# kaleo996/F5E-TTS

Measured on AMD Instinct MI355X. Metric: mel_frames_per_sec, higher is better.
Workload: dtype bf16; 1 GPU; C2: F5TTS_v1_Base random-init, batch 1 per GPU, N_ref=188 N=469 frames, euler NFE=32, CFG=2.0 (cond+uncond batched), sway=-1.0, hipGraph ODE loop, HIP log-mel front-end + Vocos decode on GPU; parallelism=replica x1 (utterance sharding, no collective on the data path)

## Files before the change

### f5e-tts_amd/_C.py

```python
from __future__ import annotations

import ctypes as C
import os

_HERE = os.path.dirname(os.path.abspath(__file__))
LIB_PATH = os.environ.get("F5E_HIP_LIB") or os.path.join(_HERE, "libf5e_hip.so")

ABI_VERSION = 2

ACT_NONE, ACT_SILU, ACT_GELU_ERF, ACT_GELU_TANH, ACT_RELU, ACT_MISH = range(6)

_P, _I, _F, _LL = C.c_void_p, C.c_int, C.c_float, C.c_longlong

SIGNATURES = {
    "f5e_abi_version": [],
    "f5e_last_error": [],
    "f5e_check_device": [],
    "f5e_gemm_bf16_bias": [_P, _P, _I, _P, _I, _P, _P, _I, _I, _I, _I, _I, _I, _I],
    "f5e_gemm_bf16_gate_residual": [_P, _P, _I, _P, _I, _P, _P, _I, _P, _I, _I, _P, _I, _I, _P, _I, _I, _I, _I],
    "f5e_gemm_bf16_qkv_rope": [_P, _P, _I, _P, _I, _P, _P, _P, _P, _I, _I, _I, _P, _P, _P, _I, _I, _I, _I],
    "f5e_gemm_bf16_bias_ln": [_P, _P, _I, _P, _I, _P, _P, _I, _I, _I, _I, _I, _I, _I, _P],
    "f5e_gemm_bf16_gate_residual_ln": [_P, _P, _I, _P, _I, _P, _P, _I, _P, _I, _I, _P, _I, _I, _P, _I, _I, _I, _I, _P],
    "f5e_gemm_bf16_qkv_rope_ln": [_P, _P, _I, _P, _I, _P, _P, _P, _P, _I, _I, _I, _P, _P, _P, _I, _I, _I, _I, _P],
    "f5e_adaln_pre": [_P, _P, _I, _P, _I, _P, _I, _I, _I, _P, _I, _P, _I, _P, _I, _I],
    "f5e_flash_attn": [_P, _P, _P, _P, _P, _I, _P, _I, _I, _I, _I, _I],
    "f5e_joint_attn": [_P, _P, _P, _P, _P, _P, _P, _P, _I, _P, _I, _P, _I, _I, _I, _I, _I, _I, _I],
    "f5e_layernorm": [_P, _P, _I, _P, _I, _I, _P, _P, _P, _P, _I, _I, _I, _P, _I, _I, _I, _F],
    "f5e_grn": [_P, _P, _P, _P, _P, _P, _I, _I, _I],
    "f5e_l2norm": [_P, _P, _I, _P, _I, _I, _P, _I, _I],
    "f5e_gemm_f32": [_P, _P, _I, _I, _I, _P, _I, _P, _I, _P, _P, _I, _I, _P, _P, _I, _P, _I, _I, _I, _I],
    "f5e_convpos": [_P, _P, _I, _P, _P, _I, _P, _I, _P, _I, _P, _I, _I, _I, _I, _I],
    "f5e_dwconv7": [_P, _P, _P, _P, _P, _I, _I, _I],
    "f5e_im2col": [_P, _P, _P, _I, _I, _I, _I, _I],
    "f5e_sinus_embed": [_P, _P, _P, _P, _I, _I, _F],
    "f5e_rope_table": [_P, _P, _P, _I, _I],
    "f5e_text_gather": [_P, _P, _P, _P, _P, _P, _I, _I, _I, _I, _I],
    "f5e_ode_update": [_P, _P, _LL, _I, _F, _F, _P, _P, _P, _P, _P, _P, _LL],
    "f5e_ode_update_traj": [_P, _P, _LL, _I, _F, _F, _P, _P, _P, _LL, _I, _P, _P, _P, _LL],
    "f5e_advance_eval": [_P, _P],
    "f5e_stitch": [_P, _P, _P, _P, _P, _LL, _I],
    "f5e_cast_bf16": [_P, _P, _P, _LL],
    "f5e_cast_f32": [_P, _P, _P, _LL],
    "f5e_axpby": [_P, _P, _P, _P, _F, _F, _F, _LL],
    "f5e_vq_eval": [_P, _P, _I, _P, _I, _P, _P, _P, _I, _I, _I, _I],
    "f5e_mas_workspace_bytes": [_I, _I, _I, C.POINTER(C.c_ulonglong)],
    "f5e_mas_path": [_P, _P, _LL, _I, _P, _P, _P, _P, _P, C.c_ulonglong, _I, _I, _I],
    "f5e_stft_logmel": [_P, _P, _I, _I, _P, _P, _P, _P, _I, _I, _I, _I],
    "f5e_stft_logmel_banded": [_P, _P, _I, _I, _P, _P, _P, _P, _I, _P, _I, _I, _I, _I],
    "f5e_stft_logmel_banded_ex": [_P, _P, _I, _I, _P, _P, _P, _P, _I, _P, _I, _I, _I, _I, _I, _I, _F],
    "f5e_bigvgan_act": [_P, _P, _P, _I, _P, _P, _P, _P, _I, _I, _I],
    "f5e_bigvgan_conv": [_P, _P, _P, _P, _P, _P, _P, _F, _I, _I, _I, _I, _I, _I, _I, _I, _I],
    "f5e_bigvgan_post": [_P, _P, _P, _P, _P, _I, _I, _I, _I, _I],
    "f5e_istft_head": [_P, _P, _I, _P, _P, _P, _P, _I, _I, _I, _I],
    "f5e_kaldi_fbank": [_P, _P, _I, _I, _P, _P, _P, _P, _I, _I, _I, _I, _F, _F, _F],
    "f5e_glu": [_P, _P, _I, _P, _I, _LL, _I],
    "f5e_dwconv": [_P, _P, _P, _P, _P, _P, _I, _I, _I, _I],
    "f5e_softmax_rows": [_P, _P, _I, _P, _I, _P, _LL, _I, _I, _F],
    "f5e_dwconv_stream": [_P, _P, _P, _P, _P, _P, _I, _I, _I, _I, _I, _I],
    "f5e_relpos_attn": [_P, _P, _I, _P, _I, _P, _I, _P, _I, _P, _I, _P, _I, _I, _I, _I, _I, _I, _I, _F],
    "f5e_dit_forward": [_P, _P],
    "f5e_sample_loop": [_P, _P],
    "f5e_workspace_bytes": [_P, _P],
    "f5e_timer_create": [_I, C.POINTER(C.c_void_p)],
    "f5e_timer_destroy": [_P],
    "f5e_timer_reset": [_P],
    "f5e_timer_read": [_P, C.POINTER(C.c_float), _I, C.POINTER(C.c_int)],
    "f5e_timer_read_ops": [_P, C.POINTER(C.c_int), _I, C.POINTER(C.c_int)],
    "f5e_graph_begin": [_P],
    "f5e_graph_end": [_P, C.POINTER(C.c_void_p)],
    "f5e_graph_launch": [_P, _P],
    "f5e_graph_destroy": [_P],
}
_RESTYPE = {"f5e_last_error": C.c_char_p}


class BlockWeights(C.Structure):
    _fields_ = [(n, _P) for n in ("w_qkv", "b_qkv", "w_out", "b_out", "w_ff1", "b_ff1", "w_ff2", "b_ff2",
                                  "q_norm_w", "k_norm_w")]


class LnFuse(C.Structure):
    _fields_ = [("stats", _P), ("parts", _I), ("c", _P), ("d", _P), ("cd_stride", _I), ("cd_rows", _I),
                ("cd_eval_stride", _I), ("eval_ptr", _P), ("rows_per_seq", _I), ("eps", _F),
                ("xs_out", _P), ("ld_xs", _I), ("next_scale", _P), ("stats_out", _P), ("row_mean", _P)]


class DitPlan(C.Structure):
    _fields_ = (
        [(n, _I) for n in ("S", "B", "N", "n_pad", "D", "H", "rope_heads", "FF", "L", "mel", "mod_rows")]
        + [("y", _P), ("w_x", _P), ("ldw_x", _I), ("in_const", _P)]
        + [(n, _P) for n in ("convpos_w1", "convpos_b1", "convpos_w2", "convpos_b2")] + [("convpos_groups", _I)]
        + [(n, _P) for n in ("rope_cs", "seq_len", "mod", "eval_ptr")]
        + [("blocks", C.POINTER(BlockWeights)), ("w_proj", _P), ("b_proj", _P)]
        + [("w_skip", _P), ("skip_res", _P), ("skip_tmp", _P)]
        + [(n, _P) for n in ("h0", "h0_bf16", "c1", "x", "hn", "q", "k", "vt", "ao", "ff", "pred")]
        + [("timer", _P), ("timer_op", _I)]
        + [("fuse_ln", _I), ("ln_stats", _P), ("ln_rowmean", _P), ("cd", _P), ("cd_stride", _I)]
        + [("mall_prefetch", _I)]
    )

class LoopPlan(C.Structure):
    _fields_ = [("eval_a", C.POINTER(DitPlan)), ("eval_b", C.POINTER(DitPlan)), ("steps", _I), ("mode", _I), ("w0", _F),
                ("w1", _F), ("n", _LL), ("y", _P), ("y_mid", _P), ("pred", _P), ("coef", _P), ("eval_ptr", _P),
                ("done_ctr", _P), ("traj", _P)]


WS_NAMES = ("h0", "h0_bf16", "c1", "x", "hn", "q", "k", "vt", "ao", "ff", "pred", "ln_stats", "skip_res", "skip_tmp",
            "ln_rowmean")


class DitWorkspace(C.Structure):
    _fields_ = [("n_pad", _I), ("bytes", C.c_ulonglong * len(WS_NAMES)), ("offset", C.c_ulonglong * len(WS_NAMES)),
                ("total", C.c_ulonglong)]


OP_NONE, OP_INPROJ, OP_CONVPOS, OP_LN, OP_QKV, OP_ATTN, OP_OUT, OP_FF1, OP_FF2, OP_FINAL = range(10)


_lib = None


def lib() -> C.CDLL:
    global _lib
    if _lib is None:
        if not os.path.exists(LIB_PATH):
            raise RuntimeError(
                f"{LIB_PATH} is missing: the HIP extension is required (no CPU/PyTorch fallback exists). "
                "Build it with `make -C f5e-tts_amd/csrc` or `__graft_entry__.build()`."
            )
        handle = C.CDLL(LIB_PATH)
        for name, argtypes in SIGNATURES.items():
            fn = getattr(handle, name)
            fn.argtypes = argtypes
            fn.restype = _RESTYPE.get(name, C.c_int)
        if handle.f5e_abi_version() != ABI_VERSION:
            raise RuntimeError(f"libf5e_hip ABI version {handle.f5e_abi_version()} != {ABI_VERSION}")
        _lib = handle
    return _lib


class F5EError(RuntimeError):
    pass


def check(rc: int, name: str) -> None:
    if rc != 0:
        msg = lib().f5e_last_error()
        raise F5EError(f"{name} failed ({rc}): {msg.decode() if msg else '?'}")
```

### f5e-tts_amd/csrc/conv.hip

```cpp
#include <cstdlib>
#include "f5e_common.h"

namespace {

struct ConvPosArgs {
  const bf16* x; int ldx;
  const bf16* w;
  const float* bias;
  bf16* out_bf16; int ldo;
  float* out_f32; int ldo32;
  const float* resid; int ldr;
  int S, N, D, mode, tiles_t, cpg;
  unsigned long long* trace;
};

__device__ __forceinline__ void glds16c(const void* g, void* lds) {
  __builtin_amdgcn_global_load_lds((const __attribute__((address_space(1))) void*)g,
                                   (__attribute__((address_space(3))) void*)lds, 16, 0, 0);
}

__device__ const uint4 conv_zero16 = {0u, 0u, 0u, 0u};

__device__ __forceinline__ void wait_vm_lgkm0(int n) {
  switch (n) {
// ... 152 lines not shown
}

template <bool TRC = false>
__global__ __launch_bounds__(256) void convpos_split_kernel(ConvPosArgs a) {
  unsigned long long ts[8] = {0, 0, 0, 0, 0, 0, 0, 0};
  if constexpr (TRC) { ts[0] = __builtin_amdgcn_s_memrealtime(); ts[1] = __builtin_amdgcn_s_memtime(); }
  constexpr int BT = 64, HALO = 15, XR = BT + 2 * HALO;
  constexpr int X_BYTES = 96 * 128, W_BYTES = 8192, NST = 4;
  constexpr int TAPS = 31, RS = 68;
  extern __shared__ __attribute__((aligned(16))) char smem[];
  char* Xs = smem;
  char* ring_base = smem + X_BYTES;
  float* Red = (float*)ring_base;

  const int tid = threadIdx.x, lane = tid & 63;
  const int wave = __builtin_amdgcn_readfirstlane(tid >> 6);
  const int g = blockIdx.x, tt = blockIdx.y, seq = blockIdx.z;
  const int c0 = g * a.cpg;
  const int t0 = tt * BT;
  const int fr = lane & 15, fq = lane >> 4;

  const int oc = (lane & 15) * 4;
  const int n = c0 + (oc < a.cpg ? oc : 0);
  f32x4 rv[4];
  if (a.mode == 1) {
#pragma unroll
    for (int p = 0; p < 4; ++p) {
      const int t = t0 + wave * 16 + p * 4 + (lane >> 4);
      rv[p] = *(const f32x4*)(a.resid + ((size_t)seq * a.N + (t < a.N ? t : a.N - 1)) * a.ldr + n);
    }
  }
  const f32x4 bias = *(const f32x4*)(a.bias + n);
  asm volatile("" ::: "memory");
  __builtin_amdgcn_sched_barrier(0);
#pragma unroll
  for (int r = 0; r < 3; ++r) {
    const int i = tid + 256 * r;
    const int row = i >> 3, c = (i & 7) ^ ((row >> 1) & 7);
    const int t = t0 - HALO + row;
    const void* src = &conv_zero16;
    if (row < XR && t >= 0 && t < a.N && c0 + c * 8 < a.D) src = a.x + ((size_t)seq * a.N + t) * a.ldx + c0 + c * 8;
    glds16c(src, Xs + (wave * 64 + 256 * r) * 16);
  }
  asm volatile("" ::: "memory");
  __builtin_amdgcn_sched_barrier(0);

  char* ring = ring_base + wave * (NST * W_BYTES);
  const bf16* wg = a.w + (size_t)g * TAPS * 4096;
  const bf16* w_src[8];
#pragma unroll
  for (int j = 0; j < 8; ++j) {
    const int i = lane + 64 * j;
    const int row = i >> 3, c = (i & 7) ^ ((row >> 1) & 7);
    w_src[j] = wg + row * 64 + c * 8;
  }
  auto stage_w = [&](int slot, int u) {
    int tap = wave + 4 * u;
    tap = tap < TAPS ? tap : TAPS - 1;
#pragma unroll
    for (int j = 0; j < 8; ++j) glds16c(w_src[j] + (size_t)tap * 4096, ring + slot * W_BYTES + j * 1024);
  };
#pragma unroll
  for (int u = 0; u < NST - 1; ++u) stage_w(u, u);

  f32x4 acc[4][4];
#pragma unroll
  for (int i = 0; i < 4; ++i)
#pragma unroll
    for (int j = 0; j < 4; ++j) acc[i][j] = f32x4{0.f, 0.f, 0.f, 0.f};

#pragma unroll
  for (int u = 0; u < 8; ++u) {
    const int issued = u + NST - 1 < 8 ? u + NST - 1 : 8;
    const int pend = 8 * (issued - u - 1);
    if (pend == 16) asm volatile("s_waitcnt vmcnt(16) lgkmcnt(0)" ::: "memory");
    else if (pend == 8) asm volatile("s_waitcnt vmcnt(8) lgkmcnt(0)" ::: "memory");
    else asm volatile("s_waitcnt vmcnt(0) lgkmcnt(0)" ::: "memory");
    if (u == 0) {
      __builtin_amdgcn_s_barrier();
      if constexpr (TRC) ts[2] = __builtin_amdgcn_s_memtime();
    }
    if constexpr (TRC) { if (u == 1) ts[3] = __builtin_amdgcn_s_memtime(); if (u == 4) ts[4] = __builtin_amdgcn_s_memtime(); }
    const int tap = wave + 4 * u;
    const bool live = !(u == 7 && tap >= TAPS);
    const char* Ws = ring + (u % NST) * W_BYTES;
    bf16x8 xf[4], wf[4];
    auto reads = [&](int kk) {
      const int c = kk * 4 + fq;
#pragma unroll
      for (int j = 0; j < 4; ++j) {
        const int row = j * 16 + fr + tap;
        xf[j] = *(const bf16x8*)(Xs + row * 128 + ((c ^ ((row >> 1) & 7)) << 4));
      }
#pragma unroll
      for (int i = 0; i < 4; ++i) {
        const int row = i * 16 + fr;
        wf[i] = *(const bf16x8*)(Ws + row * 128 + ((c ^ ((row >> 1) & 7)) << 4));
      }
    };
    auto mfmas = [&]() {
#pragma unroll
      for (int i = 0; i < 4; ++i)
#pragma unroll
        for (int j = 0; j < 4; ++j)
          acc[i][j] = __builtin_amdgcn_mfma_f32_16x16x32_bf16(wf[i], xf[j], acc[i][j], 0, 0, 0);
    };
    if (live) reads(0);
    if (u + NST - 1 < 8) stage_w((u + NST - 1) % NST, u + NST - 1);
    if (!live) break;
    mfmas();
    reads(1);
    mfmas();
  }

  if constexpr (TRC) ts[5] = __builtin_amdgcn_s_memtime();
  asm volatile("s_waitcnt vmcnt(0) lgkmcnt(0)" ::: "memory");
  __builtin_amdgcn_s_barrier();
  float* mine = Red + wave * (64 * RS);
#pragma unroll
  for (int i = 0; i < 4; ++i)
#pragma unroll
    for (int j = 0; j < 4; ++j) *(f32x4*)(mine + (j * 16 + fr) * RS + i * 16 + fq * 4) = acc[i][j];
  asm volatile("s_waitcnt lgkmcnt(0)" ::: "memory");
  __builtin_amdgcn_s_barrier();
#pragma unroll
  for (int p = 0; p < 4; ++p) asm volatile("" : "+v"(rv[p]));

  if (oc < a.cpg) {
#pragma unroll
    for (int p = 0; p < 4; ++p) {
      const int row = wave * 16 + p * 4 + (lane >> 4);
      const int t = t0 + row;
      const size_t m = (size_t)seq * a.N + t;
      const float* rp = Red + row * RS + oc;
      f32x4 v = (*(const f32x4*)rp + *(const f32x4*)(rp + 64 * RS)) + (*(const f32x4*)(rp + 2 * 64 * RS) + *(const f32x4*)(rp + 3 * 64 * RS));
      v += bias;
      v[0] = mish_f(v[0]); v[1] = mish_f(v[1]); v[2] = mish_f(v[2]); v[3] = mish_f(v[3]);
      if (t >= a.N) continue;
      if (a.mode == 0) {
        *(bf16x4*)(a.out_bf16 + m * a.ldo + n) = f2bf4(v[0], v[1], v[2], v[3]);
      } else {
        v += rv[p];
        *(f32x4*)(a.out_f32 + m * a.ldo32 + n) = v;
      }
    }
  }
  if constexpr (TRC) {
    asm volatile("s_waitcnt vmcnt(0)" ::: "memory");
    ts[6] = __builtin_amdgcn_s_memtime(); ts[7] = __builtin_amdgcn_s_memrealtime();
    if (tid == 0 && a.trace) {
      unsigned long long* o = a.trace + ((size_t)(blockIdx.z * gridDim.y + blockIdx.y) * gridDim.x + blockIdx.x) * 8;
#pragma unroll
      for (int i = 0; i < 8; ++i) o[i] = ts[i];
    }
  }
}

__global__ __launch_bounds__(256) void dwconv7_kernel(const float* x, const float* wT, const float* bias, float* y,
                                                       int B, int T, int C) {
  const int c4n = C / 4;
  const size_t total = (size_t)B * T * c4n;
  for (size_t i = (size_t)blockIdx.x * 256 + threadIdx.x; i < total; i += (size_t)gridDim.x * 256) {
    const int c = (int)(i % c4n) * 4;
    const size_t bt = i / c4n;
    const int t = (int)(bt % T);
    const size_t b = bt / T;
    f32x4 acc = *(const f32x4*)(bias + c);
#pragma unroll
    for (int j = 0; j < 7; ++j) {
      const int tj = t + j - 3;
      if (tj >= 0 && tj < T)
        acc += *(const f32x4*)(wT + (size_t)j * C + c) * *(const f32x4*)(x + (b * T + tj) * C + c);
    }
    *(f32x4*)(y + (b * T + t) * C + c) = acc;
  }
}

__global__ __launch_bounds__(256) void im2col_kernel(const float* x, float* col, int B, int T, int Cin, int ksize,
                                                      int pad) {
  const size_t total = (size_t)B * T * ksize * Cin;
  for (size_t i = (size_t)blockIdx.x * 256 + threadIdx.x; i < total; i += (size_t)gridDim.x * 256) {
    const int ic = (int)(i % Cin);
    size_t r = i / Cin;
    const int j = (int)(r % ksize);
    r /= ksize;
    const int t = (int)(r % T);
    const size_t b = r / T;
    const int tj = t + j - pad;
    col[i] = (tj >= 0 && tj < T) ? x[(b * T + tj) * Cin + ic] : 0.f;
  }
}

inline int grid_for(size_t total) {
  size_t g = (total + 255) / 256;
  return (int)(g < 4096 ? (g ? g : 1) : 4096);
}

}

#ifdef F5E_TOOLS
static unsigned long long* g_convpos_trace = nullptr;
#define F5E_CONVPOS_TRACE g_convpos_trace
#else
#define F5E_CONVPOS_TRACE ((unsigned long long*)nullptr)
#endif

extern "C" {

#ifdef F5E_TOOLS
void f5e_debug_convpos_trace(void* buf) { g_convpos_trace = (unsigned long long*)buf; }
#endif

static int convpos_launch(hipStream_t st, const void* x, int ldx, const void* w_packed, const float* bias, int mode,
                          void* out_bf16, int ldo, float* out_f32, int ldo32, const float* resid, int ldr, int S, int N,
                          int D, int groups) {
  F5E_REQUIRE(x && w_packed && bias, "convpos: null operand");
  F5E_REQUIRE(S > 0 && N > 0 && D > 0 && groups > 0 && D % groups == 0, "convpos: bad D=%d / groups=%d", D, groups);
  const int cpg = D / groups;
  F5E_REQUIRE(cpg % 16 == 0 && cpg <= 64, "convpos: channels per group = %d must be 16, 32, 48 or 64", cpg);
  F5E_REQUIRE(ldx % 8 == 0, "convpos: ldx must be a multiple of 8");
  if (mode == 0) F5E_REQUIRE(out_bf16 && ldo % 4 == 0, "convpos: mode 0 needs a bf16 output");
  else {
    F5E_REQUIRE(mode == 1, "convpos: mode must be 0 or 1");
    F5E_REQUIRE(out_f32 && resid && ldo32 % 4 == 0 && ldr % 4 == 0, "convpos: mode 1 needs f32 output + residual");
  }
  ConvPosArgs a{};
  a.x = (const bf16*)x; a.ldx = ldx; a.w = (const bf16*)w_packed; a.bias = bias;
  a.out_bf16 = (bf16*)out_bf16; a.ldo = ldo; a.out_f32 = out_f32; a.ldo32 = ldo32; a.resid = resid; a.ldr = ldr;
  a.S = S; a.N = N; a.D = D; a.mode = mode; a.cpg = cpg;
  a.tiles_t = (N + 63) / 64;
  F5E_REQUIRE(a.tiles_t <= 65535 && S <= 65535, "convpos: grid too large");
  const dim3 grid(groups, a.tiles_t, S);
  const int xs = 96 * 128;
#ifdef F5E_TOOLS
  static const int forced = getenv("F5E_CONVPOS") ? atoi(getenv("F5E_CONVPOS")) : 0;
#else
  constexpr int forced = 0;
#endif
  const int n_cu = f5e_cu_count();
  const bool split = forced ? forced == 1 : (size_t)groups * a.tiles_t * S <= (size_t)n_cu;
  const int lds_split = xs + 4 * 4 * 8192, lds_ring = xs + 4 * 8192;
  a.trace = F5E_CONVPOS_TRACE;
  static F5eDeviceOnce once_split;
  if (split) F5E_OPT_IN_LDS(once_split, convpos_split_kernel<false>, lds_split);
#ifdef F5E_TOOLS
  static F5eDeviceOnce once_split_trace;
  if (split && a.trace) {
    F5E_OPT_IN_LDS(once_split_trace, convpos_split_kernel<true>, lds_split);
    hipLaunchKernelGGL(convpos_split_kernel<true>, grid, dim3(256), lds_split, st, a);
  } else if (a.trace) {
    hipLaunchKernelGGL((convpos_kernel<4, true>), grid, dim3(256), lds_ring, st, a);
  } else
#endif
  if (split) {
    hipLaunchKernelGGL(convpos_split_kernel<false>, grid, dim3(256), lds_split, st, a);
  } else {
    hipLaunchKernelGGL((convpos_kernel<4, false>), grid, dim3(256), lds_ring, st, a);
  }
  F5E_LAUNCH_CHECK("convpos");
  return F5E_OK;
}

int f5e_convpos(hipStream_t st, const void* x, int ldx, const void* w_packed, const float* bias, int mode,
                void* out_bf16, int ldo, float* out_f32, int ldo32, const float* resid, int ldr, int S, int N, int D,
                int groups) {
  return convpos_launch(st, x, ldx, w_packed, bias, mode, out_bf16, ldo, out_f32, ldo32, resid, ldr, S, N, D, groups);
}

int f5e_dwconv7(hipStream_t st, const float* x, const float* w_t, const float* bias, float* y, int B, int T, int C) {
  F5E_REQUIRE(x && w_t && bias && y, "dwconv7: null operand");
  F5E_REQUIRE(B > 0 && T > 0 && C > 0 && C % 4 == 0, "dwconv7: C=%d must be a positive multiple of 4", C);
  hipLaunchKernelGGL(dwconv7_kernel, dim3(grid_for((size_t)B * T * C / 4)), dim3(256), 0, st, x, w_t, bias, y, B, T, C);
  F5E_LAUNCH_CHECK("dwconv7");
  return F5E_OK;
}

int f5e_im2col(hipStream_t st, const float* x, float* col, int B, int T, int Cin, int ksize, int pad) {
  F5E_REQUIRE(x && col && B > 0 && T > 0 && Cin > 0 && ksize > 0 && pad >= 0, "im2col: bad arguments");
  hipLaunchKernelGGL(im2col_kernel, dim3(grid_for((size_t)B * T * Cin * ksize)), dim3(256), 0, st, x, col, B, T, Cin,
                     ksize, pad);
  F5E_LAUNCH_CHECK("im2col");
  return F5E_OK;
}

}
```

### f5e-tts_amd/csrc/elementwise.hip

```cpp
#include "f5e_common.h"

namespace {

inline int grid_for(size_t total) {
  size_t g = (total + 255) / 256;
  return (int)(g < 2048 ? (g ? g : 1) : 2048);
}

__global__ void sinus_embed_kernel(const float* t, const float* freqs, float* out, int E, int dim, float scale) {
  const int half = dim / 2;
  const int i = blockIdx.x * blockDim.x + threadIdx.x;
  if (i >= E * half) return;
  const int e = i / half, k = i - e * half;
  const float arg = (scale * t[e]) * freqs[k];
  float s, c;
  sincosf(arg, &s, &c);
  out[(size_t)e * dim + k] = s;
  out[(size_t)e * dim + half + k] = c;
}

__global__ void rope_table_kernel(const float* inv_freq, float* out, int N, int half) {
  const int i = blockIdx.x * blockDim.x + threadIdx.x;
  if (i >= N * half) return;
  const int n = i / half, k = i - n * half;
  const float ang = (float)n * inv_freq[k];
  float s, c;
  sincosf(ang, &s, &c);
  out[(size_t)i * 2] = c;
  out[(size_t)i * 2 + 1] = s;
}

__global__ void text_gather_kernel(const int* ids, const float* table, const float* pos, const float* keep, float* out,
                                   int B, int N, int TD, int max_pos, int table_rows) {
  const int td4 = TD / 4;
  const size_t total = (size_t)B * N * td4;
  for (size_t i = (size_t)blockIdx.x * 256 + threadIdx.x; i < total; i += (size_t)gridDim.x * 256) {
    const int c = (int)(i % td4) * 4;
    const size_t bn = i / td4;
    const int n = (int)(bn % N);
    const int id = min(max(ids[bn], 0), table_rows - 1);
    f32x4 v = *(const f32x4*)(table + (size_t)id * TD + c);
    if (pos) v += *(const f32x4*)(pos + (size_t)min(n, max_pos - 1) * TD + c);
    if (keep) v *= keep[bn];
    *(f32x4*)(out + bn * TD + c) = v;
  }
}

__global__ void ode_update_kernel(const float* pred, size_t branch_stride, int mode, float w0, float w1,
                                  const float* base, float* dst, float* traj, size_t traj_stride, int traj_div,
                                  const float* coef, int* eval_ptr, unsigned* done_ctr, size_t n) {
  const int e = eval_ptr ? load_uniform_i32(eval_ptr) : 0;
  const float h = __builtin_bit_cast(float, load_uniform_i32((const int*)(coef + e)));
  if (traj && traj_stride) traj += (size_t)((e + 1) / traj_div) * traj_stride;
  for (size_t i = (size_t)blockIdx.x * 256 + threadIdx.x; i < n; i += (size_t)gridDim.x * 256) {
    const float p0 = pred[i];
    float v = p0;
    if (mode == 1) {
      v = p0 + (p0 - pred[i + branch_stride]) * w0;
    } else if (mode == 2) {
      const float p1 = pred[i + branch_stride], p2 = pred[i + 2 * branch_stride];
      v = w0 * (p2 - p1) + w1 * (p1 - p0) + p0;
    }
    const float y = base[i] + h * v;
    dst[i] = y;
    if (traj) traj[i] = y;
  }
  if (done_ctr) {
    __syncthreads();
    if (threadIdx.x == 0) {
      const unsigned t = atomicAdd(done_ctr, 1u);
      if (t == gridDim.x - 1) {
        *eval_ptr = e + 1;
        *done_ctr = 0u;
      }
    }
  }
}

__global__ void advance_eval_kernel(int* eval_ptr) { *eval_ptr += 1; }

__global__ void stitch_kernel(const float* cond, const float* y, const unsigned char* mask, float* out, size_t rows,
                              int C) {
  const size_t total = rows * C;
  for (size_t i = (size_t)blockIdx.x * 256 + threadIdx.x; i < total; i += (size_t)gridDim.x * 256)
    out[i] = mask[i / C] ? cond[i] : y[i];
}

__global__ void cast_bf16_kernel(const float* x, bf16* y, size_t n) {
  for (size_t i = (size_t)blockIdx.x * 256 + threadIdx.x; i < n; i += (size_t)gridDim.x * 256) y[i] = (bf16)x[i];
}

__global__ void cast_f32_kernel(const bf16* x, float* y, size_t n) {
  for (size_t i = (size_t)blockIdx.x * 256 + threadIdx.x; i < n; i += (size_t)gridDim.x * 256) y[i] = (float)x[i];
}

__global__ void axpby_kernel(const float* x, const float* y, float* out, float a, float b, float c, size_t n) {
  for (size_t i = (size_t)blockIdx.x * 256 + threadIdx.x; i < n; i += (size_t)gridDim.x * 256)
    out[i] = a * x[i] + (y ? b * y[i] : 0.0f) + c;
}

__global__ __launch_bounds__(256) void vq_lookup_kernel(const float* logits, int ld, const float* vars, int combine,
                                                         float* out, int* targets, int rows, int G, int V, int vd) {
  const int lane = threadIdx.x & 63;
  const long long item = (long long)blockIdx.x * 4 + (threadIdx.x >> 6);
  if (item >= (long long)rows * G) return;
  const int r = (int)(item / G), g = (int)(item % G);
  const float* lp = logits + (size_t)r * ld + (size_t)g * V;
  float best = -INFINITY;
  int bi = 0x7fffffff;
  for (int v = lane; v < V; v += 64) {
    const float x = lp[v];
    if (x > best) { best = x; bi = v; }
  }
#pragma unroll
  for (int o = 32; o > 0; o >>= 1) {
    const float ob = __shfl_xor(best, o, 64);
    const int oi = __shfl_xor(bi, o, 64);
    if (ob > best || (ob == best && oi < bi)) { best = ob; bi = oi; }
  }
  if (lane == 0 && targets) targets[(size_t)r * G + g] = bi;
  const float* src = vars + ((size_t)(combine ? 0 : g) * V + bi) * vd;
  for (int d = lane; d < vd; d += 64) out[(size_t)r * G * vd + (size_t)g * vd + d] = src[d];
}

__global__ __launch_bounds__(256) void vq_stats_kernel(const float* logits, int ld, const int* targets, float* stats,
                                                        int rows, int G, int V) {
  extern __shared__ float sm[];
  float* accw = sm;
  float* cnt = sm + 4 * V;
  __shared__ float red[2];
  const int tid = threadIdx.x, lane = tid & 63, wave = tid >> 6;
  float code_ppl = 0.f, prob_ppl = 0.f;
  for (int g = 0; g < G; ++g) {
    for (int i = tid; i < 5 * V; i += 256) sm[i] = 0.f;
    __syncthreads();
    for (int r = wave; r < rows; r += 4) {
      const float* lp = logits + (size_t)r * ld + (size_t)g * V;
      float mx = -INFINITY;
      for (int v = lane; v < V; v += 64) mx = fmaxf(mx, lp[v]);
      mx = wave_max(mx);
      float s = 0.f;
      for (int v = lane; v < V; v += 64) s += expf(lp[v] - mx);
      s = wave_sum(s);
      const float inv = 1.0f / s;
      for (int v = lane; v < V; v += 64) accw[wave * V + v] += expf(lp[v] - mx) * inv;
    }
    __syncthreads();
    if (tid == 0)
      for (int r = 0; r < rows; ++r) cnt[targets[(size_t)r * G + g]] += 1.0f;
    __syncthreads();
    float hc = 0.f, hp = 0.f;
    for (int v = tid; v < V; v += 256) {
      const float p_hard = cnt[v] / (float)rows;
      const float p_avg = ((accw[v] + accw[V + v]) + (accw[2 * V + v] + accw[3 * V + v])) / (float)rows;
      hc += p_hard * logf(p_hard + 1e-7f);
      hp += p_avg * logf(p_avg + 1e-7f);
    }
    hc = wave_sum(hc);
    hp = wave_sum(hp);
    if (tid == 0) { red[0] = 0.f; red[1] = 0.f; }
    __syncthreads();
    if (lane == 0) { atomicAdd(&red[0], hc); atomicAdd(&red[1], hp); }
    __syncthreads();
    code_ppl += expf(-red[0]);
    prob_ppl += expf(-red[1]);
    __syncthreads();
  }
  if (tid == 0) { stats[0] = code_ppl; stats[1] = prob_ppl; }
}

}

extern "C" {

int f5e_sinus_embed(hipStream_t st, const float* t, const float* freqs, float* out, int E, int dim, float scale) {
  F5E_REQUIRE(t && freqs && out && E > 0 && dim >= 4 && dim % 2 == 0, "sinus_embed: bad arguments");
  const int total = E * dim / 2;
  hipLaunchKernelGGL(sinus_embed_kernel, dim3((total + 255) / 256), dim3(256), 0, st, t, freqs, out, E, dim, scale);
  F5E_LAUNCH_CHECK("sinus_embed");
  return F5E_OK;
}

int f5e_rope_table(hipStream_t st, const float* inv_freq, float* out, int N, int half) {
  F5E_REQUIRE(inv_freq && out && N > 0 && half > 0, "rope_table: bad arguments");
  const int total = N * half;
  hipLaunchKernelGGL(rope_table_kernel, dim3((total + 255) / 256), dim3(256), 0, st, inv_freq, out, N, half);
  F5E_LAUNCH_CHECK("rope_table");
  return F5E_OK;
}

int f5e_text_gather(hipStream_t st, const int* ids, const float* table, const float* pos, const float* keep,
                    float* out, int B, int N, int TD, int max_pos, int table_rows) {
  F5E_REQUIRE(ids && table && out && B > 0 && N > 0 && TD > 0 && TD % 4 == 0 && table_rows > 0, "text_gather: bad arguments");
  hipLaunchKernelGGL(text_gather_kernel, dim3(grid_for((size_t)B * N * TD / 4)), dim3(256), 0, st, ids, table, pos,
                     keep, out, B, N, TD, max_pos, table_rows);
  F5E_LAUNCH_CHECK("text_gather");
  return F5E_OK;
}

int f5e_ode_update(hipStream_t st, const float* pred, long long branch_stride, int mode, float w0, float w1,
                   const float* base, float* dst, float* traj, const float* coef, int* eval_ptr, unsigned* done_ctr,
                   long long n) {
  return f5e_ode_update_traj(st, pred, branch_stride, mode, w0, w1, base, dst, traj, 0, 1, coef, eval_ptr, done_ctr, n);
}

int f5e_ode_update_traj(hipStream_t st, const float* pred, long long branch_stride, int mode, float w0, float w1,
                        const float* base, float* dst, float* traj, long long traj_stride, int traj_div,
                        const float* coef, int* eval_ptr, unsigned* done_ctr, long long n) {
  F5E_REQUIRE(pred && base && dst && coef && n > 0, "ode_update: bad arguments");
  F5E_REQUIRE(mode >= 0 && mode <= 2, "ode_update: mode must be 0 (plain), 1 (cfg) or 2 (three-branch)");
  F5E_REQUIRE(!done_ctr || eval_ptr, "ode_update: done_ctr (auto-advance) needs eval_ptr");
  F5E_REQUIRE(traj_stride >= 0 && traj_div >= 1 && (traj_stride == 0 || eval_ptr), "ode_update: bad trajectory indexing");
  hipLaunchKernelGGL(ode_update_kernel, dim3(grid_for((size_t)n)), dim3(256), 0, st, pred, (size_t)branch_stride, mode,
                     w0, w1, base, dst, traj, (size_t)traj_stride, traj_div, coef, eval_ptr, done_ctr, (size_t)n);
  F5E_LAUNCH_CHECK("ode_update");
  return F5E_OK;
// ... 58 lines not shown
```

### f5e-tts_amd/csrc/f5e_common.h

```cpp
#pragma once
#include <hip/hip_runtime.h>
#include <stdint.h>
#define F5E_STREAM_T hipStream_t
#include "../../include/f5e_abi.h"

typedef __bf16 bf16;
typedef __attribute__((ext_vector_type(2))) __bf16 bf16x2;
typedef __attribute__((ext_vector_type(4))) __bf16 bf16x4;
typedef __attribute__((ext_vector_type(8))) __bf16 bf16x8;
typedef __attribute__((ext_vector_type(2))) float f32x2;
typedef __attribute__((ext_vector_type(4))) float f32x4;
typedef __attribute__((ext_vector_type(16))) float f32x16;

#define F5E_WAVE 64

void f5e_set_error(const char* fmt, ...);

#define F5E_REQUIRE(cond, ...)                         \
  do {                                                 \
    if (!(cond)) {                                     \
      f5e_set_error(__VA_ARGS__);                      \
      return F5E_ERR_BAD_SHAPE;                        \
    }                                                  \
  } while (0)

#include <atomic>
inline int f5e_device_index() {
  int dev = 0;
  (void)hipGetDevice(&dev);
  return dev < 0 ? 0 : (dev > 63 ? 63 : dev);
}
struct F5eDeviceOnce {
  std::atomic<unsigned long long> done{0};
};
inline hipError_t f5e_opt_in_lds(F5eDeviceOnce& once, const void* kernel, int lds_bytes) {
  const unsigned long long bit = 1ull << f5e_device_index();
  if (once.done.load(std::memory_order_acquire) & bit) return hipSuccess;
  hipError_t e = hipFuncSetAttribute(kernel, hipFuncAttributeMaxDynamicSharedMemorySize, lds_bytes);
  if (e == hipSuccess) once.done.fetch_or(bit, std::memory_order_release);
  return e;
}
#define F5E_OPT_IN_LDS(once, kernel, lds)                                                    \
  do {                                                                                       \
    hipError_t e_ = f5e_opt_in_lds(once, (const void*)(kernel), lds);                        \
    if (e_ != hipSuccess) {                                                                  \
      f5e_set_error("hipFuncSetAttribute(%d B of LDS): %s", (int)(lds), hipGetErrorString(e_)); \
      return F5E_ERR_HIP;                                                                    \
    }                                                                                        \
  } while (0)
inline int f5e_cu_count() {
  static std::atomic<int> cache[64];
  const int dev = f5e_device_index();
  int n = cache[dev].load(std::memory_order_relaxed);
  if (n == 0) {
    int v = 0;
    if (hipDeviceGetAttribute(&v, hipDeviceAttributeMultiprocessorCount, dev) != hipSuccess || v <= 0) v = 256;
    cache[dev].store(v, std::memory_order_relaxed);
    n = v;
  }
  return n;
}

struct F5ePrefetch {
  const void* ptr[2];
  unsigned bytes[2];
};
constexpr int F5E_PF_BYTES_PER_WG = 32 * 1024;
inline int f5e_prefetch_wgs(const F5ePrefetch* pf) {
  if (!pf) return 0;
  unsigned long long b = (pf->ptr[0] ? pf->bytes[0] : 0) + (unsigned long long)(pf->ptr[1] ? pf->bytes[1] : 0);
  return (int)((b + F5E_PF_BYTES_PER_WG - 1) / F5E_PF_BYTES_PER_WG);
}
template <int NT = 256>
__device__ __forceinline__ void f5e_prefetch_run(const F5ePrefetch& pf, int wg, int tid, void* lds) {
  unsigned long long off = (unsigned long long)wg * F5E_PF_BYTES_PER_WG + (unsigned)tid * 16u;
  const unsigned long long b0 = pf.ptr[0] ? pf.bytes[0] : 0, b1 = pf.ptr[1] ? pf.bytes[1] : 0;
  char* dst = (char*)lds + (tid >> 6) * 1024;
#pragma unroll
  for (int i = 0; i < F5E_PF_BYTES_PER_WG / (NT * 16); ++i, off += NT * 16) {
    const char* p = nullptr;
    if (off + 16 <= b0) p = (const char*)pf.ptr[0] + off;
    else if (off >= b0 && off - b0 + 16 <= b1) p = (const char*)pf.ptr[1] + (off - b0);
    if (p)
      __builtin_amdgcn_global_load_lds((const __attribute__((address_space(1))) void*)p,
                                       (__attribute__((address_space(3))) void*)dst, 16, 0, 0);
  }
}

__device__ __forceinline__ void f5e_prefetch_run_packed(const F5ePrefetch& pf, int wg, int tid, int nt, unsigned per_wg,
                                                        void* lds) {
  unsigned long long off = (unsigned long long)wg * per_wg + (unsigned)tid * 16u;
  const unsigned long long end = (unsigned long long)(wg + 1) * per_wg;
  const unsigned long long b0 = pf.ptr[0] ? pf.bytes[0] : 0, b1 = pf.ptr[1] ? pf.bytes[1] : 0;
  char* dst = (char*)lds + (tid >> 6) * 1024;
  for (; off < end; off += (unsigned)nt * 16u) {
    const char* p = nullptr;
    if (off + 16 <= b0) p = (const char*)pf.ptr[0] + off;
    else if (off >= b0 && off - b0 + 16 <= b1) p = (const char*)pf.ptr[1] + (off - b0);
    if (p)
      __builtin_amdgcn_global_load_lds((const __attribute__((address_space(1))) void*)p,
                                       (__attribute__((address_space(3))) void*)dst, 16, 0, 0);
  }
}

int f5e_gemm_bf16_bias_pf(hipStream_t st, const void* A, int lda, const void* W, int ldw, const float* bias, void* out,
                          int ldo, int M, int N, int K, int act, int out_f32, int tile_hint, const f5e_ln_fuse* ln,
                          const F5ePrefetch* pf);
int f5e_gemm_bf16_gate_residual_pf(hipStream_t st, const void* A, int lda, const void* W, int ldw, const float* bias,
                                   float* resid, int ldr, const float* gate, int gate_stride, int gate_rows,
                                   const int* eval_ptr, int eval_stride, int rows_per_seq, const int* seq_len, int M,
                                   int N, int K, int tile_hint, const f5e_ln_fuse* ln, const F5ePrefetch* pf);
int f5e_gemm_bf16_qkv_rope_pf(hipStream_t st, const void* A, int lda, const void* W, int ldw, const float* bias, void* q,
                              void* k, void* vt, int n_pad, int heads, int rope_heads, const float* cos_sin,
                              const float* q_norm_w, const float* k_norm_w, int rows_per_seq, int M, int K, int tile_hint,
                              const f5e_ln_fuse* ln, const F5ePrefetch* pf);
int f5e_flash_attn_pf(hipStream_t st, const void* q, const void* k, const void* v, void* o, int ldo, const int* kv_len,
                      int S, int H, int rows_per_seq, int n_pad, int splits, const F5ePrefetch* pf);

#define F5E_LAUNCH_CHECK(name)                                                   \
  do {                                                                           \
    hipError_t e_ = hipGetLastError();                                           \
    if (e_ != hipSuccess) {                                                      \
      f5e_set_error("%s: launch failed: %s", name, hipGetErrorString(e_));       \
      return F5E_ERR_HIP;                                                        \
    }                                                                            \
  } while (0)

__device__ __forceinline__ int load_uniform_i32(const int* p) {
  return *(const __attribute__((address_space(4))) int*)(uintptr_t)p;
}

__device__ __forceinline__ bf16x4 f2bf4(float a, float b, float c, float d) {
  f32x4 v = {a, b, c, d};
  return __builtin_convertvector(v, bf16x4);
}
__device__ __forceinline__ bf16x2 f2bf2(float a, float b) {
  f32x2 v = {a, b};
  return __builtin_convertvector(v, bf16x2);
}
template <int CTRL>
__device__ __forceinline__ float dpp_f32(float v) {
  return __builtin_bit_cast(float, __builtin_amdgcn_update_dpp(0, __builtin_bit_cast(int, v), CTRL, 0xF, 0xF, false));
}
__device__ __forceinline__ float add_xor1(float v) { return v + dpp_f32<0xB1>(v); }
__device__ __forceinline__ float add_xor2(float v) { return v + dpp_f32<0x4E>(v); }
__device__ __forceinline__ void swap16(float& a, float& b) {
  asm volatile("s_nop 1\n\tv_permlane16_swap_b32 %0, %1" : "+v"(a), "+v"(b));
}
__device__ __forceinline__ void swap32(float& a, float& b) {
  asm volatile("s_nop 1\n\tv_permlane32_swap_b32 %0, %1" : "+v"(a), "+v"(b));
}
__device__ __forceinline__ float add_xor16(float v) {
  float a = v, b = v;
  swap16(a, b);
  return a + b;
}
__device__ __forceinline__ float add_xor32(float v) {
  float a = v, b = v;
  swap32(a, b);
  return a + b;
}
__device__ __forceinline__ float max_xor32(float v) {
  float a = v, b = v;
  swap32(a, b);
  return fmaxf(a, b);
}
__device__ __forceinline__ float wave_sum(float v) {
  v = add_xor1(v);
  v = add_xor2(v);
  v += dpp_f32<0x124>(v);
  v += dpp_f32<0x128>(v);
  v = add_xor16(v);
  return add_xor32(v);
}
__device__ __forceinline__ float wave_max(float v) {
#pragma unroll
  for (int o = 32; o > 0; o >>= 1) v = fmaxf(v, __shfl_xor(v, o, 64));
  return v;
}
__device__ __forceinline__ float gelu_tanh_f(float x) {
  const float t = x * x;
  const float p = __builtin_fmaf(t, -2.0f * 0.7978845608028654f * 1.4426950408889634f * 0.044715f,
                                 -2.0f * 0.7978845608028654f * 1.4426950408889634f);
  const float e = __builtin_amdgcn_exp2f(x * p);
  return x * __builtin_amdgcn_rcpf(1.0f + e);
}
__device__ __forceinline__ float gelu_erf_f(float x) { return 0.5f * x * (1.0f + erff(x * 0.7071067811865476f)); }
__device__ __forceinline__ float silu_f(float x) { return x / (1.0f + __expf(-x)); }
__device__ __forceinline__ float mish_f(float x) {
  const float e = __builtin_amdgcn_exp2f(fminf(x, 20.0f) * 1.4426950408889634f);
  const float n = e * (e + 2.0f);
  const float r = x * (n * __builtin_amdgcn_rcpf(n + 2.0f));
  return x > 20.0f ? x : r;
}
__device__ __forceinline__ float apply_act(float x, int act) {
  switch (act) {
    case F5E_ACT_SILU: return silu_f(x);
    case F5E_ACT_GELU_ERF: return gelu_erf_f(x);
    case F5E_ACT_GELU_TANH: return gelu_tanh_f(x);
    case F5E_ACT_RELU: return fmaxf(x, 0.0f);
    case F5E_ACT_MISH: return mish_f(x);
    default: return x;
  }
}
```

### f5e-tts_amd/csrc/gemm_bf16.hip

```cpp
#include <cstdlib>
#include <type_traits>

#include "f5e_common.h"
#include "gemm_bf16_args.h"

namespace {

using namespace f5e_gemm;

template <int N>
__device__ __forceinline__ void wait_vm_lgkm0() {
  asm volatile("s_waitcnt vmcnt(%0) lgkmcnt(0)" ::"n"(N) : "memory");
}

template <int LPT, int EXTRA>
__device__ __forceinline__ void wait_stages(int nst) {
  constexpr auto C = [](int v) constexpr { return v > 63 ? 63 : v; };
  switch (nst) {
    case 0: wait_vm_lgkm0<C(EXTRA)>(); break;
    case 1: wait_vm_lgkm0<C(LPT + EXTRA)>(); break;
    case 2: wait_vm_lgkm0<C(2 * LPT + EXTRA)>(); break;
    case 3: wait_vm_lgkm0<C(3 * LPT + EXTRA)>(); break;
    case 4: wait_vm_lgkm0<C(4 * LPT + EXTRA)>(); break;
    case 5: wait_vm_lgkm0<C(5 * LPT + EXTRA)>(); break;
    default: wait_vm_lgkm0<C(6 * LPT + EXTRA)>(); break;
  }
}

template <int BM, int BN, int EPI, int NSTAGE, int DBG = 0, int WGM = 2, int WGN = 2, int FUSE = 0, int NLOAD = 0, int DSTEP = 1, int DBUF = 1>
__global__ __launch_bounds__(64 * (WGM * WGN + NLOAD)) void gemm_bf16_kernel(GemmArgs a) {
  constexpr int BK = 64;
  constexpr int CPR = BK / 8;
  constexpr int ROWB = BK * 2;
  auto swz = [](int row) { return (row >> 1) & 7; };
  constexpr int NCW = WGM * WGN;
  constexpr int NC = 64 * NCW;
  constexpr int NT = NLOAD ? 64 * NLOAD : NC;
  constexpr int A_BYTES = BM * BK * 2;
  constexpr int W_BYTES = BN * BK * 2;
  constexpr int STAGE = A_BYTES + W_BYTES;
  constexpr int WM = BM / WGM, WN = BN / WGN;
  constexpr int TM = WM / 16, TN = WN / 16;
  extern __shared__ __attribute__((aligned(16))) char smem[];

  const int lane = threadIdx.x & 63;
  const int wave = __builtin_amdgcn_readfirstlane(threadIdx.x >> 6);
  const int tid = (int)threadIdx.x;
  const bool is_loader = NLOAD > 0 && wave >= NCW;
  const int stid = NLOAD ? tid - NC : tid;
  const int swave = NLOAD ? wave - NCW : wave;
  unsigned long long* trc = nullptr;
  if constexpr (DBG >= 3) {
    trc = a.trace + (size_t)blockIdx.x * 48;
    if (tid == 0) { trc[0] = __builtin_amdgcn_s_memrealtime(); trc[1] = __builtin_amdgcn_s_memtime(); }
  }

  if (FUSE == 1)
    asm volatile("" ::"s"(a.ln_stats), "s"(a.ln_c), "s"(a.ln_d), "s"(a.ln_parts), "s"(a.cd_stride), "s"(a.cd_rows),
                 "s"(a.cd_eval_stride), "s"(a.eval_ptr));
  if (EPI == EPI_GATE_RES)
    asm volatile("" ::"s"(a.resid), "s"(a.gate), "s"(a.seq_len), "s"(a.eval_ptr), "s"(a.ldr), "s"(a.gate_stride),
                 "s"(a.gate_rows), "s"(a.eval_stride), "s"(a.bias));
  if (FUSE == 2) asm volatile("" ::"s"(a.next_scale), "s"(a.xs_out), "s"(a.stats_out), "s"(a.ld_xs), "s"(a.row_mean));
  if (EPI == EPI_QKV_ROPE) asm volatile("" ::"s"(a.q), "s"(a.k), "s"(a.vt), "s"(a.cos_sin), "s"(a.n_pad), "s"(a.heads), "s"(a.rope_heads));

  if ((int)blockIdx.x >= a.n_main) {
    if (NLOAD > 0 && a.pf_per_wg) f5e_prefetch_run_packed(a.pf, (int)blockIdx.x - a.n_main, tid, 64 * (NCW + NLOAD), a.pf_per_wg, smem);
    else if (tid < 256) f5e_prefetch_run(a.pf, (int)blockIdx.x - a.n_main, tid, smem);
    return;
  }
  int bid = blockIdx.x;
  {
    const int nblk = a.n_main;
    const int q8 = nblk >> 3, r8 = nblk & 7;
    const int xcd = bid & 7, idx = bid >> 3;
    bid = (xcd < r8 ? xcd * (q8 + 1) : r8 * (q8 + 1) + (xcd - r8) * q8) + idx;
  }
  int tile_m, tile_n;
  if (a.m_major > 0) {
    tile_m = div_magic(bid, a.tiles_n, a.tile_magic);
    tile_n = bid - tile_m * a.tiles_n;
  } else {
    const int sh = -a.m_major, per = a.tiles_m << sh;
    const int g = div_magic(bid, per, a.tile_magic);
    const int r = bid - g * per;
    tile_m = r >> sh;
    tile_n = (g << sh) + (r & ((1 << sh) - 1));
  }
  const int m0 = tile_m * BM, n0 = tile_n * BN;

  constexpr int A_IT = BM * CPR / NT;
  constexpr int W_IT = BN * CPR / NT;
  static_assert(A_IT >= 1 && W_IT >= 1 && A_IT * NT == BM * CPR && W_IT * NT == BN * CPR, "tile / thread-count mismatch");
  unsigned a_off[A_IT], w_off[W_IT];
#pragma unroll
  for (int j = 0; j < A_IT; ++j) {
    const int i = (stid & (NT - 1)) + NT * j;
    const int row = i / CPR, c = (i % CPR) ^ swz(row);
    a_off[j] = (unsigned)(min(m0 + row, a.M - 1) - m0) * (unsigned)(a.lda * 2) + (unsigned)c * 16u;
  }
#pragma unroll
  for (int j = 0; j < W_IT; ++j) {
    const int i = (stid & (NT - 1)) + NT * j;
    const int row = i / CPR, c = (i % CPR) ^ swz(row);
    w_off[j] = (unsigned)(min(n0 + row, a.N - 1) - n0) * (unsigned)(a.ldw * 2) + (unsigned)c * 16u;
  }
  const char* const a_base = (const char*)(a.A + (size_t)m0 * a.lda);
  const char* const w_base = (const char*)(a.W + (size_t)n0 * a.ldw);
  const int KT = a.K / BK;
  char* const ring = smem;
  auto stage = [&](int buf, int kt) {
    char* base = ring + buf * STAGE;
    const char* ak = a_base + (size_t)kt * (BK * 2);
    const char* wk = w_base + (size_t)kt * (BK * 2);
#pragma unroll
    for (int j = 0; j < A_IT; ++j) glds16_s(ak, a_off[j], base + (swave * 64 + NT * j) * 16);
#pragma unroll
    for (int j = 0; j < W_IT; ++j) glds16_s(wk, w_off[j], base + A_BYTES + (swave * 64 + NT * j) * 16);
  };

  const int wm0 = (wave / WGN) * WM, wn0 = (wave % WGN) * WN;
  const int fr = lane & 15, fq = lane >> 4;

  f32x4 acc[TN][TM];
#pragma unroll
  for (int i = 0; i < TN; ++i)
#pragma unroll
    for (int j = 0; j < TM; ++j) acc[i][j] = f32x4{0.f, 0.f, 0.f, 0.f};

  constexpr int LPT = A_IT + W_IT;
  static_assert(NSTAGE >= 2 && NSTAGE <= 8 && (DSTEP > 1 || (NSTAGE - 2) * LPT <= 63), "vmcnt is a 6-bit counter");
  static_assert((NT & (NT - 1)) == 0, "staging thread count must be a power of two");
  static_assert(DSTEP == 1 || (NLOAD > 0 && DSTEP == 2 && NSTAGE >= 3 * DSTEP), "DSTEP: role split, ring of >= 3 steps");
  constexpr int NPRO = NSTAGE - DSTEP;
  static_assert((NSTAGE - 2 * DSTEP) * LPT <= 63, "vmcnt is a 6-bit counter");
  if (NLOAD == 0 || is_loader) {
#pragma unroll
    for (int s = 0; s < NPRO; ++s)
      if (s < KT) stage(s, s);
  }
  if constexpr (NLOAD > 0) {
    if (is_loader) {
      int nbuf_l = NPRO % NSTAGE;
      if constexpr (DBG >= 3) { if (stid == 0) trc[47] = __builtin_amdgcn_s_memtime(); }
      for (int kt = 0; kt < KT; kt += DSTEP) {
        const int rem = KT - DSTEP - kt;
        wait_stages<LPT, 0>(rem < NSTAGE - 2 * DSTEP ? (rem < 0 ? 0 : rem) : NSTAGE - 2 * DSTEP);
        __builtin_amdgcn_s_barrier();
#pragma unroll
        for (int d = 0; d < DSTEP; ++d) {
          if (kt + NPRO + d < KT) stage(nbuf_l, kt + NPRO + d);
          nbuf_l = (nbuf_l + 1 == NSTAGE) ? 0 : nbuf_l + 1;
        }
      }
      if (FUSE == 1) __syncthreads();
      if (FUSE == 2) __builtin_amdgcn_s_barrier();
      return;
    }
  }
  asm volatile("" ::: "memory");
  if constexpr (DBG >= 3) { if (tid == 0) trc[46] = __builtin_amdgcn_s_memtime(); }
  constexpr bool PREF = (TM * TN <= 4);
  static_assert(FUSE != 2 || (PREF && WM == 32 && WN == 32 && BN == 64 && (BM == 64 || (BM == 128 && NLOAD > 0))),
                "fused AdaLN producer: 64 (or, role split, 128) x 64 tiles of 32 x 32 wave sub-tiles");
  static_assert(FUSE != 1 || (WN == 32 && (BN == 64 || NLOAD > 0) && ((BM == 64 && WM == 32) || (BM == 128 && WM == 64 && NLOAD > 0))),
                "fused AdaLN consumer: 64-row tiles of 32 x 32 wave sub-tiles, or (role split) 128-row tiles of 64 x 32 ones");
  static_assert(DBUF == 1 || (NLOAD > 0 && DSTEP == 1), "single fragment set: role split, one tile per hand-over");
  constexpr int NSTATT = BM * 4;
  static_assert(FUSE != 1 || NSTATT <= NC, "fused consumer: 4 statistics threads per row");
  static_assert(FUSE != 2 || EPI == EPI_GATE_RES, "the AdaLN producer is the gate+residual epilogue");
  constexpr int NPC = NLOAD ? 0 : (FUSE == 1 ? 2 * TN + 4 : (FUSE == 2 ? 3 * TM * TN : ((PREF && EPI == EPI_GATE_RES) ? 2 * TM * TN : 0)));
  static_assert((NSTAGE - 2) * LPT + NPC <= 63, "vmcnt is a 6-bit counter");
  constexpr bool COLG = NLOAD > 0;
  f32x4 pf_bias[PREF ? TN : 1], pf_gate[PREF ? TN : 1][PREF ? (COLG ? 1 : TM) : 1], pf_x[PREF ? TN : 1][PREF ? TM : 1];
  f32x4 pf_c[FUSE == 1 ? TN : 1], pf_d[FUSE == 1 ? TN : 1];
  f32x4 pf_ns[FUSE == 2 ? TN : 1][FUSE == 2 ? (COLG ? 1 : TM) : 1];
  f32x2 pf_st[FUSE == 1 ? 4 : 1];
  bool pf_live[PREF ? TM : 1];
  int pf_len[PREF ? TM : 1];
  float pf_rm[FUSE == 2 ? TM : 1];
  auto ldv4 = [](const float* ptr) -> f32x4 { return *(const f32x4*)ptr; };
  auto fetch_epilogue_operands = [&]() {
    if (PREF) {
      if (EPI == EPI_GATE_RES) {
        const size_t eoff = a.eval_ptr ? (size_t)load_uniform_i32(a.eval_ptr) * a.eval_stride : 0;
#pragma unroll
        for (int j = 0; j < TM; ++j) {
          const int m = m0 + wm0 + j * 16 + fr, mc = min(m, a.M - 1);
          const int seq = div_magic(mc, a.rows_per_seq, a.rps_magic);
#pragma unroll
          for (int i = 0; i < TN; ++i) {
            const int nc = min(n0 + wn0 + i * 16 + fq * 4, a.N - 4);
            const size_t goff = eoff + ((COLG || a.gate_rows == 1) ? 0 : (size_t)(seq % a.gate_rows) * a.gate_stride) + nc;
            if (!COLG || j == 0) pf_gate[i][COLG ? 0 : j] = ldv4(a.gate + goff);
            pf_x[i][j] = ldv4(a.resid + (size_t)mc * a.ldr + nc);
            if (FUSE == 2 && (!COLG || j == 0)) pf_ns[i][COLG ? 0 : j] = ldv4(a.next_scale + goff);
          }
        }
      }
    }
    if (FUSE == 1) {
      const size_t eoff = a.eval_ptr ? (size_t)load_uniform_i32(a.eval_ptr) * a.cd_eval_stride : 0;
      const float* cbase = a.ln_c + eoff;
      const float* dbase = a.ln_d + eoff;
#pragma unroll
      for (int i = 0; i < TN; ++i) {
        const unsigned nc = (unsigned)min(n0 + wn0 + i * 16 + fq * 4, a.N - 4);
        pf_c[i] = ldv4(cbase + nc);
        pf_d[i] = ldv4(dbase + nc);
      }
      const int pp = a.ln_parts >> 2;
      const float* sbase = a.ln_stats + (size_t)m0 * a.ln_parts * 2;
      const unsigned rel_max = (unsigned)((a.M - m0) * a.ln_parts - 1);
#pragma unroll
      for (int u = 0; u < 4; ++u) {
        const unsigned rel = min((unsigned)((tid & (NSTATT - 1)) * pp + min(u, pp - 1)), rel_max);
        if (NC == NSTATT || tid < NSTATT) pf_st[u] = *(const f32x2*)(sbase + rel * 2u);
      }
    }
    if (PREF) {
#pragma unroll
      for (int i = 0; i < TN; ++i) {
        const int n = n0 + wn0 + i * 16 + fq * 4;
        pf_bias[i] = (a.bias && n < a.N) ? *(const f32x4*)(a.bias + n) : f32x4{0.f, 0.f, 0.f, 0.f};
      }
      if (EPI == EPI_GATE_RES) {
#pragma unroll
        for (int j = 0; j < TM; ++j) {
          const int mc = min(m0 + wm0 + j * 16 + fr, a.M - 1);
          pf_len[j] = a.seq_len ? a.seq_len[div_magic(mc, a.rows_per_seq, a.rps_magic)] : a.rows_per_seq;
          if (FUSE == 2) pf_rm[j] = a.row_mean[mc];
        }
      }
    }
  };
  if (NLOAD == 0) fetch_epilogue_operands();

  int buf = 0, nbuf = NSTAGE - 1;
  if constexpr (DBG >= 3) { if (tid == 0) trc[2] = __builtin_amdgcn_s_memtime(); }
  if constexpr (NLOAD > 0) {
    bf16x8 xs2[DBUF + 1][BK / 32][TM], ws2[DBUF + 1][BK / 32][TN];
    auto reads = [&](auto pc, int b) {
      constexpr int P = decltype(pc)::value;
      const char* As = ring + b * STAGE;
      const char* Ws = As + A_BYTES;
#pragma unroll
      for (int kk = 0; kk < BK / 32; ++kk) {
        const int c = kk * 4 + fq;
#pragma unroll
        for (int j = 0; j < TM; ++j) {
          const int row = wm0 + j * 16 + fr;
          xs2[P][kk][j] = *(const bf16x8*)(As + row * ROWB + ((c ^ swz(row)) << 4));
        }
#pragma unroll
        for (int i = 0; i < TN; ++i) {
          const int row = wn0 + i * 16 + fr;
          ws2[P][kk][i] = *(const bf16x8*)(Ws + row * ROWB + ((c ^ swz(row)) << 4));
        }
      }
    };
    auto mfmas = [&](auto pc) {
      constexpr int P = decltype(pc)::value;
#pragma unroll
      for (int kk = 0; kk < BK / 32; ++kk)
#pragma unroll
        for (int i = 0; i < TN; ++i)
#pragma unroll
          for (int j = 0; j < TM; ++j)
            acc[i][j] = __builtin_amdgcn_mfma_f32_16x16x32_bf16(ws2[P][kk][i], xs2[P][kk][j], acc[i][j], 0, 0, 0);
    };
    auto body = [&](auto pc, int kt) {
      constexpr int P = decltype(pc)::value;
      if (DSTEP == 1 || P == 0) __builtin_amdgcn_s_barrier();
      if constexpr (DBG >= 3) { if (tid == 0 && kt < 36) trc[4 + kt] = __builtin_amdgcn_s_memtime(); }
      reads(pc, buf);
      if (kt > 0) mfmas(std::integral_constant<int, 1 - P>{});
      if (DSTEP == 1 || P == 1) asm volatile("s_waitcnt lgkmcnt(0)" ::: "memory");
      buf = (buf + 1 == NSTAGE) ? 0 : buf + 1;
    };
    if constexpr (DBUF == 0) {
      auto reads_half = [&](int kk, int b) {
        if constexpr (DBG == 5) return;
        const char* As = ring + b * STAGE;
        const char* Ws = As + A_BYTES;
        const int c = kk * 4 + fq;
#pragma unroll
        for (int j = 0; j < TM; ++j) {
          const int row = wm0 + j * 16 + fr;
          xs2[0][kk][j] = *(const bf16x8*)(As + row * ROWB + ((c ^ swz(row)) << 4));
        }
#pragma unroll
        for (int i = 0; i < TN; ++i) {
          const int row = wn0 + i * 16 + fr;
          ws2[0][kk][i] = *(const bf16x8*)(Ws + row * ROWB + ((c ^ swz(row)) << 4));
        }
      };
      auto mfmas_half = [&](int kk) {
        if constexpr (DBG == 4 || DBG == 5) return;
#pragma unroll
        for (int i = 0; i < TN; ++i)
#pragma unroll
          for (int j = 0; j < TM; ++j)
            acc[i][j] = __builtin_amdgcn_mfma_f32_16x16x32_bf16(ws2[0][kk][i], xs2[0][kk][j], acc[i][j], 0, 0, 0);
      };
      static_assert(BK == 64, "half-tile pipelining: two 32-k halves per K-tile");
      for (int kt = 0; kt < KT; ++kt) {
        __builtin_amdgcn_s_barrier();
        if constexpr (DBG >= 3) { if (tid == 0 && kt < 36) trc[4 + kt] = __builtin_amdgcn_s_memtime(); }
        reads_half(0, buf);
        if (kt > 0) mfmas_half(1);
        if (kt == 0) fetch_epilogue_operands();
        asm volatile("s_waitcnt lgkmcnt(0)" ::: "memory");
        reads_half(1, buf);
        mfmas_half(0);
        asm volatile("s_waitcnt lgkmcnt(0)" ::: "memory");
        buf = (buf + 1 == NSTAGE) ? 0 : buf + 1;
      }
      mfmas_half(1);
    } else {
      for (int kt = 0; kt < KT; kt += 2) {
        body(std::integral_constant<int, 0>{}, kt);
        if (kt == 0) fetch_epilogue_operands();
        if (kt + 1 < KT) body(std::integral_constant<int, 1>{}, kt + 1);
      }
      if ((KT - 1) & 1) mfmas(std::integral_constant<int, 1>{});
      else mfmas(std::integral_constant<int, 0>{});
    }
  } else
  for (int kt = 0; kt < KT; ++kt) {
    const int rem = KT - 1 - kt;
    const int nst = rem < NSTAGE - 2 ? rem : NSTAGE - 2;
    if (NPC > 0 && kt <= NSTAGE - 2) wait_stages<LPT, NPC>(nst);
    else wait_stages<LPT, 0>(nst);
    __builtin_amdgcn_s_barrier();
    if constexpr (DBG >= 3) { if (tid == 0 && kt < 36) trc[4 + kt] = __builtin_amdgcn_s_memtime(); }
    const bool more = kt + NSTAGE - 1 < KT;
    const char* As = ring + buf * STAGE;
    const char* Ws = As + A_BYTES;
    bf16x8 xf[BK / 32][TM], wf[BK / 32][TN];
#pragma unroll
    for (int kk = 0; kk < BK / 32; ++kk) {
      const int c = kk * 4 + fq;
#pragma unroll
      for (int j = 0; j < TM; ++j) {
        const int row = wm0 + j * 16 + fr;
        xf[kk][j] = *(const bf16x8*)(As + row * ROWB + ((c ^ swz(row)) << 4));
      }
#pragma unroll
      for (int i = 0; i < TN; ++i) {
        const int row = wn0 + i * 16 + fr;
        wf[kk][i] = *(const bf16x8*)(Ws + row * ROWB + ((c ^ swz(row)) << 4));
      }
    }
    if (more) stage(nbuf, kt + NSTAGE - 1);
#pragma unroll
    for (int kk = 0; kk < BK / 32; ++kk)
#pragma unroll
      for (int i = 0; i < TN; ++i)
#pragma unroll
        for (int j = 0; j < TM; ++j)
          acc[i][j] = __builtin_amdgcn_mfma_f32_16x16x32_bf16(wf[kk][i], xf[kk][j], acc[i][j], 0, 0, 0);
    buf = (buf + 1 == NSTAGE) ? 0 : buf + 1;
    nbuf = (nbuf + 1 == NSTAGE) ? 0 : nbuf + 1;
  }

  if constexpr (DBG >= 3) { if (tid == 0) trc[3] = __builtin_amdgcn_s_memtime(); }
  float* fuse_lds = (float*)(smem + NSTAGE * STAGE);
  if (FUSE == 1) {
    const int sq = tid & 3, pp = a.ln_parts >> 2;
    float sm = 0.f;
#pragma unroll
    for (int u = 0; u < 4; ++u)
      if (u < pp) sm += pf_st[u][0];
    sm = add_xor2(add_xor1(sm));
    const float mean = sm / (float)a.ln_parts;
    const float cols = (float)(a.K / a.ln_parts);
    float m2 = 0.f;
#pragma unroll
    for (int u = 0; u < 4; ++u)
      if (u < pp) {
        const float dm = pf_st[u][0] - mean;
        m2 += pf_st[u][1] + cols * dm * dm;
      }
    m2 = add_xor2(add_xor1(m2));
    if (sq == 0 && (NC == NSTATT || tid < NSTATT)) {
      fuse_lds[(tid >> 2) * 2] = mean;
      fuse_lds[(tid >> 2) * 2 + 1] = rsqrtf(m2 / (float)a.K + a.ln_eps);
      if (tile_n == 0 && m0 + (tid >> 2) < a.M) a.row_mean[m0 + (tid >> 2)] += mean;
    }
    __syncthreads();
    if constexpr (DBG >= 3) { if (tid == 0) trc[42] = __builtin_amdgcn_s_memtime(); }
  }
  f32x4 xn[FUSE == 2 ? TN : 1][FUSE == 2 ? TM : 1];
  if (PREF && EPI == EPI_GATE_RES) {
#pragma unroll
    for (int j = 0; j < TM; ++j) {
      const int m = m0 + wm0 + j * 16 + fr;
      pf_live[j] = (m < a.M) && (m - div_magic(m, a.rows_per_seq, a.rps_magic) * a.rows_per_seq < pf_len[j]);
    }
  }

  int qkv_which = 0, qkv_head = 0, qkv_d0 = 0;
  bf16* qkv_base = nullptr;
  size_t qkv_seq_stride = 0;
  if (EPI == EPI_QKV_ROPE) {
    static_assert(EPI != EPI_QKV_ROPE || WN <= 64, "a wave's columns must stay inside one 64-wide head");
    const int inner = a.heads * 64, hb = n0 + wn0;
    qkv_which = hb / inner;
    qkv_head = (hb - qkv_which * inner) >> 6;
    qkv_d0 = hb & 63;
    qkv_seq_stride = (size_t)a.heads * a.n_pad * 64;
    qkv_base = (qkv_which == 0 ? a.q : (qkv_which == 1 ? a.k : a.vt)) + (size_t)qkv_head * a.n_pad * 64;
  }

#pragma unroll
  for (int j = 0; j < TM; ++j) {
    const int m = m0 + wm0 + j * 16 + fr;
    if (FUSE == 2) {
#pragma unroll
      for (int i = 0; i < TN; ++i) xn[i][j] = pf_x[i][j];
    }
    if (m >= a.M) continue;
    float ln_mean = 0.f, ln_rstd = 1.f;
    if (FUSE == 1) {
      ln_mean = fuse_lds[(wm0 + j * 16 + fr) * 2];
      ln_rstd = fuse_lds[(wm0 + j * 16 + fr) * 2 + 1];
    }
    int seq = 0, pos = m;
    if (EPI == EPI_GATE_RES || EPI == EPI_QKV_ROPE) {
      seq = div_magic(m, a.rows_per_seq, a.rps_magic);
      pos = m - seq * a.rows_per_seq;
    }
    float qk_rn = 1.0f;
    const float* qk_w = nullptr;
    if constexpr (EPI == EPI_QKV_ROPE && WN == 64) {
      const int which_w = (n0 + wn0) / (a.heads * 64);
      if (a.qn_w && which_w < 2) {
        float ss = 0.f;
#pragma unroll
        for (int i = 0; i < TN; ++i) {
          f32x4 t = acc[i][j];
          if (a.bias) t += *(const f32x4*)(a.bias + n0 + wn0 + i * 16 + fq * 4);
          ss += (t[0] * t[0] + t[1] * t[1]) + (t[2] * t[2] + t[3] * t[3]);
        }
        ss = add_xor32(add_xor16(ss));
        qk_rn = rsqrtf(ss * (1.0f / 64.0f) + a.qk_eps);
        qk_w = which_w == 0 ? a.qn_w : a.kn_w;
      }
    }
#pragma unroll
    for (int i = 0; i < TN; ++i) {
      const int n = n0 + wn0 + i * 16 + fq * 4;
      if (n >= a.N) continue;
      f32x4 v = acc[i][j];
      if (FUSE == 1) {
        v = ln_rstd * (v - ln_mean * pf_c[i]) + pf_d[i];
      } else if (PREF) {
        v += pf_bias[i];
      } else if (a.bias) {
        const f32x4 b = *(const f32x4*)(a.bias + n);
        v += b;
      }
      if (EPI == EPI_BF16) {
        *(bf16x4*)((bf16*)a.out + (size_t)m * a.ldo + n) = f2bf4(v[0], v[1], v[2], v[3]);
      } else if (EPI == EPI_BF16_GELU) {
        *(bf16x4*)((bf16*)a.out + (size_t)m * a.ldo + n) =
            f2bf4(gelu_tanh_f(v[0]), gelu_tanh_f(v[1]), gelu_tanh_f(v[2]), gelu_tanh_f(v[3]));
      } else if (EPI == EPI_F32) {
        *(f32x4*)((float*)a.out + (size_t)m * a.ldo + n) = v;
      } else if (EPI == EPI_GATE_RES && PREF) {
        if (pf_live[j]) {
          const f32x4 x_new = pf_x[i][j] + pf_gate[i][COLG ? 0 : j] * v;
          *(f32x4*)(a.resid + (size_t)m * a.ldr + n) = x_new;
          if (FUSE == 2) xn[i][j] = x_new;
        }
        if (FUSE == 2) {
          const f32x4 y = (xn[i][j] - pf_rm[j]) * (1.0f + pf_ns[i][COLG ? 0 : j]);
          *(bf16x4*)(a.xs_out + (size_t)m * a.ld_xs + n) = f2bf4(y[0], y[1], y[2], y[3]);
        }
      } else if (EPI == EPI_GATE_RES) {
        const bool live = (a.seq_len == nullptr) || (pos < a.seq_len[seq]);
        if (live) {
          const size_t eoff = a.eval_ptr ? (size_t)load_uniform_i32(a.eval_ptr) * a.eval_stride : 0;
          const f32x4 g = *(const f32x4*)(a.gate + eoff + (size_t)(seq % a.gate_rows) * a.gate_stride + n);
          float* xp = a.resid + (size_t)m * a.ldr + n;
          f32x4 x = *(const f32x4*)xp;
          x += g * v;
          *(f32x4*)xp = x;
        }
      } else if (EPI == EPI_QKV_ROPE) {
        const int d = qkv_d0 + i * 16 + fq * 4;
        if (qk_w) v = v * qk_rn * *(const f32x4*)(qk_w + d);
        if (qkv_which < 2) {
          if (qkv_head < a.rope_heads) {
            const f32x4 cs = *(const f32x4*)(a.cos_sin + (size_t)pos * 64 + d);
            const float x0 = v[0], x1 = v[1], x2 = v[2], x3 = v[3];
            v[0] = x0 * cs[0] - x1 * cs[1];
            v[1] = x1 * cs[0] + x0 * cs[1];
            v[2] = x2 * cs[2] - x3 * cs[3];
            v[3] = x3 * cs[2] + x2 * cs[3];
          }
          if (qkv_which == 0) v *= a.q_scale;
          const int off = (pos >> 5) * 2048 + (pos & 31) * 16 + (d >> 4) * 512 + ((d >> 3) & 1) * 8 + (d & 7);
          *(bf16x4*)(qkv_base + (size_t)seq * qkv_seq_stride + off) = f2bf4(v[0], v[1], v[2], v[3]);
        } else {
          const int k16 = pos & 15;
          const int off = (pos >> 4) * 1024 + (d >> 5) * 512 + (d & 31) * 16 + ((k16 >> 2) & 1) * 8 + (((k16 >> 3) << 2) | (k16 & 3));
          bf16* dst = qkv_base + (size_t)seq * qkv_seq_stride + off;
          dst[0] = (bf16)v[0];
          dst[16] = (bf16)v[1];
          dst[32] = (bf16)v[2];
          dst[48] = (bf16)v[3];
        }
      }
    }
  }
  if constexpr (DBG >= 3) { if (tid == 0) trc[43] = __builtin_amdgcn_s_memtime(); }
  if (FUSE == 2) {
#pragma unroll
    for (int j = 0; j < TM; ++j) {
      float sm = 0.f;
#pragma unroll
      for (int i = 0; i < TN; ++i) sm += (xn[i][j][0] + xn[i][j][1]) + (xn[i][j][2] + xn[i][j][3]);
      sm = add_xor32(add_xor16(sm));
      const float mw = sm * (1.0f / (float)WN);
      float q2 = 0.f;
#pragma unroll
      for (int i = 0; i < TN; ++i) {
        const f32x4 dv = xn[i][j] - mw;
        q2 += (dv[0] * dv[0] + dv[1] * dv[1]) + (dv[2] * dv[2] + dv[3] * dv[3]);
      }
      q2 = add_xor32(add_xor16(q2));
      if (fq == 0) {
        float* slot = fuse_lds + ((wm0 + j * 16 + fr) * WGN + (wave % WGN)) * 2;
        slot[0] = mw - pf_rm[j];
        slot[1] = q2;
      }
    }
    if constexpr (DBG >= 3) { if (tid == 0) trc[44] = __builtin_amdgcn_s_memtime(); }
    asm volatile("s_waitcnt lgkmcnt(0)" ::: "memory");
    __builtin_amdgcn_s_barrier();
    if constexpr (DBG >= 3) { if (tid == 0) trc[45] = __builtin_amdgcn_s_memtime(); }
    if (tid < BM && m0 + tid < a.M) {
      const float ma = fuse_lds[tid * 4], qa = fuse_lds[tid * 4 + 1], mb = fuse_lds[tid * 4 + 2], qb = fuse_lds[tid * 4 + 3];
      const float dm = ma - mb;
      float* dst = a.stats_out + ((size_t)(m0 + tid) * a.tiles_n + tile_n) * 2;
      dst[0] = 0.5f * (ma + mb);
      dst[1] = (qa + qb) + (0.25f * (float)BN) * dm * dm;
    }
  }
  if constexpr (DBG >= 3) {
    asm volatile("s_waitcnt vmcnt(0)" ::: "memory");
    if (tid == 0) { trc[40] = __builtin_amdgcn_s_memtime(); trc[41] = __builtin_amdgcn_s_memrealtime(); }
  }
}

inline int pick_group_shift(int tiles_m, int tiles_n, int bm, int bn) {
  struct Memo { int tm, tn, bm, bn, s; };
  static thread_local Memo memo[4] = {};
  static thread_local int next = 0;
  for (const Memo& e : memo)
    if (e.tm == tiles_m && e.tn == tiles_n && e.bm == bm && e.bn == bn) return e.s;
#ifdef F5E_TOOLS
  if (const char* f = getenv("F5E_GEMM_GROUP_SHIFT")) {
    const int s = atoi(f);
    if (s >= 0 && s <= 4 && tiles_n % (1 << s) == 0) return s;
  }
#endif
  const int n = tiles_m * tiles_n, q8 = n >> 3, r8 = n & 7;
  long best = -1;
  int best_s = 0;
  for (int s = 0; s <= 4 && (tiles_n % (1 << s)) == 0 && (1 << s) <= tiles_n; ++s) {
    long cost = 0;
    int id = 0;
    for (int x = 0; x < 8; ++x) {
      const int cnt = q8 + (x < r8 ? 1 : 0);
      unsigned long long seen_m[4] = {}, seen_n[4] = {};
      for (int i = 0; i < cnt; ++i, ++id) {
        const int per = tiles_m << s, g = id / per, r = id - g * per;
        const int tm = r >> s, tn = (g << s) + (r & ((1 << s) - 1));
        seen_m[(tm >> 6) & 3] |= 1ull << (tm & 63);
        seen_n[(tn >> 6) & 3] |= 1ull << (tn & 63);
      }
      for (int w = 0; w < 4; ++w) cost += (long)__builtin_popcountll(seen_m[w]) * bm + (long)__builtin_popcountll(seen_n[w]) * bn;
    }
    if (best < 0 || cost < best) { best = cost; best_s = s; }
  }
  memo[next] = Memo{tiles_m, tiles_n, bm, bn, best_s};
  next = (next + 1) & 3;
  return best_s;
}

inline bool pack_prefetch_on() {
#ifdef F5E_TOOLS
  if (const char* f = getenv("F5E_PF_PACK")) return atoi(f) != 0;
#endif
  return true;
}

template <int BM, int BN, int EPI, int NSTAGE, int WGM = 2, int WGN = 2, int DBG = 0, int FUSE = 0, int NLOAD = 0, int DSTEP = 1, int DBUF = 1>
int launch(GemmArgs& a, hipStream_t st) {
  constexpr int BK = 64;
  a.tiles_m = (a.M + BM - 1) / BM;
  a.tiles_n = (a.N + BN - 1) / BN;
  if (a.M > a.N) {
    a.m_major = 1;
    a.tile_magic = div_magic_of(a.tiles_n);
  } else {
    const int sh = (a.tiles_m <= 256 && a.tiles_n <= 256) ? pick_group_shift(a.tiles_m, a.tiles_n, BM, BN) : 0;
    a.m_major = -sh;
    a.tile_magic = div_magic_of(a.tiles_m << sh);
  }
  a.rps_magic = div_magic_of(a.rows_per_seq);
  a.n_main = a.tiles_m * a.tiles_n;
  int pf_wgs = ((WGM * WGN == 4 || NLOAD > 0) && a.n_main <= 3 * 256) ? f5e_prefetch_wgs(&a.pf) : 0;
  a.pf_per_wg = 0;
  constexpr int lds = NSTAGE * (BM + BN) * BK * 2 + (FUSE ? BM * 16 : 0);
  if (NLOAD > 0 && 2 * lds > 160 * 1024 && pf_wgs > 0 && pack_prefetch_on()) {
    const int idle = f5e_cu_count() - a.n_main;
    if (idle <= 0) {
      pf_wgs = 0;
    } else if (pf_wgs > idle) {
      constexpr unsigned gran = 64u * (WGM * WGN + NLOAD) * 16u;
      const unsigned long long total = (unsigned long long)pf_wgs * F5E_PF_BYTES_PER_WG;
      a.pf_per_wg = (unsigned)(((total + idle - 1) / idle + gran - 1) / gran * gran);
      pf_wgs = (int)((total + a.pf_per_wg - 1) / a.pf_per_wg);
    }
  }
  const int grid = a.n_main + pf_wgs;
  if (grid == a.n_main) a.pf = F5ePrefetch{};
  static_assert(lds <= 160 * 1024, "LDS budget");
  static F5eDeviceOnce lds_once;
  if (lds > 65536) F5E_OPT_IN_LDS(lds_once, (gemm_bf16_kernel<BM, BN, EPI, NSTAGE, DBG, WGM, WGN, FUSE, NLOAD, DSTEP, DBUF>), lds);
  hipLaunchKernelGGL((gemm_bf16_kernel<BM, BN, EPI, NSTAGE, DBG, WGM, WGN, FUSE, NLOAD, DSTEP, DBUF>), dim3(grid), dim3(64 * (WGM * WGN + NLOAD)), lds, st, a);
  F5E_LAUNCH_CHECK("gemm_bf16");
  return F5E_OK;
}

inline bool role_split_on() {
#ifdef F5E_TOOLS
  if (const char* f = getenv("F5E_GEMM_ROLE")) return atoi(f) != 0;
#endif
  return true;
}
inline int role_var() {
#ifdef F5E_TOOLS
  if (const char* f = getenv("F5E_GEMM_VAR")) return atoi(f);
#endif
  return -1;
}

inline bool big_tiles_on() {
#ifdef F5E_TOOLS
  if (const char* f = getenv("F5E_GEMM_BIG")) return atoi(f) != 0;
#endif
  return true;
}

template <int EPI>
int dispatch(GemmArgs& a, hipStream_t st, int tile_hint) {
  auto blocks = [&](int bm, int bn) { return ((a.M + bm - 1) / bm) * ((a.N + bn - 1) / bn); };
  int sel = tile_hint;
  F5E_REQUIRE(sel == 0 || sel == 1 || sel == 2 || sel == 3 || sel == 9, "gemm_bf16: unknown tile_hint %d (0, 1, 2, 3 or 9)", tile_hint);
  if (a.ln_stats || a.stats_out) {
    F5E_REQUIRE(!(a.ln_stats && a.stats_out), "gemm_bf16: a launch is an AdaLN consumer or a producer, not both");
    F5E_REQUIRE(!(EPI == EPI_QKV_ROPE && a.qn_w), "gemm_bf16: fused AdaLN and qk_norm need different tiles");
    if constexpr (EPI == EPI_GATE_RES) {
      F5E_REQUIRE(a.stats_out && !a.ln_stats, "gemm_bf16: the gate+residual epilogue is the AdaLN producer");
      if (role_split_on() && a.gate_rows == 1 && blocks(64, 64) <= 256) {
        if (a.K % 128 == 0 && role_var() != 0) return launch<64, 64, EPI, 6, 2, 2, 0, 2, 4, 2>(a, st);
        return launch<64, 64, EPI, 4, 2, 2, 0, 2, 4, 1>(a, st);
      }
      if (role_split_on() && a.gate_rows == 1 && big_tiles_on() && blocks(128, 64) <= 256) {
        if (a.K % 128 == 0) return launch<128, 64, EPI, 6, 4, 2, 0, 2, 4, 2>(a, st);
        return launch<128, 64, EPI, 4, 4, 2, 0, 2, 4, 1>(a, st);
      }
      if (a.K >= 2048 && blocks(64, 64) <= 256) return launch<64, 64, EPI, 4, 2, 2, 0, 2>(a, st);
      return launch<64, 64, EPI, 3, 2, 2, 0, 2>(a, st);
    } else {
      F5E_REQUIRE(a.ln_stats && !a.stats_out, "gemm_bf16: this epilogue can only consume AdaLN statistics");
      if (role_split_on()) {
        int wide = 3;
#ifdef F5E_TOOLS
        if (const char* f = getenv("F5E_GEMM_WIDE")) wide = atoi(f);
#endif
        if constexpr (EPI == EPI_QKV_ROPE) {
          if ((wide & 1) && a.N % 192 == 0 && blocks(64, 192) <= 256) {
            return launch<64, 192, EPI, 4, 2, 6, 0, 1, 4, 1>(a, st);
          }
          if (big_tiles_on() && a.N % 192 == 0 && blocks(128, 192) <= 256) return launch<128, 192, EPI, 3, 2, 6, 0, 1, 4, 1, 0>(a, st);
        } else {
          if ((wide & 2) && a.N % 128 == 0 && blocks(64, 128) <= 256) {
#ifdef F5E_TOOLS
            if (role_var() == 0) return launch<64, 128, EPI, 3, 2, 4, 0, 1, 4, 1>(a, st);
#endif
            if (a.K % 128 == 0) return launch<64, 128, EPI, 6, 2, 4, 0, 1, 4, 2>(a, st);
          }
          if (big_tiles_on() && a.N % 128 == 0 && blocks(128, 128) <= 256) return launch<128, 128, EPI, 4, 2, 4, 0, 1, 4, 1, 0>(a, st);
        }
      }
      return launch<64, 64, EPI, 3, 2, 2, 0, 1>(a, st);
    }
  }
  if (sel == 9 || (sel == 0 && uses_pp(a.M, a.K))) return launch_pp(EPI, a, st);
  if (EPI == EPI_QKV_ROPE && a.qn_w) sel = 1;
  if (sel == 0) {
    if (blocks(128, 128) >= 320) sel = 1;
    else if (blocks(128, 64) >= 512) sel = 2;
    else sel = 3;
  }
  if (sel == 1) return launch<128, 128, EPI, 2, 4, 2>(a, st);
  if (sel == 2) return launch<128, 64, EPI, 3>(a, st);
  if constexpr (EPI == EPI_GATE_RES) {
    if (role_split_on() && a.gate_rows == 1 && blocks(64, 64) <= 256) return launch<64, 64, EPI, 4, 2, 2, 0, 0, 4>(a, st);
  }
  if (a.K >= 2048 && blocks(64, 64) <= 256) return launch<64, 64, EPI, 4>(a, st);
  return launch<64, 64, EPI, 3>(a, st);
}

int check_common(const GemmArgs& a) {
  F5E_REQUIRE(a.M > 0 && a.N > 0 && a.K > 0, "gemm_bf16: empty problem M=%d N=%d K=%d", a.M, a.N, a.K);
  F5E_REQUIRE(a.K % 64 == 0, "gemm_bf16: K=%d must be a multiple of 64", a.K);
  F5E_REQUIRE(a.N % 4 == 0, "gemm_bf16: N=%d must be a multiple of 4", a.N);
  F5E_REQUIRE(a.lda % 8 == 0 && a.ldw % 8 == 0, "gemm_bf16: lda/ldw must be multiples of 8 elements");
  F5E_REQUIRE(a.A && a.W, "gemm_bf16: null operand");
  return F5E_OK;
}

int set_consumer(GemmArgs& a, const f5e_ln_fuse* ln, const float* bias) {
  if (!ln || !ln->stats) return F5E_OK;
  F5E_REQUIRE(bias == nullptr, "gemm_bf16: with fused AdaLN the bias is part of the d table");
  F5E_REQUIRE(ln->c && ln->d && ln->parts > 0 && ln->parts <= 16 && ln->parts % 4 == 0 && ln->cd_rows == 1 && a.K % ln->parts == 0 && ln->cd_rows > 0 &&
                  ln->cd_stride % 4 == 0 && ln->cd_eval_stride % 4 == 0 && ln->rows_per_seq > 0,
              "gemm_bf16: bad fused-AdaLN consumer arguments (parts=%d: a multiple of 4 up to 16; one table row per evaluation)",
              ln->parts);
  a.ln_stats = ln->stats; a.ln_parts = ln->parts; a.ln_c = ln->c; a.ln_d = ln->d; a.cd_stride = ln->cd_stride;
  a.cd_rows = ln->cd_rows; a.cd_eval_stride = ln->cd_eval_stride; a.ln_eps = ln->eps;
  a.eval_ptr = ln->eval_ptr;
  F5E_REQUIRE(ln->row_mean, "gemm_bf16: the fused-AdaLN consumer needs f5e_ln_fuse.row_mean (the rows' centring offsets)");
  a.row_mean = ln->row_mean;
  if (a.rows_per_seq <= 0) a.rows_per_seq = ln->rows_per_seq;
  return F5E_OK;
}

}

int f5e_gemm_bf16_bias_pf(hipStream_t st, const void* A, int lda, const void* W, int ldw, const float* bias, void* out,
                          int ldo, int M, int N, int K, int act, int out_f32, int tile_hint, const f5e_ln_fuse* ln,
                          const F5ePrefetch* pf) {
  GemmArgs a{};
  if (pf) a.pf = *pf;
  a.A = (const bf16*)A; a.lda = lda; a.W = (const bf16*)W; a.ldw = ldw; a.bias = bias;
  a.M = M; a.N = N; a.K = K; a.out = out; a.ldo = ldo;
  if (int e = check_common(a)) return e;
  if (int e = set_consumer(a, ln, bias)) return e;
  F5E_REQUIRE(out && ldo % 4 == 0, "gemm_bf16_bias: bad output");
  if (out_f32) {
    F5E_REQUIRE(act == F5E_ACT_NONE, "gemm_bf16_bias: f32 output supports no activation");
    return dispatch<EPI_F32>(a, st, tile_hint);
  }
  if (act == F5E_ACT_GELU_TANH) return dispatch<EPI_BF16_GELU>(a, st, tile_hint);
  F5E_REQUIRE(act == F5E_ACT_NONE, "gemm_bf16_bias: unsupported activation %d", act);
  return dispatch<EPI_BF16>(a, st, tile_hint);
}

int f5e_gemm_bf16_gate_residual_pf(hipStream_t st, const void* A, int lda, const void* W, int ldw, const float* bias,
                                   float* resid, int ldr, const float* gate, int gate_stride, int gate_rows,
                                   const int* eval_ptr, int eval_stride, int rows_per_seq, const int* seq_len, int M,
                                   int N, int K, int tile_hint, const f5e_ln_fuse* ln, const F5ePrefetch* pf) {
  GemmArgs a{};
  if (pf) a.pf = *pf;
  a.A = (const bf16*)A; a.lda = lda; a.W = (const bf16*)W; a.ldw = ldw; a.bias = bias;
  a.M = M; a.N = N; a.K = K;
  a.resid = resid; a.ldr = ldr; a.gate = gate; a.gate_stride = gate_stride; a.gate_rows = gate_rows;
  a.rows_per_seq = rows_per_seq; a.seq_len = seq_len; a.eval_ptr = eval_ptr; a.eval_stride = eval_stride;
  if (int e = check_common(a)) return e;
  F5E_REQUIRE(resid && gate && ldr % 4 == 0 && gate_stride % 4 == 0 && gate_rows > 0 && rows_per_seq > 0,
              "gemm_bf16_gate_residual: bad residual/gate arguments");
  if (ln && ln->stats_out) {
    F5E_REQUIRE(ln->xs_out && ln->next_scale && ln->row_mean && ln->ld_xs % 4 == 0 && N % 64 == 0,
                "gemm_bf16_gate_residual: AdaLN producer needs xs_out, next_scale, row_mean and N %% 64 == 0");
    a.xs_out = (bf16*)ln->xs_out; a.ld_xs = ln->ld_xs; a.next_scale = ln->next_scale; a.stats_out = ln->stats_out;
    a.row_mean = ln->row_mean;
  }
  return dispatch<EPI_GATE_RES>(a, st, tile_hint);
}

int f5e_gemm_bf16_qkv_rope_pf(hipStream_t st, const void* A, int lda, const void* W, int ldw, const float* bias, void* q,
                              void* k, void* vt, int n_pad, int heads, int rope_heads, const float* cos_sin,
                              const float* q_norm_w, const float* k_norm_w, int rows_per_seq, int M, int K, int tile_hint,
                              const f5e_ln_fuse* ln, const F5ePrefetch* pf) {
  GemmArgs a{};
  if (pf) a.pf = *pf;
  a.A = (const bf16*)A; a.lda = lda; a.W = (const bf16*)W; a.ldw = ldw; a.bias = bias;
  a.M = M; a.N = 3 * heads * 64; a.K = K;
  a.q = (bf16*)q; a.k = (bf16*)k; a.vt = (bf16*)vt; a.n_pad = n_pad; a.heads = heads; a.rope_heads = rope_heads;
  a.cos_sin = cos_sin; a.rows_per_seq = rows_per_seq;
  a.qn_w = q_norm_w; a.kn_w = k_norm_w; a.qk_eps = 1e-6f;
  a.q_scale = 0.125f * 1.4426950408889634f;
  F5E_REQUIRE((q_norm_w == nullptr) == (k_norm_w == nullptr), "gemm_bf16_qkv_rope: q and k norm weights go together");
  if (int e = check_common(a)) return e;
  F5E_REQUIRE(q && k && vt && cos_sin, "gemm_bf16_qkv_rope: null output/table");
  F5E_REQUIRE(heads > 0 && rope_heads >= 0 && rope_heads <= heads, "gemm_bf16_qkv_rope: bad head counts");
  F5E_REQUIRE(rows_per_seq > 0 && n_pad >= rows_per_seq && n_pad % 64 == 0,
              "gemm_bf16_qkv_rope: n_pad=%d must be a multiple of 64 and >= rows_per_seq=%d", n_pad, rows_per_seq);
  if (int e = set_consumer(a, ln, bias)) return e;
  return dispatch<EPI_QKV_ROPE>(a, st, tile_hint);
}

extern "C" {

int f5e_gemm_bf16_bias(hipStream_t st, const void* A, int lda, const void* W, int ldw, const float* bias, void* out,
                       int ldo, int M, int N, int K, int act, int out_f32, int tile_hint) {
  return f5e_gemm_bf16_bias_ln(st, A, lda, W, ldw, bias, out, ldo, M, N, K, act, out_f32, tile_hint, nullptr);
}

int f5e_gemm_bf16_bias_ln(hipStream_t st, const void* A, int lda, const void* W, int ldw, const float* bias, void* out,
                          int ldo, int M, int N, int K, int act, int out_f32, int tile_hint, const f5e_ln_fuse* ln) {
  return f5e_gemm_bf16_bias_pf(st, A, lda, W, ldw, bias, out, ldo, M, N, K, act, out_f32, tile_hint, ln, nullptr);
}

int f5e_gemm_bf16_gate_residual(hipStream_t st, const void* A, int lda, const void* W, int ldw, const float* bias,
                                float* resid, int ldr, const float* gate, int gate_stride, int gate_rows,
                                const int* eval_ptr, int eval_stride, int rows_per_seq, const int* seq_len, int M,
                                int N, int K, int tile_hint) {
  return f5e_gemm_bf16_gate_residual_ln(st, A, lda, W, ldw, bias, resid, ldr, gate, gate_stride, gate_rows, eval_ptr,
                                        eval_stride, rows_per_seq, seq_len, M, N, K, tile_hint, nullptr);
}

int f5e_gemm_bf16_gate_residual_ln(hipStream_t st, const void* A, int lda, const void* W, int ldw, const float* bias,
                                   float* resid, int ldr, const float* gate, int gate_stride, int gate_rows,
                                   const int* eval_ptr, int eval_stride, int rows_per_seq, const int* seq_len, int M,
                                   int N, int K, int tile_hint, const f5e_ln_fuse* ln) {
  return f5e_gemm_bf16_gate_residual_pf(st, A, lda, W, ldw, bias, resid, ldr, gate, gate_stride, gate_rows, eval_ptr,
                                        eval_stride, rows_per_seq, seq_len, M, N, K, tile_hint, ln, nullptr);
}

int f5e_gemm_bf16_qkv_rope(hipStream_t st, const void* A, int lda, const void* W, int ldw, const float* bias, void* q,
                           void* k, void* vt, int n_pad, int heads, int rope_heads, const float* cos_sin,
                           const float* q_norm_w, const float* k_norm_w, int rows_per_seq, int M, int K,
                           int tile_hint) {
  return f5e_gemm_bf16_qkv_rope_ln(st, A, lda, W, ldw, bias, q, k, vt, n_pad, heads, rope_heads, cos_sin, q_norm_w,
                                   k_norm_w, rows_per_seq, M, K, tile_hint, nullptr);
}

int f5e_gemm_bf16_qkv_rope_ln(hipStream_t st, const void* A, int lda, const void* W, int ldw, const float* bias,
                              void* q, void* k, void* vt, int n_pad, int heads, int rope_heads, const float* cos_sin,
                              const float* q_norm_w, const float* k_norm_w, int rows_per_seq, int M, int K,
                              int tile_hint, const f5e_ln_fuse* ln) {
  return f5e_gemm_bf16_qkv_rope_pf(st, A, lda, W, ldw, bias, q, k, vt, n_pad, heads, rope_heads, cos_sin, q_norm_w,
                                   k_norm_w, rows_per_seq, M, K, tile_hint, ln, nullptr);
}

}
```

### f5e-tts_amd/csrc/gemm_bf16_args.h

```cpp
#pragma once
#include <cstddef>

#include "f5e_common.h"

namespace f5e_gemm {

struct GemmArgs {
  const bf16* A; const bf16* W;
  int lda, ldw;
  int M, N, K;
  int tiles_m, tiles_n, m_major;
  unsigned tile_magic;
  int rows_per_seq;
  unsigned rps_magic;
  int n_main;
  const float* bias;
  void* out; int ldo;
  float* resid; int ldr;
  const float* gate; int gate_stride; int gate_rows;
  const int* eval_ptr; int eval_stride;
  const int* seq_len;
  bf16* q; bf16* k; bf16* vt;
  int n_pad; int heads; int rope_heads;
  const float* cos_sin;
  const float* qn_w; const float* kn_w; float qk_eps;
  float q_scale;
  unsigned long long* trace;
  const float* ln_stats; int ln_parts;
  const float* ln_c; const float* ln_d; int cd_stride, cd_rows, cd_eval_stride; float ln_eps;
  bf16* xs_out; int ld_xs; const float* next_scale; float* stats_out;
  float* row_mean;
  int pp_ngroup;
  F5ePrefetch pf;
  unsigned pf_per_wg;
};

static_assert(offsetof(GemmArgs, n_main) + sizeof(int) == 64, "hot kernarg fields must fill exactly the first 64-byte line");

__host__ __device__ inline unsigned div_magic_of(int d) {
  const unsigned long long m = 0x100000000ull / (unsigned long long)(d > 0 ? d : 1);
  return m > 0xFFFFFFFFull ? 0xFFFFFFFFu : (unsigned)m;
}
__device__ __forceinline__ int div_magic(int n, int d, unsigned magic) {
  unsigned q = __umulhi((unsigned)n, magic);
  if ((unsigned)n - q * (unsigned)d >= (unsigned)d) ++q;
  return (int)q;
}

enum { EPI_BF16 = 0, EPI_BF16_GELU = 1, EPI_GATE_RES = 2, EPI_QKV_ROPE = 3, EPI_F32 = 4 };

#pragma clang diagnostic push
#pragma clang diagnostic ignored "-Winline-asm"
__device__ __forceinline__ void glds16_s(const void* sbase, unsigned voff, void* lds) {
  const unsigned l = (unsigned)(unsigned long long)(__attribute__((address_space(3))) void*)lds;
  asm volatile("s_mov_b32 m0, %2\n\ts_nop 0\n\tglobal_load_lds_dwordx4 %0, %1" ::"v"(voff), "s"(sbase), "s"(l) : "memory", "m0");
}
#pragma clang diagnostic pop

__device__ __forceinline__ void glds16(const void* g, void* lds) {
  __builtin_amdgcn_global_load_lds((const __attribute__((address_space(1))) void*)g,
                                   (__attribute__((address_space(3))) void*)lds, 16, 0, 0);
}


int launch_pp(int epi, GemmArgs& a, hipStream_t st);
inline bool uses_pp(int M, int K) { return K >= 128 && (M + 255) / 256 >= 44; }

}
```

### f5e-tts_amd/csrc/runtime.hip

```cpp
#include <stdarg.h>
#include <stdio.h>
#include <string.h>
#include <cstdlib>

#include "f5e_common.h"
#include "gemm_bf16_args.h"

static thread_local char g_err[512] = "";

void f5e_set_error(const char* fmt, ...) {
  va_list ap;
  va_start(ap, fmt);
  vsnprintf(g_err, sizeof(g_err), fmt, ap);
  va_end(ap);
}

#define HIP_TRY(call, what)                                                        \
  do {                                                                             \
    hipError_t e_ = (call);                                                        \
    if (e_ != hipSuccess) {                                                        \
      f5e_set_error("%s: %s", what, hipGetErrorString(e_));                        \
      return F5E_ERR_HIP;                                                          \
    }                                                                              \
  } while (0)
// ... 2 lines not shown
  do {                       \
    int r_ = (call);         \
    if (r_ != F5E_OK) return r_; \
  } while (0)

extern "C" {

int f5e_abi_version(void) { return F5E_ABI_VERSION; }
const char* f5e_last_error(void) { return g_err; }

int f5e_check_device(void) {
  int dev = 0;
  HIP_TRY(hipGetDevice(&dev), "hipGetDevice");
  hipDeviceProp_t prop;
  HIP_TRY(hipGetDeviceProperties(&prop, dev), "hipGetDeviceProperties");
  if (strncmp(prop.gcnArchName, "gfx950", 6) != 0) {
    f5e_set_error("libf5e_hip is built for gfx950 only; device %d is %s", dev, prop.gcnArchName);
    return F5E_ERR_UNSUPPORTED;
  }
  return F5E_OK;
}

int f5e_graph_begin(hipStream_t st) {
  HIP_TRY(hipStreamBeginCapture(st, hipStreamCaptureModeRelaxed), "hipStreamBeginCapture");
  return F5E_OK;
}

int f5e_graph_end(hipStream_t st, void** graph_exec_out) {
  F5E_REQUIRE(graph_exec_out, "graph_end: null output");
  hipGraph_t g = nullptr;
  HIP_TRY(hipStreamEndCapture(st, &g), "hipStreamEndCapture");
  hipGraphExec_t ex = nullptr;
  hipError_t e = hipGraphInstantiate(&ex, g, nullptr, nullptr, 0);
  (void)hipGraphDestroy(g);
  if (e != hipSuccess) {
    f5e_set_error("hipGraphInstantiate: %s", hipGetErrorString(e));
    return F5E_ERR_HIP;
  }
  *graph_exec_out = (void*)ex;
  return F5E_OK;
}

int f5e_graph_launch(void* graph_exec, hipStream_t st) {
  F5E_REQUIRE(graph_exec, "graph_launch: null graph");
  HIP_TRY(hipGraphLaunch((hipGraphExec_t)graph_exec, st), "hipGraphLaunch");
  return F5E_OK;
}

int f5e_graph_destroy(void* graph_exec) {
  if (graph_exec) HIP_TRY(hipGraphExecDestroy((hipGraphExec_t)graph_exec), "hipGraphExecDestroy");
  return F5E_OK;
}

int f5e_workspace_bytes(const f5e_dit_plan* p, f5e_dit_workspace* out) {
  F5E_REQUIRE(p && out, "workspace_bytes: null argument");
  F5E_REQUIRE(p->S > 0 && p->N > 0 && p->D > 0 && p->H > 0 && p->FF > 0 && p->mel > 0, "workspace_bytes: bad shape");
  const unsigned long long M = (unsigned long long)p->S * p->N, D = p->D, inner = (unsigned long long)p->H * 64;
  const unsigned long long n_pad = ((unsigned long long)p->N + 63) / 64 * 64;
  const unsigned long long qk = (unsigned long long)p->S * p->H * n_pad * 64 * 2;
  memset(out, 0, sizeof(*out));
  out->n_pad = (int)n_pad;
  unsigned long long* b = out->bytes;
  b[F5E_WS_H0] = M * D * 4;       b[F5E_WS_H0_BF16] = M * D * 2;  b[F5E_WS_C1] = M * D * 2;
  b[F5E_WS_X] = M * D * 4;        b[F5E_WS_HN] = M * D * 2;
  b[F5E_WS_Q] = qk;               b[F5E_WS_K] = qk;               b[F5E_WS_VT] = qk;
  b[F5E_WS_AO] = M * inner * 2;   b[F5E_WS_FF] = M * (unsigned long long)p->FF * 2;
  b[F5E_WS_PRED] = M * (unsigned long long)p->mel * 4;
  b[F5E_WS_LN_STATS] = p->fuse_ln ? M * (D / 64) * 2 * 4 : 0;
  b[F5E_WS_LN_ROWMEAN] = p->fuse_ln ? M * 4 : 0;
  b[F5E_WS_SKIP_RES] = p->w_skip ? M * D * 4 : 0;
  b[F5E_WS_SKIP_TMP] = p->w_skip ? M * D * 4 : 0;
  unsigned long long off = 0;
  for (int i = 0; i < F5E_WS_COUNT; ++i) {
    out->offset[i] = off;
    off += (b[i] + 255) / 256 * 256;
  }
  out->total = off;
  return F5E_OK;
}

struct F5eTimer {
  int capacity, count;
  hipEvent_t* start;
  hipEvent_t* stop;
  int* op;
};

int f5e_timer_create(int capacity, void** timer_out) {
  F5E_REQUIRE(capacity > 0 && timer_out, "timer_create: bad arguments");
  F5eTimer* t = new F5eTimer{capacity, 0, new hipEvent_t[capacity], new hipEvent_t[capacity], new int[capacity]};
  for (int i = 0; i < capacity; ++i) {
    HIP_TRY(hipEventCreate(&t->start[i]), "hipEventCreate");
    HIP_TRY(hipEventCreate(&t->stop[i]), "hipEventCreate");
  }
  *timer_out = t;
  return F5E_OK;
}

int f5e_timer_destroy(void* timer) {
  if (!timer) return F5E_OK;
  F5eTimer* t = (F5eTimer*)timer;
  for (int i = 0; i < t->capacity; ++i) {
    (void)hipEventDestroy(t->start[i]);
    (void)hipEventDestroy(t->stop[i]);
  }
  delete[] t->start;
  delete[] t->stop;
  delete[] t->op;
  delete t;
  return F5E_OK;
}

int f5e_timer_reset(void* timer) {
  F5E_REQUIRE(timer, "timer_reset: null");
  ((F5eTimer*)timer)->count = 0;
  return F5E_OK;
}

int f5e_timer_read(void* timer, float* ms_out_host, int max_out, int* count_out_host) {
  F5E_REQUIRE(timer && ms_out_host && count_out_host, "timer_read: null");
  F5eTimer* t = (F5eTimer*)timer;
  const int n = t->count < max_out ? t->count : max_out;
  for (int i = 0; i < n; ++i) {
    HIP_TRY(hipEventSynchronize(t->stop[i]), "hipEventSynchronize");
    HIP_TRY(hipEventElapsedTime(&ms_out_host[i], t->start[i], t->stop[i]), "hipEventElapsedTime");
  }
  *count_out_host = n;
  return F5E_OK;
}

int f5e_timer_read_ops(void* timer, int* ops_out_host, int max_out, int* count_out_host) {
  F5E_REQUIRE(timer && ops_out_host && count_out_host, "timer_read_ops: null");
  F5eTimer* t = (F5eTimer*)timer;
  const int n = t->count < max_out ? t->count : max_out;
  for (int i = 0; i < n; ++i) ops_out_host[i] = t->op[i];
  *count_out_host = n;
  return F5E_OK;
}

#define F5E_TIMED(opclass, call)                                                  \
  do {                                                                            \
    const bool sel_ = p->timer_op >= 0 ? p->timer_op == (opclass) : (((-p->timer_op) >> (opclass)) & 1) != 0; \
    F5eTimer* tm_ = (p->timer && sel_) ? (F5eTimer*)p->timer : nullptr;          \
    const bool on_ = tm_ && tm_->count < tm_->capacity;                           \
    if (on_) HIP_TRY(hipEventRecord(tm_->start[tm_->count], st), "hipEventRecord"); \
    F5E_TRY(call);                                                                \
    if (on_) {                                                                    \
      HIP_TRY(hipEventRecord(tm_->stop[tm_->count], st), "hipEventRecord");       \
      tm_->op[tm_->count] = (opclass);                                            \
      tm_->count++;                                                               \
    }                                                                             \
  } while (0)

int f5e_dit_forward(hipStream_t st, const f5e_dit_plan* p) {
  F5E_REQUIRE(p, "dit_forward: null plan");
  F5E_REQUIRE(p->S > 0 && p->B > 0 && p->S % p->B == 0 && p->N > 0 && p->L > 0, "dit_forward: bad S/B/N/L");
  F5E_REQUIRE(p->D % 256 == 0 && p->H > 0 && p->FF % 64 == 0 && p->mel % 4 == 0, "dit_forward: unsupported dims");
  F5E_REQUIRE(p->y && p->w_x && p->in_const && p->rope_cs && p->mod && p->blocks && p->w_proj, "dit_forward: null input");
  F5E_REQUIRE(p->h0 && p->h0_bf16 && p->c1 && p->x && p->hn && p->q && p->k && p->vt && p->ao && p->ff && p->pred,
              "dit_forward: null workspace");
  const int M = p->S * p->N, D = p->D, inner = p->H * 64;
  const int row_stride = p->L * 6 * D + 2 * D;
  const int eval_stride = p->mod_rows * row_stride;

  F5E_TIMED(F5E_OP_INPROJ, f5e_gemm_f32(st, p->y, p->mel, p->B * p->N, F5E_ACT_NONE, p->w_x, p->ldw_x, nullptr, F5E_ACT_NONE, nullptr,
                       p->in_const, D, M, nullptr, p->h0, D, p->h0_bf16, D, M, D, p->mel));
  F5E_TIMED(F5E_OP_CONVPOS, f5e_convpos(st, p->h0_bf16, D, p->convpos_w1, p->convpos_b1, 0, p->c1, D, nullptr, 0, nullptr, 0, p->S, p->N, D, p->convpos_groups));
  F5E_TIMED(F5E_OP_CONVPOS, f5e_convpos(st, p->c1, D, p->convpos_w2, p->convpos_b2, 1, nullptr, 0, p->x, D, p->h0, D, p->S, p->N, D, p->convpos_groups));

  if (p->w_skip) {
    F5E_REQUIRE(p->skip_res && p->skip_tmp, "dit_forward: long skip needs skip_res / skip_tmp");
    HIP_TRY(hipMemcpyAsync(p->skip_res, p->x, (size_t)M * D * sizeof(float), hipMemcpyDeviceToDevice, st),
            "hipMemcpyAsync(skip_res)");
  }
  if (p->fuse_ln) {
    F5E_REQUIRE(!p->w_skip, "dit_forward: fused AdaLN does not cover the long skip connection");
    F5E_REQUIRE(p->ln_stats && p->ln_rowmean && p->cd && D % 256 == 0 && D <= 1024 && p->mod_rows == 1 && inner == D && p->cd_stride % 4 == 0,
                "dit_forward: fused AdaLN needs ln_stats, ln_rowmean, cd tables, D %% 256 == 0, D <= 1024, one modulation row and heads * 64 == D");
    const int parts = D / 64, ls = 6 * inner + 2 * p->FF, cd_eval_stride = p->mod_rows * p->cd_stride;
    F5E_REQUIRE(p->cd_stride >= p->L * ls + 2 * p->mel, "dit_forward: cd_stride too small");
    f5e_ln_fuse cons{}, prod{};
    cons.stats = p->ln_stats; cons.parts = parts; cons.cd_stride = p->cd_stride; cons.cd_rows = p->mod_rows;
    cons.cd_eval_stride = cd_eval_stride; cons.eval_ptr = p->eval_ptr; cons.rows_per_seq = p->N; cons.eps = 1e-6f;
    prod.xs_out = p->hn; prod.ld_xs = D; prod.stats_out = p->ln_stats;
    cons.row_mean = prod.row_mean = p->ln_rowmean;
    F5E_TIMED(F5E_OP_LN, f5e_adaln_pre(st, p->x, D, p->hn, D, p->mod + D, row_stride, p->mod_rows, p->N, p->eval_ptr, eval_stride,
                                       p->ln_stats, parts, p->ln_rowmean, M, D));
    const bool pfon = p->mall_prefetch != 0;
    const unsigned b_out = (unsigned)((size_t)D * inner * 2), b_ff = (unsigned)((size_t)p->FF * D * 2);
    const unsigned b_qkv = (unsigned)((size_t)3 * inner * D * 2);
    for (int l = 0; l < p->L; ++l) {
      const f5e_dit_block_weights& w = p->blocks[l];
      F5E_REQUIRE(!w.q_norm_w, "dit_forward: fused AdaLN and qk_norm are exclusive");
      const float* mb = p->mod + (size_t)l * 6 * D;
      const float* cdl = p->cd + (size_t)l * ls;
      const F5ePrefetch pf_next{{l + 1 < p->L ? p->blocks[l + 1].w_qkv : p->w_proj, nullptr},
                                {l + 1 < p->L ? b_qkv : (unsigned)((size_t)p->mel * D * 2), 0}};
      F5ePrefetch pf_qkv{{w.w_out, nullptr}, {b_out, 0}};
      F5ePrefetch pf_attn{{w.w_ff1, nullptr}, {b_ff, 0}};
      F5ePrefetch pf_out{{w.w_ff2, nullptr}, {b_ff, 0}};
      F5ePrefetch pf_nx = pf_next, pf_ff1{};
      {
        int scheme = 0;
#ifdef F5E_TOOLS
        static const int scheme_env = getenv("F5E_PF_SCHEME") ? atoi(getenv("F5E_PF_SCHEME")) : -1;
        if (scheme_env >= 0) scheme = scheme_env;
#endif
        const void* wout_next = l + 1 < p->L ? (const void*)p->blocks[l + 1].w_out : nullptr;
        if (scheme == 1 || scheme == 3) {
          pf_attn = F5ePrefetch{{w.w_ff1, w.w_ff2}, {b_ff, b_ff}};
          pf_out = F5ePrefetch{};
        }
        if (scheme == 2 || scheme == 3) {
          pf_nx = F5ePrefetch{{pf_next.ptr[0], wout_next}, {pf_next.bytes[0], wout_next ? b_out : 0}};
          if (l > 0) pf_qkv = F5ePrefetch{};
        }
#ifdef F5E_TOOLS
        if (scheme == 5 || scheme == 6) {
          pf_qkv = F5ePrefetch{{w.w_out, w.w_ff1}, {b_out, b_ff}};
          pf_attn = F5ePrefetch{};
          if (scheme == 6) { pf_out = F5ePrefetch{}; pf_ff1 = F5ePrefetch{{w.w_ff2, nullptr}, {b_ff, 0}}; }
        }
        if (scheme == 7) {
          pf_attn = F5ePrefetch{};
          pf_out = F5ePrefetch{{w.w_ff1, nullptr}, {b_ff, 0}};
          pf_ff1 = F5ePrefetch{{w.w_ff2, nullptr}, {b_ff, 0}};
        }
        if (scheme == 4) {
          pf_attn = F5ePrefetch{{w.w_ff1, pf_next.ptr[0]}, {b_ff, pf_next.bytes[0]}};
          pf_nx = F5ePrefetch{};
        }
#endif
      }
      cons.c = cdl; cons.d = cdl + 3 * inner;
      F5E_TIMED(F5E_OP_QKV, f5e_gemm_bf16_qkv_rope_pf(st, p->hn, D, w.w_qkv, D, nullptr, p->q, p->k, p->vt, p->n_pad, p->H,
                                        p->rope_heads, p->rope_cs, nullptr, nullptr, p->N, M, D, 0, &cons, pfon ? &pf_qkv : nullptr));
      F5E_TIMED(F5E_OP_ATTN, f5e_flash_attn_pf(st, p->q, p->k, p->vt, p->ao, inner, p->seq_len, p->S, p->H, p->N, p->n_pad, 0,
                                               pfon ? &pf_attn : nullptr));
      prod.next_scale = mb + 4 * D;
      F5E_TIMED(F5E_OP_OUT, f5e_gemm_bf16_gate_residual_pf(st, p->ao, inner, w.w_out, inner, w.b_out, p->x, D, mb + 2 * D,
                                          row_stride, p->mod_rows, p->eval_ptr, eval_stride, p->N, p->seq_len, M, D,
                                          inner, 0, &prod, pfon ? &pf_out : nullptr));
      cons.c = cdl + 6 * inner; cons.d = cdl + 6 * inner + p->FF;
      F5E_TIMED(F5E_OP_FF1, f5e_gemm_bf16_bias_pf(st, p->hn, D, w.w_ff1, D, nullptr, p->ff, p->FF, M, p->FF, D,
                                    F5E_ACT_GELU_TANH, 0, 0, &cons, pfon && pf_ff1.ptr[0] ? &pf_ff1 : nullptr));
      prod.next_scale = (l + 1 < p->L) ? mb + 6 * D + D : p->mod + (size_t)p->L * 6 * D;
      F5E_TIMED(F5E_OP_FF2, f5e_gemm_bf16_gate_residual_pf(st, p->ff, p->FF, w.w_ff2, p->FF, w.b_ff2, p->x, D, mb + 5 * D,
                                          row_stride, p->mod_rows, p->eval_ptr, eval_stride, p->N, nullptr, M, D, p->FF,
                                          0, &prod, pfon ? &pf_nx : nullptr));
    }
    cons.c = p->cd + (size_t)p->L * ls; cons.d = cons.c + p->mel;
    F5E_TIMED(F5E_OP_FINAL, f5e_gemm_bf16_bias_ln(st, p->hn, D, p->w_proj, D, nullptr, p->pred, p->mel, M, p->mel, D,
                                    F5E_ACT_NONE, 1, 0, &cons));
    return F5E_OK;
  }
  for (int l = 0; l < p->L; ++l) {
    const f5e_dit_block_weights& w = p->blocks[l];
    const float* mb = p->mod + (size_t)l * 6 * D;
    F5E_TIMED(F5E_OP_LN, f5e_layernorm(st, p->x, D, p->hn, D, 1, nullptr, nullptr, mb + D, mb, row_stride, p->mod_rows, p->N,
                          p->eval_ptr, eval_stride, M, D, 1e-6f));
    F5E_TIMED(F5E_OP_QKV, f5e_gemm_bf16_qkv_rope(st, p->hn, D, w.w_qkv, D, w.b_qkv, p->q, p->k, p->vt, p->n_pad, p->H, p->rope_heads,
                                   p->rope_cs, w.q_norm_w, w.k_norm_w, p->N, M, D, 0));
    F5E_TIMED(F5E_OP_ATTN, f5e_flash_attn(st, p->q, p->k, p->vt, p->ao, inner, p->seq_len, p->S, p->H, p->N, p->n_pad, 0));
    F5E_TIMED(F5E_OP_OUT, f5e_gemm_bf16_gate_residual(st, p->ao, inner, w.w_out, inner, w.b_out, p->x, D, mb + 2 * D, row_stride,
                                        p->mod_rows, p->eval_ptr, eval_stride, p->N, p->seq_len, M, D, inner, 0));
    F5E_TIMED(F5E_OP_LN, f5e_layernorm(st, p->x, D, p->hn, D, 1, nullptr, nullptr, mb + 4 * D, mb + 3 * D, row_stride, p->mod_rows,
                          p->N, p->eval_ptr, eval_stride, M, D, 1e-6f));
    F5E_TIMED(F5E_OP_FF1, f5e_gemm_bf16_bias(st, p->hn, D, w.w_ff1, D, w.b_ff1, p->ff, p->FF, M, p->FF, D, F5E_ACT_GELU_TANH, 0, 0));
    F5E_TIMED(F5E_OP_FF2, f5e_gemm_bf16_gate_residual(st, p->ff, p->FF, w.w_ff2, p->FF, w.b_ff2, p->x, D, mb + 5 * D, row_stride,
                                        p->mod_rows, p->eval_ptr, eval_stride, p->N, nullptr, M, D, p->FF, 0));
  }
  if (p->w_skip) {
    F5E_TRY(f5e_gemm_f32(st, p->x, D, M, F5E_ACT_NONE, p->w_skip, 2 * D, nullptr, F5E_ACT_NONE, nullptr, nullptr, 0, 0,
                         nullptr, p->skip_tmp, D, nullptr, 0, M, D, D));
    F5E_TRY(f5e_gemm_f32(st, p->skip_res, D, M, F5E_ACT_NONE, p->w_skip + D, 2 * D, nullptr, F5E_ACT_NONE, nullptr,
                         p->skip_tmp, D, M, nullptr, p->x, D, nullptr, 0, M, D, D));
  }
  const float* mf = p->mod + (size_t)p->L * 6 * D;
  F5E_TIMED(F5E_OP_LN, f5e_layernorm(st, p->x, D, p->hn, D, 1, nullptr, nullptr, mf, mf + D, row_stride, p->mod_rows, p->N,
                        p->eval_ptr, eval_stride, M, D, 1e-6f));
  F5E_TIMED(F5E_OP_FINAL, f5e_gemm_bf16_bias(st, p->hn, D, p->w_proj, D, p->b_proj, p->pred, p->mel, M, p->mel, D, F5E_ACT_NONE, 1, 0));
  return F5E_OK;
}

int f5e_sample_loop(hipStream_t st, const f5e_loop_plan* lp) {
  F5E_REQUIRE(lp && lp->eval_a, "sample_loop: null plan");
  F5E_REQUIRE(lp->steps > 0 && lp->n > 0 && lp->y && lp->pred && lp->coef && lp->eval_ptr && lp->done_ctr,
              "sample_loop: steps, n, y, pred, coef, eval_ptr and done_ctr are required");
  F5E_REQUIRE(lp->eval_a->eval_ptr == lp->eval_ptr && lp->eval_a->y == lp->y,
              "sample_loop: eval_a must read the loop's state y and evaluation counter");
  const bool midpoint = lp->eval_b != nullptr;
  if (midpoint)
    F5E_REQUIRE(lp->y_mid && lp->eval_b->y == lp->y_mid && lp->eval_b->eval_ptr == lp->eval_ptr,
                "sample_loop: eval_b must read y_mid and the loop's evaluation counter");
  const long long ts = lp->traj ? lp->n : 0;
  for (int i = 0; i < lp->steps; ++i) {
    F5E_TRY(f5e_dit_forward(st, lp->eval_a));
    if (!midpoint) {
      F5E_TRY(f5e_ode_update_traj(st, lp->pred, lp->n, lp->mode, lp->w0, lp->w1, lp->y, lp->y, lp->traj, ts, 1, lp->coef,
                                  lp->eval_ptr, lp->done_ctr, lp->n));
    } else {
      F5E_TRY(f5e_ode_update_traj(st, lp->pred, lp->n, lp->mode, lp->w0, lp->w1, lp->y, lp->y_mid, nullptr, 0, 1, lp->coef,
                                  lp->eval_ptr, lp->done_ctr, lp->n));
      F5E_TRY(f5e_dit_forward(st, lp->eval_b));
      F5E_TRY(f5e_ode_update_traj(st, lp->pred, lp->n, lp->mode, lp->w0, lp->w1, lp->y, lp->y, lp->traj, ts, 2, lp->coef,
                                  lp->eval_ptr, lp->done_ctr, lp->n));
    }
  }
  return F5E_OK;
}

}
```

### f5e-tts_amd/ops.py

```python
from __future__ import annotations

import ctypes as C
import threading
from typing import Optional

import torch

from . import _C
from ._C import ACT_GELU_ERF, ACT_GELU_TANH, ACT_MISH, ACT_NONE, ACT_RELU, ACT_SILU, check, lib

Tensor = torch.Tensor
_checked_device = False


def _stream() -> int:
    return torch.cuda.current_stream().cuda_stream


def require_device() -> None:
    global _checked_device
    if not _checked_device:
        if not torch.cuda.is_available():
            raise _C.F5EError("f5e_tts_amd needs a ROCm GPU (gfx950); torch.cuda.is_available() is False and there "
                              "is no CPU fallback")
# ... 64 lines not shown
    return out


def gemm_bf16_gate_residual(a: Tensor, w: Tensor, bias: Optional[Tensor], resid: Tensor, gate: Tensor,
                            rows_per_seq: int, seq_len: Optional[Tensor] = None, eval_ptr: Optional[Tensor] = None,
                            eval_stride: int = 0, tile_hint: int = 0, ln=None):
    require_device()
    M, K = a.shape
    N = w.shape[0]
    check(lib().f5e_gemm_bf16_gate_residual_ln(
        _stream(), _p(a, BF, "a"), a.stride(0), _p(w, BF, "w"), w.stride(0), _p(bias, F32, "bias"),
        _p(resid, F32, "resid"), resid.stride(0), C.c_void_p(gate.data_ptr()), gate.stride(0), gate.shape[0],
        _p(eval_ptr, I32, "eval_ptr"), eval_stride, rows_per_seq, _p(seq_len, I32, "seq_len"), M, N, K, tile_hint,
        _ln_ref(ln)), "f5e_gemm_bf16_gate_residual")
    return resid


def gemm_bf16_qkv_rope(a: Tensor, w: Tensor, bias: Tensor, q: Tensor, k: Tensor, vt: Tensor, heads: int,
                       rope_heads: int, cos_sin: Tensor, rows_per_seq: int, tile_hint: int = 0,
                       q_norm_w: Optional[Tensor] = None, k_norm_w: Optional[Tensor] = None, ln=None):
    require_device()
    M, K = a.shape
    n_pad = q.shape[2]
    check(lib().f5e_gemm_bf16_qkv_rope_ln(
        _stream(), _p(a, BF, "a"), a.stride(0), _p(w, BF, "w"), w.stride(0), _p(bias, F32, "bias"), _p(q, BF, "q"),
        _p(k, BF, "k"), _p(vt, BF, "vt"), n_pad, heads, rope_heads, _p(cos_sin, F32, "cos_sin"),
        _p(q_norm_w, F32, "q_norm_w"), _p(k_norm_w, F32, "k_norm_w"), rows_per_seq, M, K, tile_hint, _ln_ref(ln)),
        "f5e_gemm_bf16_qkv_rope")


def qk_frag_index(n_pad: int) -> Tensor:
    pos = torch.arange(n_pad)[:, None]
    d = torch.arange(64)[None, :]
    return (((pos // 32) * 4 + d // 16) * 32 + pos % 32) * 16 + ((d // 8) % 2) * 8 + d % 8


def v_frag_index(n_pad: int) -> Tensor:
    key = torch.arange(n_pad)[:, None]
    d = torch.arange(64)[None, :]
    k16 = key % 16
    j = (k16 // 8) * 4 + k16 % 4
    h = (k16 // 4) % 2
    return (((((key // 32) * 2 + (key % 32) // 16) * 2 + d // 32) * 32 + d % 32) * 2 + h) * 8 + j


def flash_attn(q: Tensor, k: Tensor, vt: Tensor, out: Tensor, rows_per_seq: int, kv_len: Optional[Tensor] = None,
               waves: int = 0):
    require_device()
    S, H, n_pad, _ = q.shape
    check(lib().f5e_flash_attn(_stream(), _p(q, BF, "q"), _p(k, BF, "k"), _p(vt, BF, "vt"), _p(out, BF, "out"),
                               out.stride(0), _p(kv_len, I32, "kv_len"), S, H, rows_per_seq, n_pad, waves),
          "f5e_flash_attn")
    return out


def joint_attn(qx: Tensor, kx: Tensor, vtx: Tensor, qc: Optional[Tensor], kc: Tensor, vtc: Tensor, out_x: Tensor,
               out_c: Optional[Tensor], N: int, Nt: int, kv_len: Optional[Tensor] = None, waves: int = 0):
    require_device()
    S, H, n_pad_x, _ = qx.shape
    n_pad_c = kc.shape[2]
    if kx.shape != qx.shape or vtx.numel() != qx.numel() or kc.shape[:2] != (S, H) or vtc.numel() != kc.numel():
        raise _C.F5EError("joint_attn: audio buffers [S, H, n_pad_x, 64], text buffers [S, H, n_pad_c, 64]")
    if out_c is not None and (qc is None or qc.shape != kc.shape):
        raise _C.F5EError("joint_attn: out_c needs qc of kc's shape")
    if out_x.shape[0] != S * N or (out_c is not None and out_c.shape[0] != S * Nt):
        raise _C.F5EError(f"joint_attn: out_x must have S*N = {S * N} rows and out_c S*Nt = {S * Nt}")
    if kv_len is not None and kv_len.numel() < S:
        raise _C.F5EError(f"joint_attn: kv_len needs one entry per sequence ({S})")
    check(lib().f5e_joint_attn(_stream(), _p(qx, BF, "qx"), _p(kx, BF, "kx"), _p(vtx, BF, "vtx"), _p(qc, BF, "qc"),
                               _p(kc, BF, "kc"), _p(vtc, BF, "vtc"), _p(out_x, BF, "out_x"), out_x.stride(0),
                               _p(out_c, BF, "out_c"), out_c.stride(0) if out_c is not None else 0,
                               _p(kv_len, I32, "kv_len"), S, H, N, n_pad_x, Nt, n_pad_c, waves), "f5e_joint_attn")
    return out_x, out_c


def layernorm(x: Tensor, out: Tensor, gamma: Optional[Tensor] = None, beta: Optional[Tensor] = None,
              scale: Optional[Tensor] = None, shift: Optional[Tensor] = None, rows_per_seq: int = 1,
              eval_ptr: Optional[Tensor] = None, eval_stride: int = 0, eps: float = 1e-6):
    require_device()
    rows, D = x.shape
    mod_rows = scale.shape[0] if scale is not None else 0
    mod_stride = scale.stride(0) if scale is not None else 0
    if scale is not None and shift.stride(0) != mod_stride:
        raise _C.F5EError("scale and shift must share a row stride")
    sp = C.c_void_p(scale.data_ptr()) if scale is not None else None
    hp = C.c_void_p(shift.data_ptr()) if shift is not None else None
    check(lib().f5e_layernorm(_stream(), _p(x, F32, "x"), x.stride(0), _p(out, None, "out"), out.stride(0),
                              1 if out.dtype == BF else 0, _p(gamma, F32, "gamma"), _p(beta, F32, "beta"), sp, hp,
                              mod_stride, mod_rows, rows_per_seq, _p(eval_ptr, I32, "eval_ptr"), eval_stride, rows, D,
                              eps), "f5e_layernorm")
    return out


def l2norm(x: Tensor, out: Tensor, g: Tensor):
    require_device()
    rows, D = x.shape
    check(lib().f5e_l2norm(_stream(), _p(x, F32, "x"), x.stride(0), _p(out, None, "out"), out.stride(0),
                           1 if out.dtype == BF else 0, _p(g, F32, "g"), rows, D), "f5e_l2norm")
    return out


def grn(x: Tensor, out: Tensor, gamma: Tensor, beta: Tensor, ws: Tensor):
    require_device()
    B, T, Cc = x.shape
    check(lib().f5e_grn(_stream(), _p(x, F32, "x"), _p(out, F32, "out"), _p(ws, F32, "ws"), _p(gamma, F32, "gamma"),
                        _p(beta, F32, "beta"), B, T, Cc), "f5e_grn")
    return out


def gemm_f32(a: Tensor, w: Tensor, bias: Optional[Tensor] = None, *, out: Optional[Tensor] = None,
             out_bf16: Optional[Tensor] = None, M: Optional[int] = None, a_act: int = ACT_NONE, act: int = ACT_NONE,
             ch_scale: Optional[Tensor] = None, addend: Optional[Tensor] = None, row_scale: Optional[Tensor] = None,
             K: Optional[int] = None):
    require_device()
    a_rows = a.shape[0]
    K = a.shape[1] if K is None else K
    N = w.shape[0]
    M = a_rows if M is None else M
    for t, nm in ((a, "a"), (w, "w")):
        if not t.is_cuda or t.dtype != F32 or t.stride(1) != 1:
            raise _C.F5EError(f"gemm_f32: {nm} must be an f32 GPU tensor with unit column stride")
    ad = addend
    check(lib().f5e_gemm_f32(
        _stream(), C.c_void_p(a.data_ptr()), a.stride(0), a_rows, a_act, C.c_void_p(w.data_ptr()), w.stride(0),
        _p(bias, F32, "bias"), act, _p(ch_scale, F32, "ch_scale"),
        C.c_void_p(ad.data_ptr()) if ad is not None else None, ad.stride(0) if ad is not None else 0,
        ad.shape[0] if ad is not None else 0, _p(row_scale, F32, "row_scale"),
        C.c_void_p(out.data_ptr()) if out is not None else None, out.stride(0) if out is not None else 0,
        C.c_void_p(out_bf16.data_ptr()) if out_bf16 is not None else None,
        out_bf16.stride(0) if out_bf16 is not None else 0, M, N, K), "f5e_gemm_f32")
    return out if out is not None else out_bf16


def pack_convpos_weight(w: Tensor, groups: int = 16) -> Tensor:
    D, cpg, taps = w.shape
    out = torch.zeros(groups, taps, 64, 64, dtype=w.dtype, device=w.device)
    out[:, :, :cpg, :cpg] = w.view(groups, cpg, cpg, taps).permute(0, 3, 1, 2)
    return out.to(BF).contiguous()


def convpos(x: Tensor, w_packed: Tensor, bias: Tensor, S: int, N: int, *, out_bf16: Optional[Tensor] = None,
            out_f32: Optional[Tensor] = None, resid: Optional[Tensor] = None):
    require_device()
    D = x.shape[1]
    mode = 0 if out_f32 is None else 1
    check(lib().f5e_convpos(_stream(), _p(x, BF, "x"), x.stride(0), _p(w_packed, BF, "w_packed"), _p(bias, F32, "bias"),
                            mode, _p(out_bf16, BF, "out_bf16"), out_bf16.stride(0) if out_bf16 is not None else 0,
                            _p(out_f32, F32, "out_f32"), out_f32.stride(0) if out_f32 is not None else 0,
                            _p(resid, F32, "resid"), resid.stride(0) if resid is not None else 0, S, N, D,
                            w_packed.shape[0]),
          "f5e_convpos")


def dwconv7(x: Tensor, w_t: Tensor, bias: Tensor, out: Tensor):
    require_device()
    B, T, Cc = x.shape
    check(lib().f5e_dwconv7(_stream(), _p(x, F32, "x"), _p(w_t, F32, "w_t"), _p(bias, F32, "bias"), _p(out, F32, "out"),
                            B, T, Cc), "f5e_dwconv7")
    return out


def im2col(x: Tensor, col: Tensor, ksize: int, pad: int):
    require_device()
    B, T, Cin = x.shape
    check(lib().f5e_im2col(_stream(), _p(x, F32, "x"), _p(col, F32, "col"), B, T, Cin, ksize, pad), "f5e_im2col")
    return col


def sinus_embed(t: Tensor, freqs: Tensor, out: Tensor, scale: float = 1000.0):
    require_device()
    E, dim = out.shape
    check(lib().f5e_sinus_embed(_stream(), _p(t, F32, "t"), _p(freqs, F32, "freqs"), _p(out, F32, "out"), E, dim, scale),
          "f5e_sinus_embed")
    return out


def rope_table(inv_freq: Tensor, out: Tensor):
    require_device()
    N, half, _ = out.shape
    check(lib().f5e_rope_table(_stream(), _p(inv_freq, F32, "inv_freq"), _p(out, F32, "out"), N, half), "f5e_rope_table")
    return out


def text_gather(ids: Tensor, table: Tensor, pos: Optional[Tensor], keep: Optional[Tensor], out: Tensor):
    require_device()
    B, N, TD = out.shape
    check(lib().f5e_text_gather(_stream(), _p(ids, I32, "ids"), _p(table, F32, "table"), _p(pos, F32, "pos"),
                                _p(keep, F32, "keep"), _p(out, F32, "out"), B, N, TD,
                                pos.shape[0] if pos is not None else 1, table.shape[0]), "f5e_text_gather")
    return out


def ode_update(pred: Tensor, branch_stride: int, mode: int, w0: float, w1: float, base: Tensor, dst: Tensor,
               coef: Tensor, eval_ptr: Optional[Tensor], traj: Optional[Tensor] = None,
               done_ctr: Optional[Tensor] = None, traj_stride: int = 0, traj_div: int = 1):
    require_device()
    check(lib().f5e_ode_update_traj(_stream(), _p(pred, F32, "pred"), branch_stride, mode, w0, w1, _p(base, F32, "base"),
                                    _p(dst, F32, "dst"), C.c_void_p(traj.data_ptr()) if traj is not None else None,
                                    traj_stride, traj_div, _p(coef, F32, "coef"), _p(eval_ptr, I32, "eval_ptr"),
                                    _p(done_ctr, I32, "done_ctr"), base.numel()), "f5e_ode_update")
    return dst


def sample_loop(loop: "_C.LoopPlan"):
    require_device()
    check(lib().f5e_sample_loop(_stream(), C.byref(loop)), "f5e_sample_loop")


def advance_eval(eval_ptr: Tensor):
    require_device()
    check(lib().f5e_advance_eval(_stream(), _p(eval_ptr, I32, "eval_ptr")), "f5e_advance_eval")


def stitch(cond: Tensor, y: Tensor, mask_u8: Tensor, out: Tensor):
    require_device()
    Cc = cond.shape[-1]
    check(lib().f5e_stitch(_stream(), _p(cond, F32, "cond"), _p(y, F32, "y"), _p(mask_u8, U8, "mask"),
                           _p(out, F32, "out"), cond.numel() // Cc, Cc), "f5e_stitch")
    return out


def cast_bf16(x: Tensor, out: Tensor):
    require_device()
    check(lib().f5e_cast_bf16(_stream(), _p(x, F32, "x"), _p(out, BF, "out"), x.numel()), "f5e_cast_bf16")
    return out


def cast_f32(x: Tensor, out: Tensor):
    require_device()
    check(lib().f5e_cast_f32(_stream(), _p(x, BF, "x"), _p(out, F32, "out"), x.numel()), "f5e_cast_f32")
    return out


def axpby(x: Tensor, y: Optional[Tensor], out: Tensor, a: float = 1.0, b: float = 1.0, c: float = 0.0):
    require_device()
    if y is not None and y.numel() != x.numel() or out.numel() != x.numel():
        raise _C.F5EError("axpby: size mismatch")
    check(lib().f5e_axpby(_stream(), _p(x, F32, "x"), _p(y, F32, "y"), _p(out, F32, "out"), a, b, c, x.numel()),
          "f5e_axpby")
    return out


def vq_eval(logits: Tensor, vars_: Tensor, combine_groups: bool, out: Tensor, targets: Tensor,
            stats: Optional[Tensor], groups: int, num_vars: int):
    require_device()
    rows = logits.shape[0]
    check(lib().f5e_vq_eval(_stream(), _p(logits, F32, "logits"), logits.stride(0), _p(vars_, F32, "vars"),
                            1 if combine_groups else 0, _p(out, F32, "out"), _p(targets, I32, "targets"),
                            _p(stats, F32, "stats"), rows, groups, num_vars, vars_.shape[-1]), "f5e_vq_eval")
    return out


def mas_workspace_bytes(B: int, Ty: int, Tx: int) -> int:
    n = C.c_ulonglong()
    check(lib().f5e_mas_workspace_bytes(B, Ty, Tx, C.byref(n)), "f5e_mas_workspace_bytes")
    return int(n.value)


def mas_path(logp: Tensor, t_y: Tensor, t_x: Tensor, token_of_frame: Tensor, durations: Optional[Tensor] = None,
             workspace: Optional[Tensor] = None):
    require_device()
    if logp.ndim != 3 or not logp.is_cuda or logp.dtype != F32 or logp.stride(2) != 1:
        raise _C.F5EError("mas_path: logp must be an f32 GPU tensor [B, Ty, Tx] with unit column stride; there is no "
                          "CPU path")
    B, Ty, Tx = logp.shape
    if t_y.numel() != B or t_x.numel() != B or token_of_frame.shape != (B, Ty) or \
            (durations is not None and durations.shape != (B, Tx)):
        raise _C.F5EError(f"mas_path: lengths [{B}], token_of_frame [{B}, {Ty}], durations [{B}, {Tx}]")
    need = mas_workspace_bytes(B, Ty, Tx)
    if workspace is None:
        workspace = torch.empty((need + 7) // 8, dtype=torch.int64, device=logp.device)
    nbytes = workspace.numel() * workspace.element_size()
    check(lib().f5e_mas_path(_stream(), C.c_void_p(logp.data_ptr()), logp.stride(0), logp.stride(1), _p(t_y, I32, "t_y"),
                             _p(t_x, I32, "t_x"), _p(token_of_frame, I32, "token_of_frame"),
                             _p(durations, I32, "durations"), _p(workspace, None, "workspace"), nbytes, B, Ty, Tx),
          "f5e_mas_path")
    return token_of_frame, durations


def stft_logmel(wav: Tensor, window: Tensor, twiddle: Tensor, fb: Tensor, out: Tensor, n_fft: int, hop: int):
    require_device()
    B, nw = wav.shape
    check(lib().f5e_stft_logmel(_stream(), _p(wav, F32, "wav"), nw, wav.stride(0), _p(window, F32, "window"),
                                _p(twiddle, F32, "twiddle"), _p(fb, F32, "fb"), _p(out, F32, "out"), B, n_fft, hop,
                                fb.shape[1]), "f5e_stft_logmel")
    return out


def band_filterbank(fb: Tensor):
    h = fb.detach().to("cpu", F32)
    nz = h != 0
    bands, chunks, off = [], [], 0
    for m in range(h.shape[1]):
        idx = torch.nonzero(nz[:, m]).flatten()
        if idx.numel() == 0:
            bands.append((0, 0, off))
            continue
        lo, hi = int(idx[0]), int(idx[-1])
        bands.append((lo, hi - lo + 1, off))
        chunks.append(h[lo:hi + 1, m])
        off += hi - lo + 1
    if off == 0 or off > 2048:
        return None
    return torch.cat(chunks).contiguous().to(fb.device), torch.tensor(bands, dtype=I32).contiguous().to(fb.device)


def stft_logmel_banded(wav: Tensor, window: Tensor, twiddle: Tensor, fb_compact: Tensor, fb_band: Tensor, out: Tensor,
                       n_fft: int, hop: int):
    require_device()
    B, nw = wav.shape
    check(lib().f5e_stft_logmel_banded(_stream(), _p(wav, F32, "wav"), nw, wav.stride(0), _p(window, F32, "window"),
                                       _p(twiddle, F32, "twiddle"), _p(fb_compact, F32, "fb_compact"),
                                       _p(fb_band, I32, "fb_band"), fb_compact.numel(), _p(out, F32, "out"), B, n_fft, hop,
                                       fb_band.shape[0]), "f5e_stft_logmel_banded")
    return out


def stft_logmel_banded_ex(wav: Tensor, window: Tensor, twiddle: Tensor, fb_compact: Tensor, fb_band: Tensor, out: Tensor,
                          n_fft: int, hop: int, pad_left: int, mag_eps: float):
    require_device()
    B, nw = wav.shape
    T = out.shape[1]
    if out.shape != (B, T, fb_band.shape[0]):
        raise _C.F5EError(f"out must be [B, T, n_mels] = [{B}, T, {fb_band.shape[0]}] (got {tuple(out.shape)})")
    check(lib().f5e_stft_logmel_banded_ex(_stream(), _p(wav, F32, "wav"), nw, wav.stride(0), _p(window, F32, "window"),
                                          _p(twiddle, F32, "twiddle"), _p(fb_compact, F32, "fb_compact"),
                                          _p(fb_band, I32, "fb_band"), fb_compact.numel(), _p(out, F32, "out"), B, n_fft,
                                          hop, fb_band.shape[0], pad_left, T, mag_eps), "f5e_stft_logmel_banded_ex")
    return out


def istft_head(z: Tensor, window: Tensor, twiddle: Tensor, frames_ws: Tensor, out: Tensor, B: int, T: int, n_fft: int,
               hop: int):
    require_device()
    check(lib().f5e_istft_head(_stream(), _p(z, F32, "z"), z.stride(0), _p(window, F32, "window"),
                               _p(twiddle, F32, "twiddle"), _p(frames_ws, F32, "frames_ws"), _p(out, F32, "out"), B, T,
                               n_fft, hop), "f5e_istft_head")
    return out


def bigvgan_act(x: Tensor, out: Tensor, alpha: Tensor, inv_beta: Tensor, f_up: Tensor, f_dn: Tensor):
    require_device()
    B, L, C = x.shape
    if out.shape != x.shape or out.dtype not in (BF, F32):
        raise _C.F5EError("bigvgan_act: out must be bf16 or f32 of x's shape")
    if alpha.numel() != C or inv_beta.numel() != C or f_up.numel() != 12 or f_dn.numel() != 12:
        raise _C.F5EError("bigvgan_act: alpha / inv_beta [C], filters [12]")
    check(lib().f5e_bigvgan_act(_stream(), _p(x, F32, "x"), _p(out, None, "out"), 1 if out.dtype == F32 else 0,
                                _p(alpha, F32, "alpha"), _p(inv_beta, F32, "inv_beta"), _p(f_up, F32, "f_up"),
                                _p(f_dn, F32, "f_dn"), B, L, C), "f5e_bigvgan_act")
    return out


# ... 145 lines not shown
```

### include/f5e_abi.h

```cpp
#ifndef F5E_ABI_H_
#define F5E_ABI_H_

#ifdef __cplusplus
extern "C" {
#endif

#define F5E_ABI_VERSION 2

#if defined(__GNUC__)
#define F5E_API __attribute__((visibility("default")))
#else
#define F5E_API
#endif

enum { F5E_OK = 0, F5E_ERR_BAD_SHAPE = -1, F5E_ERR_UNSUPPORTED = -2, F5E_ERR_HIP = -3 };

enum { F5E_ACT_NONE = 0, F5E_ACT_SILU = 1, F5E_ACT_GELU_ERF = 2, F5E_ACT_GELU_TANH = 3, F5E_ACT_RELU = 4, F5E_ACT_MISH = 5 };

#ifdef F5E_STREAM_T
typedef F5E_STREAM_T f5e_stream;
#else
typedef void* f5e_stream;
#endif

F5E_API int f5e_abi_version(void);
F5E_API const char* f5e_last_error(void);
F5E_API int f5e_check_device(void);


F5E_API int f5e_gemm_bf16_bias(f5e_stream st, const void* A, int lda, const void* W, int ldw, const float* bias, void* out,
                       int ldo, int M, int N, int K, int act, int out_f32, int tile_hint);

F5E_API int f5e_gemm_bf16_gate_residual(f5e_stream st, const void* A, int lda, const void* W, int ldw, const float* bias,
                                float* resid, int ldr, const float* gate, int gate_stride, int gate_rows,
                                const int* eval_ptr, int eval_stride, int rows_per_seq, const int* seq_len, int M,
                                int N, int K, int tile_hint);

F5E_API int f5e_gemm_bf16_qkv_rope(f5e_stream st, const void* A, int lda, const void* W, int ldw, const float* bias, void* q,
                           void* k, void* vt, int n_pad, int heads, int rope_heads, const float* cos_sin,
                           const float* q_norm_w, const float* k_norm_w, int rows_per_seq, int M, int K,
                           int tile_hint);

typedef struct f5e_ln_fuse {
  const float* stats; int parts;
  const float* c; const float* d; int cd_stride; int cd_rows; int cd_eval_stride;
  const int* eval_ptr; int rows_per_seq; float eps;
  void* xs_out; int ld_xs; const float* next_scale;
  float* stats_out;
  float* row_mean;
} f5e_ln_fuse;

F5E_API int f5e_gemm_bf16_bias_ln(f5e_stream st, const void* A, int lda, const void* W, int ldw, const float* bias, void* out,
                          int ldo, int M, int N, int K, int act, int out_f32, int tile_hint, const f5e_ln_fuse* ln);
F5E_API int f5e_gemm_bf16_gate_residual_ln(f5e_stream st, const void* A, int lda, const void* W, int ldw, const float* bias,
                                   float* resid, int ldr, const float* gate, int gate_stride, int gate_rows,
                                   const int* eval_ptr, int eval_stride, int rows_per_seq, const int* seq_len, int M,
                                   int N, int K, int tile_hint, const f5e_ln_fuse* ln);
F5E_API int f5e_gemm_bf16_qkv_rope_ln(f5e_stream st, const void* A, int lda, const void* W, int ldw, const float* bias,
                              void* q, void* k, void* vt, int n_pad, int heads, int rope_heads, const float* cos_sin,
                              const float* q_norm_w, const float* k_norm_w, int rows_per_seq, int M, int K,
                              int tile_hint, const f5e_ln_fuse* ln);


F5E_API int f5e_flash_attn(f5e_stream st, const void* q, const void* k, const void* vt, void* o, int ldo, const int* kv_len,
                   int S, int H, int rows_per_seq, int n_pad, int splits);

F5E_API int f5e_joint_attn(f5e_stream st, const void* qx, const void* kx, const void* vx, const void* qc, const void* kc,
                   const void* vc, void* o_x, int ldo_x, void* o_c, int ldo_c, const int* kv_len, int S, int H, int N,
                   int n_pad_x, int Nt, int n_pad_c, int splits);


F5E_API int f5e_layernorm(f5e_stream st, const float* x, int ldx, void* y, int ldy, int y_bf16, const float* gamma,
                  const float* beta, const float* scale, const float* shift, int mod_stride, int mod_rows,
                  int rows_per_seq, const int* eval_ptr, int eval_stride, int rows, int D, float eps);

F5E_API int f5e_adaln_pre(f5e_stream st, const float* x, int ldx, void* xs, int ld_xs, const float* scale, int mod_stride,
                  int mod_rows, int rows_per_seq, const int* eval_ptr, int eval_stride, float* stats, int parts,
                  float* row_mean, int rows, int D);

F5E_API int f5e_l2norm(f5e_stream st, const float* x, int ldx, void* y, int ldy, int y_bf16, const float* g, int rows, int D);

F5E_API int f5e_grn(f5e_stream st, const float* x, float* y, float* gx_ws, const float* gamma, const float* beta, int B, int T,
            int C);


F5E_API int f5e_gemm_f32(f5e_stream st, const float* A, int lda, int a_rows, int a_act, const float* W, int ldw,
                 const float* bias, int act, const float* ch_scale, const float* addend, int ld_add, int add_rows,
                 const float* row_scale, float* out, int ldo, void* out_bf16, int ldo_bf16, int M, int N, int K);


F5E_API int f5e_convpos(f5e_stream st, const void* x, int ldx, const void* w_packed, const float* bias, int mode,
                void* out_bf16, int ldo, float* out_f32, int ldo32, const float* resid, int ldr, int S, int N, int D,
                int groups);

F5E_API int f5e_dwconv7(f5e_stream st, const float* x, const float* w_t, const float* bias, float* y, int B, int T, int C);

F5E_API int f5e_im2col(f5e_stream st, const float* x, float* col, int B, int T, int Cin, int ksize, int pad);


F5E_API int f5e_sinus_embed(f5e_stream st, const float* t, const float* freqs, float* out, int E, int dim, float scale);
F5E_API int f5e_rope_table(f5e_stream st, const float* inv_freq, float* out, int N, int half);
F5E_API int f5e_text_gather(f5e_stream st, const int* ids, const float* table, const float* pos, const float* keep, float* out,
                    int B, int N, int TD, int max_pos, int table_rows);
F5E_API int f5e_ode_update(f5e_stream st, const float* pred, long long branch_stride, int mode, float w0, float w1,
                   const float* base, float* dst, float* traj, const float* coef, int* eval_ptr, unsigned* done_ctr,
                   long long n);
F5E_API int f5e_ode_update_traj(f5e_stream st, const float* pred, long long branch_stride, int mode, float w0, float w1,
                        const float* base, float* dst, float* traj, long long traj_stride, int traj_div,
                        const float* coef, int* eval_ptr, unsigned* done_ctr, long long n);
F5E_API int f5e_advance_eval(f5e_stream st, int* eval_ptr);
F5E_API int f5e_stitch(f5e_stream st, const float* cond, const float* y, const unsigned char* mask, float* out, long long rows,
               int C);
F5E_API int f5e_cast_bf16(f5e_stream st, const float* x, void* y, long long n);
F5E_API int f5e_cast_f32(f5e_stream st, const void* x, float* y, long long n);
F5E_API int f5e_axpby(f5e_stream st, const float* x, const float* y, float* out, float a, float b, float c, long long n);
F5E_API int f5e_vq_eval(f5e_stream st, const float* logits, int ld, const float* vars, int combine_groups, float* out,
                int* targets, float* stats, int rows, int groups, int num_vars, int var_dim);

F5E_API int f5e_mas_workspace_bytes(int B, int Ty, int Tx, unsigned long long* bytes_out_host);
F5E_API int f5e_mas_path(f5e_stream st, const float* logp, long long batch_stride, int ld, const int* t_y, const int* t_x,
                 int* token_of_frame, int* durations, void* workspace, unsigned long long workspace_bytes, int B, int Ty,
                 int Tx);


F5E_API int f5e_stft_logmel(f5e_stream st, const float* wav, int nw, int ldw, const float* window, const float* twiddle,
                    const float* fb, float* out, int B, int n_fft, int hop, int n_mels);
F5E_API int f5e_stft_logmel_banded(f5e_stream st, const float* wav, int nw, int ldw, const float* window, const float* twiddle,
                           const float* fb_compact, const int* fb_band, int nnz, float* out, int B, int n_fft, int hop,
                           int n_mels);
F5E_API int f5e_stft_logmel_banded_ex(f5e_stream st, const float* wav, int nw, int ldw, const float* window,
                              const float* twiddle, const float* fb_compact, const int* fb_band, int nnz, float* out, int B,
                              int n_fft, int hop, int n_mels, int pad_left, int T, float mag_eps);
F5E_API int f5e_istft_head(f5e_stream st, const float* z, int ldz, const float* window, const float* twiddle, float* frames_ws,
                   float* out, int B, int T, int n_fft, int hop);


F5E_API int f5e_bigvgan_act(f5e_stream st, const float* x, void* y, int out_f32, const float* alpha, const float* inv_beta,
                    const float* f_up, const float* f_dn, int B, int L, int C);
F5E_API int f5e_bigvgan_conv(f5e_stream st, const void* x, const void* w_packed, const float* bias, const float* resid,
                     float* out, float* sum, float sum_scale, int sum_init, int B, int L, int Cin, int Cin_pad, int N,
                     int ksz, int dil, int pad);
F5E_API int f5e_bigvgan_post(f5e_stream st, const float* a, const float* w, const float* bias, float* out, int B, int L, int C,
                     int ksz, int use_tanh);


F5E_API int f5e_kaldi_fbank(f5e_stream st, const float* wav, int nw, int ldw, const float* window, const float* twiddle,
                    const float* fb, float* out, int B, int win, int shift, int n_mels, float in_scale, float preemph,
                    float eps);
F5E_API int f5e_glu(f5e_stream st, const float* x, int ldx, float* y, int ldy, long long rows, int C);
F5E_API int f5e_dwconv(f5e_stream st, const float* x, const float* w_t, const float* bias, const float* keep, float* y, int B,
               int T, int C, int K);
F5E_API int f5e_softmax_rows(f5e_stream st, const float* x, int ldx, float* y, int ldy, const int* kv_len, long long rows,
                     int rows_per_seq, int L, float scale);
F5E_API int f5e_dwconv_stream(f5e_stream st, const float* x, const float* w_t, const float* bias, const float* fill, float* y,
                      int B, int T, int C, int K, int causal, int chunk);
F5E_API int f5e_relpos_attn(f5e_stream st, const float* qu, int ldq, const float* k, int ldk, const float* pos, int ldp,
                    const float* v, int ldv, float* out, int ldo, const int* kv_len, int B, int T, int H, int dk,
                    int q_begin, int chunk, int left_chunks, float scale);


typedef struct f5e_dit_block_weights {
  const void* w_qkv;  const float* b_qkv;
  const void* w_out;  const float* b_out;
  const void* w_ff1;  const float* b_ff1;
  const void* w_ff2;  const float* b_ff2;
  const float* q_norm_w; const float* k_norm_w;
} f5e_dit_block_weights;

typedef struct f5e_dit_plan {
  int S, B, N, n_pad, D, H, rope_heads, FF, L, mel;
  int mod_rows;
  const float* y;
  const float* w_x; int ldw_x;
  const float* in_const;
  const void* convpos_w1; const float* convpos_b1;
  const void* convpos_w2; const float* convpos_b2;
  int convpos_groups;
  const float* rope_cs;
  const int* seq_len;
  const float* mod;
  const int* eval_ptr;
  const f5e_dit_block_weights* blocks;
  const void* w_proj; const float* b_proj;
  const float* w_skip;
  float* skip_res; float* skip_tmp;
  float* h0; void* h0_bf16; void* c1;
  float* x;
  void* hn;
  void* q; void* k; void* vt;
  void* ao;
  void* ff;
  float* pred;
  void* timer;
  int timer_op;
  int fuse_ln;
  float* ln_stats;
  float* ln_rowmean;
  const float* cd;
  int cd_stride;
  int mall_prefetch;
} f5e_dit_plan;

enum { F5E_WS_H0 = 0, F5E_WS_H0_BF16, F5E_WS_C1, F5E_WS_X, F5E_WS_HN, F5E_WS_Q, F5E_WS_K, F5E_WS_VT, F5E_WS_AO, F5E_WS_FF,
       F5E_WS_PRED, F5E_WS_LN_STATS, F5E_WS_SKIP_RES, F5E_WS_SKIP_TMP, F5E_WS_LN_ROWMEAN, F5E_WS_COUNT };
typedef struct f5e_dit_workspace {
  int n_pad;
  unsigned long long bytes[F5E_WS_COUNT];
  unsigned long long offset[F5E_WS_COUNT];
  unsigned long long total;
} f5e_dit_workspace;
F5E_API int f5e_workspace_bytes(const f5e_dit_plan* shape, f5e_dit_workspace* out_host);

enum { F5E_OP_NONE = 0, F5E_OP_INPROJ = 1, F5E_OP_CONVPOS = 2, F5E_OP_LN = 3, F5E_OP_QKV = 4, F5E_OP_ATTN = 5,
       F5E_OP_OUT = 6, F5E_OP_FF1 = 7, F5E_OP_FF2 = 8, F5E_OP_FINAL = 9 };

F5E_API int f5e_timer_create(int capacity, void** timer_out);
F5E_API int f5e_timer_destroy(void* timer);
F5E_API int f5e_timer_reset(void* timer);
F5E_API int f5e_timer_read(void* timer, float* ms_out_host, int max_out, int* count_out_host);
F5E_API int f5e_timer_read_ops(void* timer, int* ops_out_host, int max_out, int* count_out_host);

#ifdef F5E_TOOLS
F5E_API void f5e_debug_convpos_trace(void* buf);
#endif

F5E_API int f5e_dit_forward(f5e_stream st, const f5e_dit_plan* plan);

typedef struct f5e_loop_plan {
  const f5e_dit_plan* eval_a;
  const f5e_dit_plan* eval_b;
  int steps;
  int mode; float w0, w1;
  long long n;
  float* y;
  float* y_mid;
  const float* pred;
  const float* coef;
  int* eval_ptr;
  unsigned* done_ctr;
  float* traj;
} f5e_loop_plan;
F5E_API int f5e_sample_loop(f5e_stream st, const f5e_loop_plan* loop);

F5E_API int f5e_graph_begin(f5e_stream st);
F5E_API int f5e_graph_end(f5e_stream st, void** graph_exec_out);
F5E_API int f5e_graph_launch(void* graph_exec, f5e_stream st);
F5E_API int f5e_graph_destroy(void* graph_exec);

#ifdef __cplusplus
}
#endif
#endif
```

Before: 12960 mel-frames/s.

## Fuse the two conv-position convs and fold the ODE update into the final GEMM

Adds a single-kernel convpos pair that computes both grouped convolutions per tile, keeping the Mish intermediate in LDS instead of writing and rereading it through global memory. It applies only when the grid fits in one workgroup per CU and otherwise falls back to two launches. Adds a final-projection GEMM epilogue that pairs the cond and uncond rows per tile and applies the CFG Euler update directly, which removes the separate ODE update kernel on each step. This makes the GEMM epilogue and tile mapping more complex and narrows the conditions under which the fused path is used.

```diff
diff --git a/f5e-tts_amd/_C.py b/f5e-tts_amd/_C.py
--- a/f5e-tts_amd/_C.py
+++ b/f5e-tts_amd/_C.py
@@ -22,6 +22,7 @@
     "f5e_gemm_bf16_bias_ln": [_P, _P, _I, _P, _I, _P, _P, _I, _I, _I, _I, _I, _I, _I, _P],
     "f5e_gemm_bf16_gate_residual_ln": [_P, _P, _I, _P, _I, _P, _P, _I, _P, _I, _I, _P, _I, _I, _P, _I, _I, _I, _I, _P],
     "f5e_gemm_bf16_qkv_rope_ln": [_P, _P, _I, _P, _I, _P, _P, _P, _P, _I, _I, _I, _P, _P, _P, _I, _I, _I, _I, _P],
+    "f5e_gemm_bf16_final_ode": [_P, _P, _I, _P, _I, _P, _I, _I, _I, _P, _P],
     "f5e_adaln_pre": [_P, _P, _I, _P, _I, _P, _I, _I, _I, _P, _I, _P, _I, _P, _I, _I],
     "f5e_flash_attn": [_P, _P, _P, _P, _P, _I, _P, _I, _I, _I, _I, _I],
     "f5e_joint_attn": [_P, _P, _P, _P, _P, _P, _P, _P, _I, _P, _I, _P, _I, _I, _I, _I, _I, _I, _I],
@@ -30,6 +31,7 @@
     "f5e_l2norm": [_P, _P, _I, _P, _I, _I, _P, _I, _I],
     "f5e_gemm_f32": [_P, _P, _I, _I, _I, _P, _I, _P, _I, _P, _P, _I, _I, _P, _P, _I, _P, _I, _I, _I, _I],
     "f5e_convpos": [_P, _P, _I, _P, _P, _I, _P, _I, _P, _I, _P, _I, _I, _I, _I, _I],
+    "f5e_convpos_pair": [_P, _P, _I, _P, _P, _P, _P, _P, _I, _P, _I, _P, _I, _I, _I, _I, _I],
     "f5e_dwconv7": [_P, _P, _P, _P, _P, _I, _I, _I],
     "f5e_im2col": [_P, _P, _P, _I, _I, _I, _I, _I],
     "f5e_sinus_embed": [_P, _P, _P, _P, _I, _I, _F],
@@ -83,6 +85,11 @@
     _fields_ = [("stats", _P), ("parts", _I), ("c", _P), ("d", _P), ("cd_stride", _I), ("cd_rows", _I),
                 ("cd_eval_stride", _I), ("eval_ptr", _P), ("rows_per_seq", _I), ("eps", _F),
                 ("xs_out", _P), ("ld_xs", _I), ("next_scale", _P), ("stats_out", _P), ("row_mean", _P)]
+
+
+class OdeFuse(C.Structure):
+    _fields_ = [("mode", _I), ("w0", _F), ("base", _P), ("dst", _P), ("traj", _P), ("traj_stride", _LL), ("traj_div", _I),
+                ("coef", _P), ("eval_ptr", _P), ("done_ctr", _P)]
 
 
 class DitPlan(C.Structure):
diff --git a/f5e-tts_amd/csrc/conv.hip b/f5e-tts_amd/csrc/conv.hip
--- a/f5e-tts_amd/csrc/conv.hip
+++ b/f5e-tts_amd/csrc/conv.hip
@@ -328,6 +328,183 @@
       unsigned long long* o = a.trace + ((size_t)(blockIdx.z * gridDim.y + blockIdx.y) * gridDim.x + blockIdx.x) * 8;
 #pragma unroll
       for (int i = 0; i < 8; ++i) o[i] = ts[i];
+    }
+  }
+}
+
+struct ConvPairArgs {
+  const bf16* x; int ldx;
+  const bf16* w1; const bf16* w2;
+  const float* bias1; const float* bias2;
+  float* out; int ldo;
+  const float* resid; int ldr;
+  int S, N, D, cpg;
+};
+
+template <int NJ, bool ACT_BARRIER>
+__device__ __forceinline__ void convpos_tap_loop(const char* Xs, const bf16* wg, char* ring, int wave, int lane,
+                                                 f32x4 (&acc)[4][NJ]) {
+  constexpr int W_BYTES = 8192, NST = 4, TAPS = 31;
+  const int fr = lane & 15, fq = lane >> 4;
+  const bf16* w_src[8];
+#pragma unroll
+  for (int j = 0; j < 8; ++j) {
+    const int i = lane + 64 * j;
+    const int row = i >> 3, c = (i & 7) ^ ((row >> 1) & 7);
+    w_src[j] = wg + row * 64 + c * 8;
+  }
+  auto stage_w = [&](int slot, int u) {
+    int tap = wave + 4 * u;
+    tap = tap < TAPS ? tap : TAPS - 1;
+#pragma unroll
+    for (int j = 0; j < 8; ++j) glds16c(w_src[j] + (size_t)tap * 4096, ring + slot * W_BYTES + j * 1024);
+  };
+#pragma unroll
+  for (int u = 0; u < NST - 1; ++u) stage_w(u, u);
+#pragma unroll
+  for (int i = 0; i < 4; ++i)
+#pragma unroll
+    for (int j = 0; j < NJ; ++j) acc[i][j] = f32x4{0.f, 0.f, 0.f, 0.f};
+
+#pragma unroll
+  for (int u = 0; u < 8; ++u) {
+    const int issued = u + NST - 1 < 8 ? u + NST - 1 : 8;
+    const int pend = 8 * (issued - u - 1);
+    if (pend == 16) asm volatile("s_waitcnt vmcnt(16) lgkmcnt(0)" ::: "memory");
+    else if (pend == 8) asm volatile("s_waitcnt vmcnt(8) lgkmcnt(0)" ::: "memory");
+    else asm volatile("s_waitcnt vmcnt(0) lgkmcnt(0)" ::: "memory");
+    if (ACT_BARRIER && u == 0) __builtin_amdgcn_s_barrier();
+    const int tap = wave + 4 * u;
+    const bool live = !(u == 7 && tap >= TAPS);
+    const char* Ws = ring + (u % NST) * W_BYTES;
+    bf16x8 xf[NJ], wf[4];
+    auto reads = [&](int kk) {
+      const int c = kk * 4 + fq;
+#pragma unroll
+      for (int j = 0; j < NJ; ++j) {
+        const int row = j * 16 + fr + tap;
+        xf[j] = *(const bf16x8*)(Xs + row * 128 + ((c ^ ((row >> 1) & 7)) << 4));
+      }
+#pragma unroll
+      for (int i = 0; i < 4; ++i) {
+        const int row = i * 16 + fr;
+        wf[i] = *(const bf16x8*)(Ws + row * 128 + ((c ^ ((row >> 1) & 7)) << 4));
+      }
+    };
+    auto mfmas = [&]() {
+#pragma unroll
+      for (int i = 0; i < 4; ++i)
+#pragma unroll
+        for (int j = 0; j < NJ; ++j)
+          acc[i][j] = __builtin_amdgcn_mfma_f32_16x16x32_bf16(wf[i], xf[j], acc[i][j], 0, 0, 0);
+    };
+    if (live) reads(0);
+    if (u + NST - 1 < 8) stage_w((u + NST - 1) % NST, u + NST - 1);
+    if (!live) break;
+    mfmas();
+    reads(1);
+    mfmas();
+  }
+}
+
+__global__ __launch_bounds__(256) void convpos_pair_kernel(ConvPairArgs a) {
+  constexpr int BT = 64, HALO = 15, MR = 96;
+  constexpr int X_ROWS = 128, X_USED = MR + 2 * HALO;
+  constexpr int X_BYTES = X_ROWS * 128, M_BYTES = MR * 128, W_BYTES = 8192, NST = 4;
+  constexpr int TAPS = 31, RS = 68;
+  extern __shared__ __attribute__((aligned(16))) char smem[];
+  char* Xs = smem;
+  char* Ms = smem + X_BYTES;
+  char* ring_base = smem + X_BYTES + M_BYTES;
+  float* Red = (float*)ring_base;
+  static_assert(4 * MR * RS * 4 <= 4 * NST * W_BYTES, "conv 1's partial sums must fit the ring space");
+
+  const int tid = threadIdx.x, lane = tid & 63;
+  const int wave = __builtin_amdgcn_readfirstlane(tid >> 6);
+  const int g = blockIdx.x, tt = blockIdx.y, seq = blockIdx.z;
+  const int c0 = g * a.cpg;
+  const int t0 = tt * BT;
+  const int fr = lane & 15, fq = lane >> 4;
+
+  const int oc = (lane & 15) * 4;
+  const int n = c0 + (oc < a.cpg ? oc : 0);
+  f32x4 rv[4];
+#pragma unroll
+  for (int p = 0; p < 4; ++p) {
+    const int t = t0 + wave * 16 + p * 4 + (lane >> 4);
+    rv[p] = *(const f32x4*)(a.resid + ((size_t)seq * a.N + (t < a.N ? t : a.N - 1)) * a.ldr + n);
+  }
+  const f32x4 bias1 = *(const f32x4*)(a.bias1 + n);
+  const f32x4 bias2 = *(const f32x4*)(a.bias2 + n);
+  asm volatile("" ::: "memory");
+  __builtin_amdgcn_sched_barrier(0);
+#pragma unroll
+  for (int r = 0; r < 4; ++r) {
+    const int i = tid + 256 * r;
+    const int row = i >> 3, c = (i & 7) ^ ((row >> 1) & 7);
+    const int t = t0 - 2 * HALO + row;
+    const void* src = &conv_zero16;
+    if (row < X_USED && t >= 0 && t < a.N && c0 + c * 8 < a.D) src = a.x + ((size_t)seq * a.N + t) * a.ldx + c0 + c * 8;
+    glds16c(src, Xs + (wave * 64 + 256 * r) * 16);
+  }
+  asm volatile("" ::: "memory");
+  __builtin_amdgcn_sched_barrier(0);
+
+  char* ring = ring_base + wave * (NST * W_BYTES);
+  {
+    f32x4 acc[4][6];
+    convpos_tap_loop<6, true>(Xs, a.w1 + (size_t)g * TAPS * 4096, ring, wave, lane, acc);
+    asm volatile("s_waitcnt vmcnt(0) lgkmcnt(0)" ::: "memory");
+    __builtin_amdgcn_s_barrier();
+    float* mine = Red + wave * (MR * RS);
+#pragma unroll
+    for (int i = 0; i < 4; ++i)
+#pragma unroll
+      for (int j = 0; j < 6; ++j) *(f32x4*)(mine + (j * 16 + fr) * RS + i * 16 + fq * 4) = acc[i][j];
+    asm volatile("s_waitcnt lgkmcnt(0)" ::: "memory");
+    __builtin_amdgcn_s_barrier();
+#pragma unroll
+    for (int p = 0; p < 6; ++p) {
+      const int row = wave * 24 + p * 4 + (lane >> 4);
+      const int t = t0 - HALO + row;
+      const float* rp = Red + row * RS + oc;
+      f32x4 v = (*(const f32x4*)rp + *(const f32x4*)(rp + MR * RS)) + (*(const f32x4*)(rp + 2 * MR * RS) + *(const f32x4*)(rp + 3 * MR * RS));
+      v += bias1;
+      v[0] = mish_f(v[0]); v[1] = mish_f(v[1]); v[2] = mish_f(v[2]); v[3] = mish_f(v[3]);
+      if (t < 0 || t >= a.N || oc >= a.cpg) v = f32x4{0.f, 0.f, 0.f, 0.f};
+      *(bf16x4*)(Ms + row * 128 + (((oc >> 3) ^ ((row >> 1) & 7)) << 4) + (oc & 4) * 2) = f2bf4(v[0], v[1], v[2], v[3]);
+    }
+    asm volatile("s_waitcnt lgkmcnt(0)" ::: "memory");
+    __builtin_amdgcn_s_barrier();
+  }
+
+  f32x4 acc[4][4];
+  convpos_tap_loop<4, false>(Ms, a.w2 + (size_t)g * TAPS * 4096, ring, wave, lane, acc);
+  asm volatile("s_waitcnt vmcnt(0) lgkmcnt(0)" ::: "memory");
+  __builtin_amdgcn_s_barrier();
+  float* mine = Red + wave * (64 * RS);
+#pragma unroll
+  for (int i = 0; i < 4; ++i)
+#pragma unroll
+    for (int j = 0; j < 4; ++j) *(f32x4*)(mine + (j * 16 + fr) * RS + i * 16 + fq * 4) = acc[i][j];
+  asm volatile("s_waitcnt lgkmcnt(0)" ::: "memory");
+  __builtin_amdgcn_s_barrier();
+#pragma unroll
+  for (int p = 0; p < 4; ++p) asm volatile("" : "+v"(rv[p]));
+
+  if (oc < a.cpg) {
+#pragma unroll
+    for (int p = 0; p < 4; ++p) {
+      const int row = wave * 16 + p * 4 + (lane >> 4);
+      const int t = t0 + row;
+      const size_t m = (size_t)seq * a.N + t;
+      const float* rp = Red + row * RS + oc;
+      f32x4 v = (*(const f32x4*)rp + *(const f32x4*)(rp + 64 * RS)) + (*(const f32x4*)(rp + 2 * 64 * RS) + *(const f32x4*)(rp + 3 * 64 * RS));
+      v += bias2;
+      v[0] = mish_f(v[0]); v[1] = mish_f(v[1]); v[2] = mish_f(v[2]); v[3] = mish_f(v[3]);
+      if (t >= a.N) continue;
+      v += rv[p];
+      *(f32x4*)(a.out + m * a.ldo + n) = v;
     }
   }
 }
@@ -443,6 +620,33 @@
   return convpos_launch(st, x, ldx, w_packed, bias, mode, out_bf16, ldo, out_f32, ldo32, resid, ldr, S, N, D, groups);
 }
 
+int f5e_convpos_pair(hipStream_t st, const void* x, int ldx, const void* w1_packed, const float* bias1,
+                     const void* w2_packed, const float* bias2, void* mid_bf16, int ldm, float* out_f32, int ldo32,
+                     const float* resid, int ldr, int S, int N, int D, int groups) {
+  F5E_REQUIRE(x && w1_packed && bias1 && w2_packed && bias2 && out_f32 && resid, "convpos_pair: null operand");
+  F5E_REQUIRE(S > 0 && N > 0 && D > 0 && groups > 0 && D % groups == 0, "convpos_pair: bad D=%d / groups=%d", D, groups);
+  const int cpg = D / groups, tiles_t = (N + 63) / 64;
+  const bool fused = cpg % 16 == 0 && cpg <= 64 && tiles_t <= 65535 && S <= 65535 &&
+                     (size_t)groups * tiles_t * S <= (size_t)f5e_cu_count();
+  if (!fused) {
+    F5E_REQUIRE(mid_bf16, "convpos_pair: a grid of more than one workgroup per CU needs the mid_bf16 buffer");
+    if (int e = convpos_launch(st, x, ldx, w1_packed, bias1, 0, mid_bf16, ldm, nullptr, 0, nullptr, 0, S, N, D, groups)) return e;
+    return convpos_launch(st, mid_bf16, ldm, w2_packed, bias2, 1, nullptr, 0, out_f32, ldo32, resid, ldr, S, N, D, groups);
+  }
+  F5E_REQUIRE(ldx % 8 == 0 && ldo32 % 4 == 0 && ldr % 4 == 0, "convpos_pair: ldx must be a multiple of 8, ldo32 and ldr of 4");
+  ConvPairArgs a{};
+  a.x = (const bf16*)x; a.ldx = ldx; a.w1 = (const bf16*)w1_packed; a.w2 = (const bf16*)w2_packed;
+  a.bias1 = bias1; a.bias2 = bias2; a.out = out_f32; a.ldo = ldo32; a.resid = resid; a.ldr = ldr;
+  a.S = S; a.N = N; a.D = D; a.cpg = cpg;
+  constexpr int lds = 128 * 128 + 96 * 128 + 4 * 4 * 8192;
+  static_assert(lds <= 160 * 1024, "LDS budget");
+  static F5eDeviceOnce once;
+  F5E_OPT_IN_LDS(once, convpos_pair_kernel, lds);
+  hipLaunchKernelGGL(convpos_pair_kernel, dim3(groups, tiles_t, S), dim3(256), lds, st, a);
+  F5E_LAUNCH_CHECK("convpos_pair");
+  return F5E_OK;
+}
+
 int f5e_dwconv7(hipStream_t st, const float* x, const float* w_t, const float* bias, float* y, int B, int T, int C) {
   F5E_REQUIRE(x && w_t && bias && y, "dwconv7: null operand");
   F5E_REQUIRE(B > 0 && T > 0 && C > 0 && C % 4 == 0, "dwconv7: C=%d must be a positive multiple of 4", C);
diff --git a/f5e-tts_amd/csrc/elementwise.hip b/f5e-tts_amd/csrc/elementwise.hip
--- a/f5e-tts_amd/csrc/elementwise.hip
+++ b/f5e-tts_amd/csrc/elementwise.hip
@@ -54,14 +54,17 @@
   if (traj && traj_stride) traj += (size_t)((e + 1) / traj_div) * traj_stride;
   for (size_t i = (size_t)blockIdx.x * 256 + threadIdx.x; i < n; i += (size_t)gridDim.x * 256) {
     const float p0 = pred[i];
-    float v = p0;
+    float y;
     if (mode == 1) {
-      v = p0 + (p0 - pred[i + branch_stride]) * w0;
-    } else if (mode == 2) {
-      const float p1 = pred[i + branch_stride], p2 = pred[i + 2 * branch_stride];
-      v = w0 * (p2 - p1) + w1 * (p1 - p0) + p0;
-    }
-    const float y = base[i] + h * v;
+      y = f5e_cfg_step(p0, pred[i + branch_stride], w0, base[i], h);
+    } else {
+      float v = p0;
+      if (mode == 2) {
+        const float p1 = pred[i + branch_stride], p2 = pred[i + 2 * branch_stride];
+        v = w0 * (p2 - p1) + w1 * (p1 - p0) + p0;
+      }
+      y = base[i] + h * v;
+    }
     dst[i] = y;
     if (traj) traj[i] = y;
   }
diff --git a/f5e-tts_amd/csrc/f5e_common.h b/f5e-tts_amd/csrc/f5e_common.h
--- a/f5e-tts_amd/csrc/f5e_common.h
+++ b/f5e-tts_amd/csrc/f5e_common.h
@@ -130,6 +130,11 @@
   return *(const __attribute__((address_space(4))) int*)(uintptr_t)p;
 }
 
+__device__ __forceinline__ float f5e_cfg_step(float p0, float p1, float w0, float base, float h) {
+  const float v = p0 + (p0 - p1) * w0;
+  return base + h * v;
+}
+
 __device__ __forceinline__ bf16x4 f2bf4(float a, float b, float c, float d) {
   f32x4 v = {a, b, c, d};
   return __builtin_convertvector(v, bf16x4);
diff --git a/f5e-tts_amd/csrc/gemm_bf16.hip b/f5e-tts_amd/csrc/gemm_bf16.hip
--- a/f5e-tts_amd/csrc/gemm_bf16.hip
+++ b/f5e-tts_amd/csrc/gemm_bf16.hip
@@ -41,6 +41,9 @@
   constexpr int STAGE = A_BYTES + W_BYTES;
   constexpr int WM = BM / WGM, WN = BN / WGN;
   constexpr int TM = WM / 16, TN = WN / 16;
+  constexpr bool CONS = FUSE == 1 || FUSE == 3;
+  constexpr bool ODE = FUSE == 3;
+  static_assert(!ODE || (EPI == EPI_F32 && NLOAD == 0 && BM == 64 && WM == 32), "ODE epilogue: the classic 64-row f32 consumer");
   extern __shared__ __attribute__((aligned(16))) char smem[];
 
   const int lane = threadIdx.x & 63;
@@ -55,12 +58,15 @@
     if (tid == 0) { trc[0] = __builtin_amdgcn_s_memrealtime(); trc[1] = __builtin_amdgcn_s_memtime(); }
   }
 
-  if (FUSE == 1)
+  if (CONS)
     asm volatile("" ::"s"(a.ln_stats), "s"(a.ln_c), "s"(a.ln_d), "s"(a.ln_parts), "s"(a.cd_stride), "s"(a.cd_rows),
                  "s"(a.cd_eval_stride), "s"(a.eval_ptr));
   if (EPI == EPI_GATE_RES)
     asm volatile("" ::"s"(a.resid), "s"(a.gate), "s"(a.seq_len), "s"(a.eval_ptr), "s"(a.ldr), "s"(a.gate_stride),
                  "s"(a.gate_rows), "s"(a.eval_stride), "s"(a.bias));
+  if (ODE)
+    asm volatile("" ::"s"(a.ode_base), "s"(a.ode_dst), "s"(a.ode_traj), "s"(a.ode_coef), "s"(a.ode_eval), "s"(a.ode_done),
+                 "s"(a.ode_mode), "s"(a.ode_half));
   if (FUSE == 2) asm volatile("" ::"s"(a.next_scale), "s"(a.xs_out), "s"(a.stats_out), "s"(a.ld_xs), "s"(a.row_mean));
   if (EPI == EPI_QKV_ROPE) asm volatile("" ::"s"(a.q), "s"(a.k), "s"(a.vt), "s"(a.cos_sin), "s"(a.n_pad), "s"(a.heads), "s"(a.rope_heads));
 
@@ -87,7 +93,10 @@
     tile_m = r >> sh;
     tile_n = (g << sh) + (r & ((1 << sh) - 1));
   }
-  const int m0 = tile_m * BM, n0 = tile_n * BN;
+  const bool pair = ODE && a.ode_mode == 1;
+  const int m0 = tile_m * (pair ? BM / 2 : BM), n0 = tile_n * BN;
+  auto grow = [&](int r) { return pair ? m0 + (r & 31) + (r >> 5) * a.ode_half : m0 + r; };
+  auto glast = [&](int r) { return pair ? (r >> 5) * a.ode_half + a.ode_half - 1 : a.M - 1; };
 
   constexpr int A_IT = BM * CPR / NT;
   constexpr int W_IT = BN * CPR / NT;
@@ -97,7 +106,8 @@
   for (int j = 0; j < A_IT; ++j) {
     const int i = (stid & (NT - 1)) + NT * j;
     const int row = i / CPR, c = (i % CPR) ^ swz(row);
-    a_off[j] = (unsigned)(min(m0 + row, a.M - 1) - m0) * (unsigned)(a.lda * 2) + (unsigned)c * 16u;
+    const int mrow = ODE ? min(grow(row), glast(row)) : min(m0 + row, a.M - 1);
+    a_off[j] = (unsigned)(mrow - m0) * (unsigned)(a.lda * 2) + (unsigned)c * 16u;
   }
 #pragma unroll
   for (int j = 0; j < W_IT; ++j) {
@@ -153,7 +163,7 @@
           nbuf_l = (nbuf_l + 1 == NSTAGE) ? 0 : nbuf_l + 1;
         }
       }
-      if (FUSE == 1) __syncthreads();
+      if (CONS) __syncthreads();
       if (FUSE == 2) __builtin_amdgcn_s_barrier();
       return;
     }
@@ -163,19 +173,21 @@
   constexpr bool PREF = (TM * TN <= 4);
   static_assert(FUSE != 2 || (PREF && WM == 32 && WN == 32 && BN == 64 && (BM == 64 || (BM == 128 && NLOAD > 0))),
                 "fused AdaLN producer: 64 (or, role split, 128) x 64 tiles of 32 x 32 wave sub-tiles");
-  static_assert(FUSE != 1 || (WN == 32 && (BN == 64 || NLOAD > 0) && ((BM == 64 && WM == 32) || (BM == 128 && WM == 64 && NLOAD > 0))),
+  static_assert(!CONS || (WN == 32 && (BN == 64 || NLOAD > 0) && ((BM == 64 && WM == 32) || (BM == 128 && WM == 64 && NLOAD > 0))),
                 "fused AdaLN consumer: 64-row tiles of 32 x 32 wave sub-tiles, or (role split) 128-row tiles of 64 x 32 ones");
   static_assert(DBUF == 1 || (NLOAD > 0 && DSTEP == 1), "single fragment set: role split, one tile per hand-over");
   constexpr int NSTATT = BM * 4;
-  static_assert(FUSE != 1 || NSTATT <= NC, "fused consumer: 4 statistics threads per row");
+  static_assert(!CONS || NSTATT <= NC, "fused consumer: 4 statistics threads per row");
   static_assert(FUSE != 2 || EPI == EPI_GATE_RES, "the AdaLN producer is the gate+residual epilogue");
-  constexpr int NPC = NLOAD ? 0 : (FUSE == 1 ? 2 * TN + 4 : (FUSE == 2 ? 3 * TM * TN : ((PREF && EPI == EPI_GATE_RES) ? 2 * TM * TN : 0)));
+  constexpr int NPC = NLOAD ? 0 : (CONS ? 2 * TN + 4 : (FUSE == 2 ? 3 * TM * TN : ((PREF && EPI == EPI_GATE_RES) ? 2 * TM * TN : 0)));
   static_assert((NSTAGE - 2) * LPT + NPC <= 63, "vmcnt is a 6-bit counter");
   constexpr bool COLG = NLOAD > 0;
   f32x4 pf_bias[PREF ? TN : 1], pf_gate[PREF ? TN : 1][PREF ? (COLG ? 1 : TM) : 1], pf_x[PREF ? TN : 1][PREF ? TM : 1];
-  f32x4 pf_c[FUSE == 1 ? TN : 1], pf_d[FUSE == 1 ? TN : 1];
+  f32x4 pf_c[CONS ? TN : 1], pf_d[CONS ? TN : 1];
   f32x4 pf_ns[FUSE == 2 ? TN : 1][FUSE == 2 ? (COLG ? 1 : TM) : 1];
-  f32x2 pf_st[FUSE == 1 ? 4 : 1];
+  f32x2 pf_st[CONS ? 4 : 1];
+  int ode_e = 0;
+  float ode_h = 0.f;
   bool pf_live[PREF ? TM : 1];
   int pf_len[PREF ? TM : 1];
   float pf_rm[FUSE == 2 ? TM : 1];
@@ -199,7 +211,7 @@
         }
       }
     }
-    if (FUSE == 1) {
+    if (CONS) {
       const size_t eoff = a.eval_ptr ? (size_t)load_uniform_i32(a.eval_ptr) * a.cd_eval_stride : 0;
       const float* cbase = a.ln_c + eoff;
       const float* dbase = a.ln_d + eoff;
@@ -214,9 +226,17 @@
       const unsigned rel_max = (unsigned)((a.M - m0) * a.ln_parts - 1);
 #pragma unroll
       for (int u = 0; u < 4; ++u) {
-        const unsigned rel = min((unsigned)((tid & (NSTATT - 1)) * pp + min(u, pp - 1)), rel_max);
+        unsigned rel = min((unsigned)((tid & (NSTATT - 1)) * pp + min(u, pp - 1)), rel_max);
+        if constexpr (ODE) {
+          const int r = (tid & (NSTATT - 1)) >> 2;
+          rel = (unsigned)(min(grow(r), glast(r)) - m0) * (unsigned)a.ln_parts + (unsigned)((tid & 3) * pp + min(u, pp - 1));
+        }
         if (NC == NSTATT || tid < NSTATT) pf_st[u] = *(const f32x2*)(sbase + rel * 2u);
       }
+    }
+    if constexpr (ODE) {
+      ode_e = load_uniform_i32(a.ode_eval);
+      ode_h = __builtin_bit_cast(float, load_uniform_i32((const int*)(a.ode_coef + ode_e)));
     }
     if (PREF) {
 #pragma unroll
@@ -366,7 +386,7 @@
 
   if constexpr (DBG >= 3) { if (tid == 0) trc[3] = __builtin_amdgcn_s_memtime(); }
   float* fuse_lds = (float*)(smem + NSTAGE * STAGE);
-  if (FUSE == 1) {
+  if (CONS) {
     const int sq = tid & 3, pp = a.ln_parts >> 2;
     float sm = 0.f;
 #pragma unroll
@@ -386,12 +406,20 @@
     if (sq == 0 && (NC == NSTATT || tid < NSTATT)) {
       fuse_lds[(tid >> 2) * 2] = mean;
       fuse_lds[(tid >> 2) * 2 + 1] = rsqrtf(m2 / (float)a.K + a.ln_eps);
-      if (tile_n == 0 && m0 + (tid >> 2) < a.M) a.row_mean[m0 + (tid >> 2)] += mean;
+      const int mr = ODE ? grow(tid >> 2) : m0 + (tid >> 2);
+      if (tile_n == 0 && mr <= (ODE ? glast(tid >> 2) : a.M - 1)) a.row_mean[mr] += mean;
     }
     __syncthreads();
     if constexpr (DBG >= 3) { if (tid == 0) trc[42] = __builtin_amdgcn_s_memtime(); }
   }
   f32x4 xn[FUSE == 2 ? TN : 1][FUSE == 2 ? TM : 1];
+  f32x4 ov[ODE ? TN : 1][ODE ? TM : 1];
+  if constexpr (ODE) {
+#pragma unroll
+    for (int i = 0; i < TN; ++i)
+#pragma unroll
+      for (int j = 0; j < TM; ++j) ov[i][j] = f32x4{0.f, 0.f, 0.f, 0.f};
+  }
   if (PREF && EPI == EPI_GATE_RES) {
 #pragma unroll
     for (int j = 0; j < TM; ++j) {
@@ -415,14 +443,14 @@
 
 #pragma unroll
   for (int j = 0; j < TM; ++j) {
-    const int m = m0 + wm0 + j * 16 + fr;
+    const int m = ODE ? grow(wm0 + j * 16 + fr) : m0 + wm0 + j * 16 + fr;
     if (FUSE == 2) {
 #pragma unroll
       for (int i = 0; i < TN; ++i) xn[i][j] = pf_x[i][j];
     }
-    if (m >= a.M) continue;
+    if (m > (ODE ? glast(wm0 + j * 16 + fr) : a.M - 1)) continue;
     float ln_mean = 0.f, ln_rstd = 1.f;
-    if (FUSE == 1) {
+    if (CONS) {
       ln_mean = fuse_lds[(wm0 + j * 16 + fr) * 2];
       ln_rstd = fuse_lds[(wm0 + j * 16 + fr) * 2 + 1];
     }
@@ -453,7 +481,7 @@
       const int n = n0 + wn0 + i * 16 + fq * 4;
       if (n >= a.N) continue;
       f32x4 v = acc[i][j];
-      if (FUSE == 1) {
+      if (CONS) {
         v = ln_rstd * (v - ln_mean * pf_c[i]) + pf_d[i];
       } else if (PREF) {
         v += pf_bias[i];
@@ -468,6 +496,7 @@
             f2bf4(gelu_tanh_f(v[0]), gelu_tanh_f(v[1]), gelu_tanh_f(v[2]), gelu_tanh_f(v[3]));
       } else if (EPI == EPI_F32) {
         *(f32x4*)((float*)a.out + (size_t)m * a.ldo + n) = v;
+        if constexpr (ODE) ov[i][j] = v;
       } else if (EPI == EPI_GATE_RES && PREF) {
         if (pf_live[j]) {
           const f32x4 x_new = pf_x[i][j] + pf_gate[i][COLG ? 0 : j] * v;
@@ -516,6 +545,57 @@
     }
   }
   if constexpr (DBG >= 3) { if (tid == 0) trc[43] = __builtin_amdgcn_s_memtime(); }
+  if constexpr (ODE) {
+    constexpr int XS = BN + 4;
+    float* xch = (float*)smem;
+    if (pair) {
+      if (wm0 >= BM / 2) {
+#pragma unroll
+        for (int j = 0; j < TM; ++j)
+#pragma unroll
+          for (int i = 0; i < TN; ++i)
+            *(f32x4*)(xch + (wm0 - BM / 2 + j * 16 + fr) * XS + wn0 + i * 16 + fq * 4) = ov[i][j];
+      }
+      __syncthreads();
+    }
+    if (!pair || wm0 < BM / 2) {
+      float* traj = a.ode_traj;
+      if (traj && a.ode_traj_stride) traj += (size_t)((ode_e + 1) / a.ode_traj_div) * (size_t)a.ode_traj_stride;
+#pragma unroll
+      for (int j = 0; j < TM; ++j) {
+        const int r = wm0 + j * 16 + fr, m = grow(r);
+        if (m > glast(r)) continue;
+#pragma unroll
+        for (int i = 0; i < TN; ++i) {
+          const int n = n0 + wn0 + i * 16 + fq * 4;
+          if (n >= a.N) continue;
+          const size_t idx = (size_t)m * a.N + n;
+          const f32x4 p0 = ov[i][j], b = *(const f32x4*)(a.ode_base + idx);
+          f32x4 y;
+          if (pair) {
+            const f32x4 p1 = *(const f32x4*)(xch + r * XS + wn0 + i * 16 + fq * 4);
+#pragma unroll
+            for (int q = 0; q < 4; ++q) y[q] = f5e_cfg_step(p0[q], p1[q], a.ode_w0, b[q], ode_h);
+          } else {
+#pragma unroll
+            for (int q = 0; q < 4; ++q) y[q] = b[q] + ode_h * p0[q];
+          }
+          *(f32x4*)(a.ode_dst + idx) = y;
+          if (traj) *(f32x4*)(traj + idx) = y;
+        }
+      }
+    }
+    if (a.ode_done) {
+      __syncthreads();
+      if (tid == 0) {
+        const unsigned t = atomicAdd(a.ode_done, 1u);
+        if (t == (unsigned)a.n_main - 1u) {
+          *a.ode_eval = ode_e + 1;
+          *a.ode_done = 0u;
+        }
+      }
+    }
+  }
   if (FUSE == 2) {
 #pragma unroll
     for (int j = 0; j < TM; ++j) {
@@ -602,6 +682,7 @@
 int launch(GemmArgs& a, hipStream_t st) {
   constexpr int BK = 64;
   a.tiles_m = (a.M + BM - 1) / BM;
+  if (FUSE == 3 && a.ode_mode == 1) a.tiles_m = (a.ode_half + BM / 2 - 1) / (BM / 2);
   a.tiles_n = (a.N + BN - 1) / BN;
   if (a.M > a.N) {
     a.m_major = 1;
@@ -810,6 +891,24 @@
 
 extern "C" {
 
+int f5e_gemm_bf16_final_ode(hipStream_t st, const void* A, int lda, const void* W, int ldw, float* pred, int M, int N, int K,
+                            const f5e_ln_fuse* ln, const f5e_ode_fuse* ode) {
+  F5E_REQUIRE(ln && ln->stats && ode, "gemm_bf16_final_ode: the fused-AdaLN consumer side and the update are required");
+  GemmArgs a{};
+  a.A = (const bf16*)A; a.lda = lda; a.W = (const bf16*)W; a.ldw = ldw;
+  a.M = M; a.N = N; a.K = K; a.out = pred; a.ldo = N;
+  if (int e = check_common(a)) return e;
+  if (int e = set_consumer(a, ln, nullptr)) return e;
+  F5E_REQUIRE(pred && ode->base && ode->dst && ode->coef && ode->eval_ptr, "gemm_bf16_final_ode: null operand");
+  F5E_REQUIRE(ode->mode == 0 || (ode->mode == 1 && M % 2 == 0), "gemm_bf16_final_ode: mode 0 (plain) or 1 (CFG, two branches of M / 2 rows)");
+  F5E_REQUIRE(ode->traj_stride >= 0 && ode->traj_div >= 1, "gemm_bf16_final_ode: bad trajectory indexing");
+  F5E_REQUIRE((unsigned long long)(M + 64) * (unsigned)lda * 2ull < (1ull << 32), "gemm_bf16_final_ode: A panel too large");
+  a.ode_mode = ode->mode; a.ode_half = ode->mode == 1 ? M / 2 : M; a.ode_w0 = ode->w0;
+  a.ode_base = ode->base; a.ode_dst = ode->dst; a.ode_traj = ode->traj; a.ode_traj_stride = ode->traj_stride;
+  a.ode_traj_div = ode->traj_div; a.ode_coef = ode->coef; a.ode_eval = ode->eval_ptr; a.ode_done = ode->done_ctr;
+  return launch<64, 64, EPI_F32, 3, 2, 2, 0, 3>(a, st);
+}
+
 int f5e_gemm_bf16_bias(hipStream_t st, const void* A, int lda, const void* W, int ldw, const float* bias, void* out,
                        int ldo, int M, int N, int K, int act, int out_f32, int tile_hint) {
   return f5e_gemm_bf16_bias_ln(st, A, lda, W, ldw, bias, out, ldo, M, N, K, act, out_f32, tile_hint, nullptr);
diff --git a/f5e-tts_amd/csrc/gemm_bf16_args.h b/f5e-tts_amd/csrc/gemm_bf16_args.h
--- a/f5e-tts_amd/csrc/gemm_bf16_args.h
+++ b/f5e-tts_amd/csrc/gemm_bf16_args.h
@@ -33,6 +33,11 @@
   int pp_ngroup;
   F5ePrefetch pf;
   unsigned pf_per_wg;
+  int ode_mode, ode_half;
+  float ode_w0;
+  const float* ode_base; float* ode_dst; float* ode_traj;
+  long long ode_traj_stride; int ode_traj_div;
+  const float* ode_coef; int* ode_eval; unsigned* ode_done;
 };
 
 static_assert(offsetof(GemmArgs, n_main) + sizeof(int) == 64, "hot kernarg fields must fill exactly the first 64-byte line");
diff --git a/f5e-tts_amd/csrc/runtime.hip b/f5e-tts_amd/csrc/runtime.hip
--- a/f5e-tts_amd/csrc/runtime.hip
+++ b/f5e-tts_amd/csrc/runtime.hip
@@ -178,7 +178,7 @@
     }                                                                             \
   } while (0)
 
-int f5e_dit_forward(hipStream_t st, const f5e_dit_plan* p) {
+static int dit_forward_impl(hipStream_t st, const f5e_dit_plan* p, const f5e_ode_fuse* tail) {
   F5E_REQUIRE(p, "dit_forward: null plan");
   F5E_REQUIRE(p->S > 0 && p->B > 0 && p->S % p->B == 0 && p->N > 0 && p->L > 0, "dit_forward: bad S/B/N/L");
   F5E_REQUIRE(p->D % 256 == 0 && p->H > 0 && p->FF % 64 == 0 && p->mel % 4 == 0, "dit_forward: unsupported dims");
@@ -191,8 +191,8 @@
 
   F5E_TIMED(F5E_OP_INPROJ, f5e_gemm_f32(st, p->y, p->mel, p->B * p->N, F5E_ACT_NONE, p->w_x, p->ldw_x, nullptr, F5E_ACT_NONE, nullptr,
                        p->in_const, D, M, nullptr, p->h0, D, p->h0_bf16, D, M, D, p->mel));
-  F5E_TIMED(F5E_OP_CONVPOS, f5e_convpos(st, p->h0_bf16, D, p->convpos_w1, p->convpos_b1, 0, p->c1, D, nullptr, 0, nullptr, 0, p->S, p->N, D, p->convpos_groups));
-  F5E_TIMED(F5E_OP_CONVPOS, f5e_convpos(st, p->c1, D, p->convpos_w2, p->convpos_b2, 1, nullptr, 0, p->x, D, p->h0, D, p->S, p->N, D, p->convpos_groups));
+  F5E_TIMED(F5E_OP_CONVPOS, f5e_convpos_pair(st, p->h0_bf16, D, p->convpos_w1, p->convpos_b1, p->convpos_w2, p->convpos_b2, p->c1, D,
+                                             p->x, D, p->h0, D, p->S, p->N, D, p->convpos_groups));
 
   if (p->w_skip) {
     F5E_REQUIRE(p->skip_res && p->skip_tmp, "dit_forward: long skip needs skip_res / skip_tmp");
@@ -276,10 +276,15 @@
                                           0, &prod, pfon ? &pf_nx : nullptr));
     }
     cons.c = p->cd + (size_t)p->L * ls; cons.d = cons.c + p->mel;
+    if (tail) {
+      F5E_TIMED(F5E_OP_FINAL, f5e_gemm_bf16_final_ode(st, p->hn, D, p->w_proj, D, p->pred, M, p->mel, D, &cons, tail));
+      return F5E_OK;
+    }
     F5E_TIMED(F5E_OP_FINAL, f5e_gemm_bf16_bias_ln(st, p->hn, D, p->w_proj, D, nullptr, p->pred, p->mel, M, p->mel, D,
                                     F5E_ACT_NONE, 1, 0, &cons));
     return F5E_OK;
   }
+  F5E_REQUIRE(!tail, "dit_forward: the fused update needs the fused-AdaLN path");
   for (int l = 0; l < p->L; ++l) {
     const f5e_dit_block_weights& w = p->blocks[l];
     const float* mb = p->mod + (size_t)l * 6 * D;
@@ -309,6 +314,8 @@
   return F5E_OK;
 }
 
+int f5e_dit_forward(hipStream_t st, const f5e_dit_plan* p) { return dit_forward_impl(st, p, nullptr); }
+
 int f5e_sample_loop(hipStream_t st, const f5e_loop_plan* lp) {
   F5E_REQUIRE(lp && lp->eval_a, "sample_loop: null plan");
   F5E_REQUIRE(lp->steps > 0 && lp->n > 0 && lp->y && lp->pred && lp->coef && lp->eval_ptr && lp->done_ctr,
@@ -320,17 +327,26 @@
     F5E_REQUIRE(lp->y_mid && lp->eval_b->y == lp->y_mid && lp->eval_b->eval_ptr == lp->eval_ptr,
                 "sample_loop: eval_b must read y_mid and the loop's evaluation counter");
   const long long ts = lp->traj ? lp->n : 0;
+  auto fusable = [&](const f5e_dit_plan* p) {
+    return p && p->fuse_ln && !p->w_skip && (lp->mode == 0 || lp->mode == 1) && p->mel % 128 != 0 && p->pred == lp->pred &&
+           p->S == (lp->mode + 1) * p->B && lp->n == (long long)p->B * p->N * p->mel;
+  };
+  const bool fuse_a = fusable(lp->eval_a), fuse_b = midpoint && fusable(lp->eval_b);
+  auto eval_update = [&](const f5e_dit_plan* p, bool fused, float* dst, float* traj, long long traj_stride, int traj_div) -> int {
+    if (fused) {
+      const f5e_ode_fuse tail{lp->mode, lp->w0, lp->y, dst, traj, traj_stride, traj_div, lp->coef, lp->eval_ptr, lp->done_ctr};
+      return dit_forward_impl(st, p, &tail);
+    }
+    F5E_TRY(dit_forward_impl(st, p, nullptr));
+    return f5e_ode_update_traj(st, lp->pred, lp->n, lp->mode, lp->w0, lp->w1, lp->y, dst, traj, traj_stride, traj_div, lp->coef,
+                               lp->eval_ptr, lp->done_ctr, lp->n);
+  };
   for (int i = 0; i < lp->steps; ++i) {
-    F5E_TRY(f5e_dit_forward(st, lp->eval_a));
     if (!midpoint) {
-      F5E_TRY(f5e_ode_update_traj(st, lp->pred, lp->n, lp->mode, lp->w0, lp->w1, lp->y, lp->y, lp->traj, ts, 1, lp->coef,
-                                  lp->eval_ptr, lp->done_ctr, lp->n));
+      F5E_TRY(eval_update(lp->eval_a, fuse_a, lp->y, lp->traj, ts, 1));
     } else {
-      F5E_TRY(f5e_ode_update_traj(st, lp->pred, lp->n, lp->mode, lp->w0, lp->w1, lp->y, lp->y_mid, nullptr, 0, 1, lp->coef,
-                                  lp->eval_ptr, lp->done_ctr, lp->n));
-      F5E_TRY(f5e_dit_forward(st, lp->eval_b));
-      F5E_TRY(f5e_ode_update_traj(st, lp->pred, lp->n, lp->mode, lp->w0, lp->w1, lp->y, lp->y, lp->traj, ts, 2, lp->coef,
-                                  lp->eval_ptr, lp->done_ctr, lp->n));
+      F5E_TRY(eval_update(lp->eval_a, fuse_a, lp->y_mid, nullptr, 0, 1));
+      F5E_TRY(eval_update(lp->eval_b, fuse_b, lp->y, lp->traj, ts, 2));
     }
   }
   return F5E_OK;
diff --git a/f5e-tts_amd/ops.py b/f5e-tts_amd/ops.py
--- a/f5e-tts_amd/ops.py
+++ b/f5e-tts_amd/ops.py
@@ -240,6 +240,18 @@
           "f5e_convpos")
 
 
+def convpos_pair(x: Tensor, w1_packed: Tensor, bias1: Tensor, w2_packed: Tensor, bias2: Tensor, S: int, N: int, *,
+                 out_f32: Tensor, resid: Tensor, mid_bf16: Optional[Tensor] = None):
+    require_device()
+    check(lib().f5e_convpos_pair(_stream(), _p(x, BF, "x"), x.stride(0), _p(w1_packed, BF, "w1_packed"),
+                                 _p(bias1, F32, "bias1"), _p(w2_packed, BF, "w2_packed"), _p(bias2, F32, "bias2"),
+                                 _p(mid_bf16, BF, "mid_bf16"), mid_bf16.stride(0) if mid_bf16 is not None else 0,
+                                 _p(out_f32, F32, "out_f32"), out_f32.stride(0), _p(resid, F32, "resid"),
+                                 resid.stride(0), S, N, x.shape[1], w1_packed.shape[0]),
+          "f5e_convpos_pair")
+    return out_f32
+
+
 def dwconv7(x: Tensor, w_t: Tensor, bias: Tensor, out: Tensor):
     require_device()
     B, T, Cc = x.shape
@@ -287,6 +299,22 @@
                                     _p(dst, F32, "dst"), C.c_void_p(traj.data_ptr()) if traj is not None else None,
                                     traj_stride, traj_div, _p(coef, F32, "coef"), _p(eval_ptr, I32, "eval_ptr"),
                                     _p(done_ctr, I32, "done_ctr"), base.numel()), "f5e_ode_update")
+    return dst
+
+
+def gemm_bf16_final_ode(a: Tensor, w: Tensor, pred: Tensor, ln, mode: int, w0: float, base: Tensor, dst: Tensor,
+                        coef: Tensor, eval_ptr: Tensor, traj: Optional[Tensor] = None, done_ctr: Optional[Tensor] = None,
+                        traj_stride: int = 0, traj_div: int = 1):
+    require_device()
+    M, K = a.shape
+    o = _C.OdeFuse()
+    o.mode, o.w0, o.base, o.dst = mode, w0, _p(base, F32, "base").value, _p(dst, F32, "dst").value
+    o.traj, o.traj_stride, o.traj_div = traj.data_ptr() if traj is not None else None, traj_stride, traj_div
+    o.coef, o.eval_ptr = _p(coef, F32, "coef").value, _p(eval_ptr, I32, "eval_ptr").value
+    o.done_ctr = done_ctr.data_ptr() if done_ctr is not None else None
+    check(lib().f5e_gemm_bf16_final_ode(_stream(), _p(a, BF, "a"), a.stride(0), _p(w, BF, "w"), w.stride(0),
+                                        _p(pred, F32, "pred"), M, w.shape[0], K, _ln_ref(ln), C.byref(o)),
+          "f5e_gemm_bf16_final_ode")
     return dst
 
 
diff --git a/include/f5e_abi.h b/include/f5e_abi.h
--- a/include/f5e_abi.h
+++ b/include/f5e_abi.h
@@ -92,6 +92,10 @@
 F5E_API int f5e_convpos(f5e_stream st, const void* x, int ldx, const void* w_packed, const float* bias, int mode,
                 void* out_bf16, int ldo, float* out_f32, int ldo32, const float* resid, int ldr, int S, int N, int D,
                 int groups);
+
+F5E_API int f5e_convpos_pair(f5e_stream st, const void* x, int ldx, const void* w1_packed, const float* bias1,
+                     const void* w2_packed, const float* bias2, void* mid_bf16, int ldm, float* out_f32, int ldo32,
+                     const float* resid, int ldr, int S, int N, int D, int groups);
 
 F5E_API int f5e_dwconv7(f5e_stream st, const float* x, const float* w_t, const float* bias, float* y, int B, int T, int C);
 
@@ -109,6 +113,15 @@
                         const float* base, float* dst, float* traj, long long traj_stride, int traj_div,
                         const float* coef, int* eval_ptr, unsigned* done_ctr, long long n);
 F5E_API int f5e_advance_eval(f5e_stream st, int* eval_ptr);
+
+typedef struct f5e_ode_fuse {
+  int mode; float w0;
+  const float* base; float* dst;
+  float* traj; long long traj_stride; int traj_div;
+  const float* coef; int* eval_ptr; unsigned* done_ctr;
+} f5e_ode_fuse;
+F5E_API int f5e_gemm_bf16_final_ode(f5e_stream st, const void* A, int lda, const void* W, int ldw, float* pred, int M, int N,
+                            int K, const f5e_ln_fuse* ln, const f5e_ode_fuse* ode);
 F5E_API int f5e_stitch(f5e_stream st, const float* cond, const float* y, const unsigned char* mask, float* out, long long rows,
                int C);
 F5E_API int f5e_cast_bf16(f5e_stream st, const float* x, void* y, long long n);
```

New measurement: 13000 mel-frames/s, median of 6. About the same (+0.3%).
